# convexbrain/Totsu

Measured on AMD Instinct MI355X. Metric: solver iters/sec + time-to-eps, dense SOCP n=50k (value = iters/sec; time_to_eps beside it), higher is better.
Workload: dtype f32

## Files before the change

### include/totsu_f32hip.h

```cpp
#ifndef TOTSU_F32HIP_H
#define TOTSU_F32HIP_H

#include <stddef.h>
#include <stdint.h>

#ifdef __cplusplus
extern "C" {
#endif

#define THIP_E_INVALID   10001
#define THIP_E_NOTINIT   10002
#define THIP_E_NOGPU     10003
#define THIP_E_WORK      10004
#define THIP_E_NOCONV    10005
#define THIP_E_TIMEOUT   10006

int  thip_init(int device);
int  thip_shutdown(void);
int  thip_device_count(int *host_count);
int  thip_set_stream(void *hip_stream);
void *thip_get_stream(void);
int  thip_sync(void);
const char *thip_last_error(void);
const char *thip_version(void);

int thip_alloc(size_t n, float **out);
int thip_alloc_zeroed(size_t n, float **out);
int thip_free(float *p);
int thip_h2d(float *dst, const float *host_src, size_t n);
int thip_d2h(float *host_dst, const float *src, size_t n);
int thip_get(const float *x, size_t idx, float *host_out);
int thip_set(float *x, size_t idx, float val);

int thip_norm(size_t n, const float *x, float *host_out);
int thip_copy(size_t n, const float *x, float *y);
int thip_scale(size_t n, float alpha, float *x);
int thip_add(size_t n, float alpha, const float *x, float *y);
int thip_adds(size_t n, float s, float *y);
int thip_abssum(size_t len, const float *x, size_t incx, float *host_out);
int thip_transform_di(size_t n, float alpha, const float *d, const float *x,
                      float beta, float *y);

int thip_transform_ge(int transpose, size_t n_row, size_t n_col, float alpha, const float *mat,
                      const float *x, float beta, float *y);
int thip_set_lazy_gemv(int on);
int thip_get_lazy_gemv(int *host_on);
int thip_lazy_gemv_stats(int64_t *host_deferred, int64_t *host_flushes);
int thip_lazy_plan_stats(int64_t *host_hits, int64_t *host_misses);
int thip_lazy_read_stats(int64_t *host_served, int64_t *host_fetches);
int thip_transform_sp(size_t n, float alpha, const float *mat, const float *x, float beta, float *y);
enum { THIP_A_F32 = 0, THIP_A_BF16 = 1, THIP_A_F16 = 2 };
int thip_to_bf16(size_t n_row, size_t n_col, const float *mat, uint16_t *mat16, size_t ld16);
int thip_transform_ge_bf16(int transpose, size_t n_row, size_t n_col, float alpha, const uint16_t *mat16, size_t ld16,
                           const float *x, float beta, float *y);
int thip_to_f16(size_t n_row, size_t n_col, const float *mat, uint16_t *mat16, size_t ld16, float *inv_scale);
int thip_transform_ge_f16(int transpose, size_t n_row, size_t n_col, float alpha, const uint16_t *mat16, size_t ld16,
                          const float *inv_scale, const float *x, float beta, float *y);
size_t thip_map_eig_worklen(size_t n);
int thip_map_eig(size_t n, float *mat, int has_scale, float scale_diag, float eps_zero,
                 float *work, size_t worklen, int map_kind);
int thip_eig_decompose(size_t n, float *mat, int has_scale, float scale_diag, float eps_zero,
                       float *work, size_t worklen, float *host_w);
int thip_eig_rebuild(size_t n, float *mat, int has_scale, float scale_diag,
                     float *work, size_t worklen, const float *host_e, const uint8_t *host_keep);
int thip_eig_engine_info(int *host_engine, int *host_polish, float *host_cert);

int thip_spmv_csr(size_t n_row, size_t n_col, size_t nnz, const int64_t *dev_rowptr, const int32_t *dev_colidx,
                  const float *vals, float alpha, const float *x, float beta, float *y, int abs_mode);

typedef struct thip_sptile thip_sptile;
int thip_sptile_create(size_t n_row, size_t n_col, size_t nnz, const int64_t *host_colptr, const int32_t *host_rowidx,
                       const float *host_vals, thip_sptile **out);
int thip_sptile_destroy(thip_sptile *mat);
int thip_sptile_mv(thip_sptile *mat, int transpose, float alpha, const float *x, float beta, float *y, int abs_mode);
int thip_sptile_info(const thip_sptile *mat, size_t *host_nnz_stored, int *host_tiles, int *host_items_n, int *host_items_t,
                     int *host_slices_n, int *host_slices_t, size_t *host_bytes);
int thip_sptile_layout(const thip_sptile *mat, int *host_dense_tiles, size_t *host_indexed_entries, size_t *host_bytes_per_product);

typedef struct thip_sptile_builder thip_sptile_builder;
int thip_sptile_builder_create(size_t n_row, size_t n_col, thip_sptile_builder **out);
int thip_sptile_builder_count(thip_sptile_builder *b, size_t c0, size_t ncols, const float *dev_panel, size_t ld);
int thip_sptile_builder_plan(thip_sptile_builder *b, size_t *host_nnz, int *host_dense_tiles, size_t *host_indexed_entries,
                             size_t *host_bytes_per_product);
int thip_sptile_builder_fill(thip_sptile_builder *b, size_t c0, size_t ncols, const float *dev_panel, size_t ld);
int thip_sptile_builder_finish(thip_sptile_builder *b, thip_sptile **out);
int thip_sptile_builder_destroy(thip_sptile_builder *b);
int thip_sptile_from_dense(size_t n_row, size_t n_col, const float *dev_mat, size_t ld, thip_sptile **out);

int thip_norm_dev(size_t n, const float *x, float *dev_out);
int thip_dot_dev(size_t n, const float *x, const float *y, float *dev_out);
int thip_abssum_dev(size_t len, const float *x, size_t incx, float *dev_out);

int thip_absadd_cols(size_t n_row, size_t n_col, const float *mat, float *tau);
int thip_absadd_rows(size_t n_row, size_t n_col, const float *mat, float *sigma);
int thip_absadd_sympack(size_t n, const float *mat, float *y);
int thip_recip_max(size_t n, float eps_zero, float *x);

int thip_copy_block(int transposed, size_t n_row, size_t n_col, float sign, const float *src, float *dst, size_t ld_dst);

enum { THIP_CONE_ZERO = 0, THIP_CONE_RPOS = 1, THIP_CONE_SOC = 2, THIP_CONE_ROTSOC = 3, THIP_CONE_PSD = 4 };
int thip_proj_zero(int dual_cone, size_t n, float *x);
int thip_proj_rpos(size_t n, float *x);
int thip_proj_soc(size_t n, float *x);
int thip_proj_rotsoc(size_t n, float *x);
int thip_proj_soc_batched(float *x, const int64_t *dev_offs, size_t n_cones, int rotated, size_t max_len);
int thip_proj_psd(size_t sn, float *x, float eps_zero, float *work, size_t worklen);
int thip_group_min_batched(float *dp_tau, const int64_t *dev_offs, size_t n_groups, size_t max_len);

typedef struct thip_solver thip_solver;

enum { THIP_STATE_COMPENSATED = 0, THIP_STATE_PLAIN = 1 };

typedef struct thip_param {
    int64_t max_iter;
    float   eps_acc, eps_inf, eps_zero;
    int64_t log_period;
    int32_t state_arith;
    int32_t reserved;
} thip_param;

enum { THIP_ST_RUNNING = -1,
       THIP_ST_OK = 0, THIP_ST_UNBOUNDED = 1, THIP_ST_INFEASIBLE = 2, THIP_ST_EXCESS_ITER = 3,
       THIP_ST_INVALID_OP = 4, THIP_ST_WORK_SHORTAGE = 5, THIP_ST_CONE_FAILURE = 6 };

enum { THIP_SCHED_REFERENCE = 0,
       THIP_SCHED_FUSED     = 1,
       THIP_SCHED_CARRIED   = 2,
       THIP_SCHED_SWEEP     = 3 };

typedef struct thip_problem {
    size_t n, m;
    const float *mat_a;
    const float *vec_b;
    const float *vec_c;
    const float *vec_b_rowabs;
    size_t n_seg;
    const int32_t *host_seg_type;
    const int64_t *host_seg_len;
} thip_problem;

typedef struct thip_status {
    int32_t state;
    int64_t iter;
    int32_t kind;
    float   cri[3];
    float   tau, kappa;
    float   norm_b, norm_c;
} thip_status;

typedef int (*thip_allreduce_fn)(void *ctx, float *dev_buf, size_t n, void *hip_stream);

int thip_comm_unique_id(uint8_t *host_id128);
int thip_comm_init(int rank, int world, const uint8_t *host_id128);
int thip_comm_allreduce(float *dev_buf, size_t n);
int thip_comm_count(int *host_ranks);
int thip_comm_destroy(void);
int thip_solver_use_rccl(thip_solver *s);

int thip_oneshot_init(int rank, int world, size_t max_floats, uint8_t *host_handle64);
int thip_oneshot_connect(const uint8_t *host_handles);
int thip_oneshot_allreduce(float *dev_buf, size_t n);
int thip_oneshot_error(int *host_err);
int thip_oneshot_destroy(void);
int thip_solver_use_oneshot(thip_solver *s);

int thip_solver_create(const thip_problem *prob, const thip_param *par, int schedule, thip_solver **out);
int thip_solver_set_csr(thip_solver *s, size_t nnz,
                        const int64_t *dev_rowptr, const int32_t *dev_colidx, const float *dev_vals,
                        const int64_t *dev_t_rowptr, const int32_t *dev_t_colidx, const float *dev_t_vals);
int thip_solver_set_sptile(thip_solver *s, thip_sptile *mat);
int thip_solver_set_allreduce(thip_solver *s, thip_allreduce_fn fn, void *ctx);
enum { THIP_OVERLAP_OFF = 0, THIP_OVERLAP_LOCAL_ROWS = 1, THIP_OVERLAP_COLUMN_PIPELINE = 2, THIP_OVERLAP_COLUMN_INORDER = 3 };
int thip_solver_set_overlap(thip_solver *s, int mode);
int thip_solver_set_gemv_autotune(thip_solver *s, int on);
int thip_solver_set_lda_pad(thip_solver *s, int floats);
int thip_solver_overlap_info(thip_solver *s, int *host_mode, int *host_launches_per_pass, size_t *host_split_col);
int thip_solver_set_a_storage(thip_solver *s, int a_kind);
int thip_solver_set_a_bf16(thip_solver *s, const uint16_t *mat16, size_t ld16);
int thip_solver_set_a_f16(thip_solver *s, const uint16_t *mat16, size_t ld16, const float *inv_scale);
int thip_solver_init(thip_solver *s);
int thip_solver_run(thip_solver *s, int64_t max_steps, int64_t poll_every, thip_status *host_status);
int thip_solver_status(thip_solver *s, thip_status *host_status);
int thip_solver_resume(thip_solver *s);
int thip_solver_set_param(thip_solver *s, const thip_param *par);
int thip_solver_solution(thip_solver *s, float *host_x, float *host_y);
int thip_solver_iterate(thip_solver *s, float *host_x, float *host_y);
int thip_solver_precond(thip_solver *s, float *host_dp_tau, float *host_dp_sigma);
int thip_solver_destroy(thip_solver *s);
int thip_solver_passes(const thip_solver *s, int *host_passes, size_t *host_bytes_per_pass);
int thip_solver_schedule_in_use(thip_solver *s, int *host_schedule);
int thip_solver_set_sweep_min_bytes(thip_solver *s, size_t bytes);
int thip_solver_sweep_plan(thip_solver *s, int *host_members, int *host_cols_per_panel, int *host_slots, float *host_ms);
int thip_solver_set_column_shard(thip_solver *s, int on);
int thip_sweep_probe(size_t m, size_t n_local, size_t lda, int elem, int *host_ok);

typedef struct thip_batch thip_batch;
#define THIP_BATCH_MAX 64
#define THIP_BATCH_GROUP_DEFAULT 8
typedef struct thip_batch_info_t {
    int32_t n_inst, max_group;
    int32_t groups;
    int32_t passes_per_iteration;
    int32_t a_copies;
    int32_t reserved;
    size_t  a_bytes;
    size_t  bytes_per_pass;
    size_t  arena_bytes;
    size_t  device_bytes;
    int32_t plan_nj[4], plan_blocks[4];
    float   plan_ms[4];
} thip_batch_info_t;
int thip_batch_create(const thip_problem *prob_template, int n_inst, const float *const *host_vec_b,
                      const float *const *host_vec_c, const thip_param *par, thip_batch **out);
int thip_batch_set_a_storage(thip_batch *b, int a_kind);
int thip_batch_set_gemv_autotune(thip_batch *b, int on);
int thip_batch_set_max_group(thip_batch *b, int max_group);
int thip_batch_set_param(thip_batch *b, const thip_param *par);
int thip_batch_init(thip_batch *b);
int thip_batch_run(thip_batch *b, int64_t max_steps, int64_t poll_every, thip_status *host_status);
int thip_batch_status(thip_batch *b, int i, thip_status *host_status);
int thip_batch_solution(thip_batch *b, int i, float *host_x, float *host_y);
int thip_batch_iterate(thip_batch *b, int i, float *host_x, float *host_y);
int thip_batch_precond(thip_batch *b, int i, float *host_dp_tau, float *host_dp_sigma);
int thip_batch_info(const thip_batch *b, thip_batch_info_t *host_info);
int thip_batch_grouping(int n_inst, int max_group, int *host_groups, int *host_members);
int thip_batch_destroy(thip_batch *b);

int thip_batch_replace(thip_batch *b, int i, const float *dev_vec_b, const float *dev_vec_c);
int thip_batch_set_regroup(thip_batch *b, int on);
int thip_batch_run_until_any(thip_batch *b, int64_t max_steps, int64_t poll_every, thip_status *host_status);
int thip_batch_live_grouping(int n_inst, int max_group, const int *host_live, int *host_groups, int *host_group_sizes,
                             int *host_members);
typedef struct thip_batch_counters_t {
    int64_t launches[4];
    int64_t passes;
    int64_t instance_iterations;
    int64_t replaced;
    int32_t live, groups_now;
} thip_batch_counters_t;
int thip_batch_counters(const thip_batch *b, thip_batch_counters_t *host);

typedef struct thip_smallbatch thip_smallbatch;
typedef struct thip_smallbatch_info_t {
    int32_t n_prob, threads;
    int32_t lds_bytes, live;
    size_t  arena_bytes;
    size_t  device_bytes;
    size_t  device_bytes_all;
    int64_t launches, workgroups;
} thip_smallbatch_info_t;
int thip_smallbatch_fits(size_t n, size_t m, size_t n_seg, const int32_t *host_seg_type, const int64_t *host_seg_len,
                         size_t *host_lds_bytes, int *host_threads);
int thip_smallbatch_create(size_t n, size_t m, size_t n_prob, const float *dev_mats_a, const float *dev_vecs_b,
                           const float *dev_vecs_c, const float *dev_vecs_b_rowabs, size_t n_seg, const int32_t *host_seg_type,
                           const int64_t *host_seg_len, const thip_param *par, thip_smallbatch **out);
int thip_smallbatch_set_param(thip_smallbatch *h, const thip_param *par);
int thip_smallbatch_init(thip_smallbatch *h);
int thip_smallbatch_run(thip_smallbatch *h, int64_t max_steps, int64_t poll_every, thip_status *host_status);
int thip_smallbatch_run_until_any(thip_smallbatch *h, int64_t max_steps, int64_t poll_every, thip_status *host_status);
int thip_smallbatch_status(thip_smallbatch *h, int i, thip_status *host_status);
int thip_smallbatch_solution(thip_smallbatch *h, int i, float *host_x, float *host_y);
int thip_smallbatch_iterate(thip_smallbatch *h, int i, float *host_x, float *host_y);
int thip_smallbatch_precond(thip_smallbatch *h, int i, float *host_dp_tau, float *host_dp_sigma);
int thip_smallbatch_replace(thip_smallbatch *h, int i, const float *dev_mat_a, const float *dev_vec_b, const float *dev_vec_c,
                            const float *dev_vec_b_rowabs);
int thip_smallbatch_info(const thip_smallbatch *h, thip_smallbatch_info_t *host_info);
int thip_smallbatch_destroy(thip_smallbatch *h);

typedef struct thip_midbatch thip_midbatch;
typedef struct thip_midbatch_info_t {
    int32_t n_prob, threads;
    int32_t lds_bytes, live;
    size_t  arena_bytes;
    size_t  device_bytes;
    size_t  device_bytes_all;
    int64_t launches, workgroups;
    int32_t load_bytes, reserved;
    size_t  a_bytes_per_iter;
} thip_midbatch_info_t;
int thip_midbatch_fits(size_t n, size_t m, size_t n_seg, const int32_t *host_seg_type, const int64_t *host_seg_len,
                       size_t *host_lds_bytes, int *host_threads);
int thip_midbatch_create(size_t n, size_t m, size_t n_prob, const float *dev_mats_a, const float *dev_vecs_b,
                         const float *dev_vecs_c, const float *dev_vecs_b_rowabs, size_t n_seg, const int32_t *host_seg_type,
                         const int64_t *host_seg_len, const thip_param *par, thip_midbatch **out);
int thip_midbatch_set_param(thip_midbatch *h, const thip_param *par);
int thip_midbatch_init(thip_midbatch *h);
int thip_midbatch_run(thip_midbatch *h, int64_t max_steps, int64_t poll_every, thip_status *host_status);
int thip_midbatch_run_until_any(thip_midbatch *h, int64_t max_steps, int64_t poll_every, thip_status *host_status);
int thip_midbatch_status(thip_midbatch *h, int i, thip_status *host_status);
int thip_midbatch_solution(thip_midbatch *h, int i, float *host_x, float *host_y);
int thip_midbatch_iterate(thip_midbatch *h, int i, float *host_x, float *host_y);
int thip_midbatch_precond(thip_midbatch *h, int i, float *host_dp_tau, float *host_dp_sigma);
int thip_midbatch_replace(thip_midbatch *h, int i, const float *dev_mat_a, const float *dev_vec_b, const float *dev_vec_c,
                          const float *dev_vec_b_rowabs);
int thip_midbatch_info(const thip_midbatch *h, thip_midbatch_info_t *host_info);
int thip_midbatch_destroy(thip_midbatch *h);

typedef struct thip_sdpbatch thip_sdpbatch;
typedef struct thip_sdpbatch_info_t {
    int32_t n_prob, threads;
    int32_t lds_bytes, live;
    size_t  arena_bytes;
    size_t  device_bytes;
    size_t  device_bytes_all;
    int64_t launches, workgroups;
    int32_t load_bytes, reserved;
    size_t  a_bytes_per_iter;
    int32_t max_psd_order, n_psd;
    size_t  psd_lds_bytes;
} thip_sdpbatch_info_t;
int thip_sdpbatch_fits(size_t n, size_t m, size_t n_seg, const int32_t *host_seg_type, const int64_t *host_seg_len,
                       size_t *host_lds_bytes, int *host_threads);
int thip_sdpbatch_create(size_t n, size_t m, size_t n_prob, const float *dev_mats_a, const float *dev_vecs_b,
                         const float *dev_vecs_c, const float *dev_vecs_b_rowabs, size_t n_seg, const int32_t *host_seg_type,
                         const int64_t *host_seg_len, const thip_param *par, thip_sdpbatch **out);
int thip_sdpbatch_set_param(thip_sdpbatch *h, const thip_param *par);
int thip_sdpbatch_init(thip_sdpbatch *h);
int thip_sdpbatch_run(thip_sdpbatch *h, int64_t max_steps, int64_t poll_every, thip_status *host_status);
int thip_sdpbatch_run_until_any(thip_sdpbatch *h, int64_t max_steps, int64_t poll_every, thip_status *host_status);
int thip_sdpbatch_status(thip_sdpbatch *h, int i, thip_status *host_status);
int thip_sdpbatch_solution(thip_sdpbatch *h, int i, float *host_x, float *host_y);
int thip_sdpbatch_iterate(thip_sdpbatch *h, int i, float *host_x, float *host_y);
int thip_sdpbatch_precond(thip_sdpbatch *h, int i, float *host_dp_tau, float *host_dp_sigma);
int thip_sdpbatch_replace(thip_sdpbatch *h, int i, const float *dev_mat_a, const float *dev_vec_b, const float *dev_vec_c,
                          const float *dev_vec_b_rowabs);
int thip_sdpbatch_info(const thip_sdpbatch *h, thip_sdpbatch_info_t *host_info);
int thip_sdpbatch_destroy(thip_sdpbatch *h);

int thip_stream_probe(const void *dev_ptr, size_t bytes, int reps, float *host_best_ms, float *host_avg_ms);

int thip_solver_sweep_faults(thip_solver *s, int *host_faults, int *host_last_word, int64_t *host_restored_iter);
int thip_solver_set_sweep_publish(thip_solver *s, int agent_scope);
int thip_sweep_publish_selftest(int mode, int *host_agent_scope, int *host_info);


int thip_solver_gemv_plan(const thip_solver *s, int *host_nj, int *host_blocks, float *host_ms);

int thip_prof_enable(int on);
int thip_prof_read_psd(int64_t *host_spans, double *host_total_ms);
int thip_prof_read(int64_t *host_launches, double *host_total_ms);

int thip_gen_vector(float *out, size_t n, uint64_t seed, uint64_t stream, uint64_t idx0,
                    int kind, float scale, float shift);
int thip_gen_matrix(float *out, size_t n_row, size_t n_col, size_t lda, uint64_t seed, uint64_t stream,
                    uint64_t row0, uint64_t col0, uint64_t ld_index, int kind, float scale, float shift);
int thip_gen_identity(float *out, size_t n_row, size_t n_col, size_t lda, uint64_t row0, float value);


#ifdef __cplusplus
}
#endif
#endif
```

### rust/totsu_f32hip/src/ffi.rs

```rust
#![allow(non_camel_case_types)]
use std::os::raw::{c_char, c_int, c_void};

#[repr(C)]
pub struct thip_param { pub max_iter: i64, pub eps_acc: f32, pub eps_inf: f32, pub eps_zero: f32, pub log_period: i64,
                         pub state_arith: i32, pub reserved: i32 }
pub const THIP_STATE_COMPENSATED: i32 = 0;
pub const THIP_STATE_PLAIN: i32 = 1;

#[repr(C)]
pub struct thip_problem {
    pub n: usize, pub m: usize,
    pub mat_a: *const f32, pub vec_b: *const f32, pub vec_c: *const f32, pub vec_b_rowabs: *const f32,
    pub n_seg: usize, pub host_seg_type: *const i32, pub host_seg_len: *const i64,
}

#[repr(C)]
#[derive(Default, Clone, Copy)]
pub struct thip_status {
    pub state: i32, pub iter: i64, pub kind: i32, pub cri: [f32; 3],
    pub tau: f32, pub kappa: f32, pub norm_b: f32, pub norm_c: f32,
}

#[repr(C)]
#[derive(Default, Clone, Copy)]
pub struct thip_batch_info_t {
    pub n_inst: i32, pub max_group: i32, pub groups: i32, pub passes_per_iteration: i32, pub a_copies: i32, pub reserved: i32,
    pub a_bytes: usize, pub bytes_per_pass: usize, pub arena_bytes: usize, pub device_bytes: usize,
    pub plan_nj: [i32; 4], pub plan_blocks: [i32; 4], pub plan_ms: [f32; 4],
}
#[repr(C)]
#[derive(Default, Clone, Copy)]
pub struct thip_batch_counters_t {
    pub launches: [i64; 4], pub passes: i64, pub instance_iterations: i64, pub replaced: i64,
    pub live: i32, pub groups_now: i32,
}
#[repr(C)]
#[derive(Default, Clone, Copy)]
pub struct thip_smallbatch_info_t {
    pub n_prob: i32, pub threads: i32, pub lds_bytes: i32, pub live: i32,
    pub arena_bytes: usize, pub device_bytes: usize, pub device_bytes_all: usize,
    pub launches: i64, pub workgroups: i64,
}
#[repr(C)]
#[derive(Default, Clone, Copy)]
pub struct thip_midbatch_info_t {
    pub n_prob: i32, pub threads: i32, pub lds_bytes: i32, pub live: i32,
    pub arena_bytes: usize, pub device_bytes: usize, pub device_bytes_all: usize,
    pub launches: i64, pub workgroups: i64,
    pub load_bytes: i32, pub reserved: i32,
    pub a_bytes_per_iter: usize,
}
#[repr(C)]
#[derive(Default, Clone, Copy)]
pub struct thip_sdpbatch_info_t {
    pub n_prob: i32, pub threads: i32, pub lds_bytes: i32, pub live: i32,
    pub arena_bytes: usize, pub device_bytes: usize, pub device_bytes_all: usize,
    pub launches: i64, pub workgroups: i64,
    pub load_bytes: i32, pub reserved: i32,
    pub a_bytes_per_iter: usize,
    pub max_psd_order: i32, pub n_psd: i32,
    pub psd_lds_bytes: usize,
}
pub const THIP_BATCH_MAX: c_int = 64;
pub const THIP_BATCH_GROUP_DEFAULT: c_int = 8;

#[repr(C)]
pub struct thip_sweep_test {
    pub m: usize, pub n: usize, pub lda: usize,
    pub mat_a: *const f32, pub v: *const f32, pub xy: *const f32, pub c: *const f32, pub su: *const f32, pub tx: *const f32,
    pub u: *mut f32, pub ku: *mut f32,
    pub xx_in: *const f32, pub kx_in: *const f32,
    pub xx_out: *mut f32, pub kx_out: *mut f32, pub gp: *mut f32, pub hn: *mut f32, pub h3: *mut f32,
    pub kappa: f32, pub rtau: f32, pub first: i32, pub reps: i32,
    pub force_members: i32, pub pub_agent: i32, pub variant: i32, pub elem: i32,
    pub inv_s: *const f32,
    pub host_sums: *mut f32,
}

pub enum thip_solver {}
pub enum thip_batch {}
pub enum thip_smallbatch {}
pub enum thip_midbatch {}
pub enum thip_sdpbatch {}
pub enum thip_sptile {}
pub enum thip_sptile_builder {}
pub type thip_allreduce_fn = Option<unsafe extern "C" fn(ctx: *mut c_void, dev_buf: *mut f32, n: usize, stream: *mut c_void) -> c_int>;

pub const THIP_CONE_ZERO: i32 = 0;
pub const THIP_CONE_RPOS: i32 = 1;
pub const THIP_CONE_SOC: i32 = 2;
pub const THIP_CONE_ROTSOC: i32 = 3;
pub const THIP_CONE_PSD: i32 = 4;
pub const THIP_SCHED_REFERENCE: c_int = 0;
pub const THIP_SCHED_FUSED: c_int = 1;
pub const THIP_SCHED_CARRIED: c_int = 2;
pub const THIP_SCHED_SWEEP: c_int = 3;
pub const THIP_OVERLAP_OFF: c_int = 0;
pub const THIP_OVERLAP_LOCAL_ROWS: c_int = 1;
pub const THIP_OVERLAP_COLUMN_PIPELINE: c_int = 2;
pub const THIP_OVERLAP_COLUMN_INORDER: c_int = 3;

extern "C" {
    pub fn thip_init(device: c_int) -> c_int;
    pub fn thip_shutdown() -> c_int;
    pub fn thip_sync() -> c_int;
    pub fn thip_last_error() -> *const c_char;
    pub fn thip_alloc(n: usize, out: *mut *mut f32) -> c_int;
    pub fn thip_free(p: *mut f32) -> c_int;
    pub fn thip_h2d(dst: *mut f32, host_src: *const f32, n: usize) -> c_int;
    pub fn thip_d2h(host_dst: *mut f32, src: *const f32, n: usize) -> c_int;
    pub fn thip_get(x: *const f32, idx: usize, host_out: *mut f32) -> c_int;
    pub fn thip_set(x: *mut f32, idx: usize, val: f32) -> c_int;

    pub fn thip_norm(n: usize, x: *const f32, host_out: *mut f32) -> c_int;
    pub fn thip_copy(n: usize, x: *const f32, y: *mut f32) -> c_int;
    pub fn thip_scale(n: usize, alpha: f32, x: *mut f32) -> c_int;
    pub fn thip_add(n: usize, alpha: f32, x: *const f32, y: *mut f32) -> c_int;
    pub fn thip_adds(n: usize, s: f32, y: *mut f32) -> c_int;
    pub fn thip_abssum(len: usize, x: *const f32, incx: usize, host_out: *mut f32) -> c_int;
    pub fn thip_transform_di(n: usize, alpha: f32, d: *const f32, x: *const f32, beta: f32, y: *mut f32) -> c_int;

    pub fn thip_transform_ge(transpose: c_int, n_row: usize, n_col: usize, alpha: f32, mat: *const f32,
                             x: *const f32, beta: f32, y: *mut f32) -> c_int;
    pub fn thip_transform_sp(n: usize, alpha: f32, mat: *const f32, x: *const f32, beta: f32, y: *mut f32) -> c_int;
    pub fn thip_map_eig_worklen(n: usize) -> usize;
    pub fn thip_map_eig(n: usize, mat: *mut f32, has_scale: c_int, scale_diag: f32, eps_zero: f32,
                        work: *mut f32, worklen: usize, map_kind: c_int) -> c_int;
    pub fn thip_eig_decompose(n: usize, mat: *mut f32, has_scale: c_int, scale_diag: f32, eps_zero: f32,
                              work: *mut f32, worklen: usize, host_w: *mut f32) -> c_int;
    pub fn thip_eig_rebuild(n: usize, mat: *mut f32, has_scale: c_int, scale_diag: f32, work: *mut f32,
                            worklen: usize, host_e: *const f32, host_keep: *const u8) -> c_int;
    pub fn thip_eig_engine_info(host_engine: *mut c_int, host_polish: *mut c_int, host_cert: *mut f32) -> c_int;

    pub fn thip_absadd_cols(n_row: usize, n_col: usize, mat: *const f32, tau: *mut f32) -> c_int;
    pub fn thip_absadd_rows(n_row: usize, n_col: usize, mat: *const f32, sigma: *mut f32) -> c_int;
    pub fn thip_recip_max(n: usize, eps_zero: f32, x: *mut f32) -> c_int;
    pub fn thip_copy_block(transposed: c_int, n_row: usize, n_col: usize, sign: f32, src: *const f32, dst: *mut f32,
                           ld_dst: usize) -> c_int;
    pub fn thip_set_lazy_gemv(on: c_int) -> c_int;
    pub fn thip_get_lazy_gemv(host_on: *mut c_int) -> c_int;
    pub fn thip_lazy_gemv_stats(host_deferred: *mut i64, host_flushes: *mut i64) -> c_int;
    pub fn thip_lazy_plan_stats(host_hits: *mut i64, host_misses: *mut i64) -> c_int;
    pub fn thip_lazy_read_stats(host_served: *mut i64, host_fetches: *mut i64) -> c_int;
    pub fn thip_proj_zero(dual_cone: c_int, n: usize, x: *mut f32) -> c_int;
    pub fn thip_proj_rpos(n: usize, x: *mut f32) -> c_int;
    pub fn thip_proj_soc(n: usize, x: *mut f32) -> c_int;
    pub fn thip_proj_rotsoc(n: usize, x: *mut f32) -> c_int;
    pub fn thip_proj_psd(sn: usize, x: *mut f32, eps_zero: f32, work: *mut f32, worklen: usize) -> c_int;

    pub fn thip_solver_create(prob: *const thip_problem, par: *const thip_param, schedule: c_int,
                              out: *mut *mut thip_solver) -> c_int;
    pub fn thip_solver_set_allreduce(s: *mut thip_solver, f: thip_allreduce_fn, ctx: *mut c_void) -> c_int;
    pub fn thip_solver_set_overlap(s: *mut thip_solver, mode: c_int) -> c_int;
    pub fn thip_solver_overlap_info(s: *mut thip_solver, host_mode: *mut c_int, host_launches_per_pass: *mut c_int,
                                    host_split_col: *mut usize) -> c_int;
    pub fn thip_solver_init(s: *mut thip_solver) -> c_int;
    pub fn thip_solver_run(s: *mut thip_solver, max_steps: i64, poll_every: i64, host_status: *mut thip_status) -> c_int;
    pub fn thip_solver_solution(s: *mut thip_solver, host_x: *mut f32, host_y: *mut f32) -> c_int;
    pub fn thip_solver_destroy(s: *mut thip_solver) -> c_int;

    pub fn thip_version() -> *const c_char;
    pub fn thip_device_count(host_count: *mut c_int) -> c_int;
    pub fn thip_set_stream(hip_stream: *mut c_void) -> c_int;
    pub fn thip_get_stream() -> *mut c_void;
    pub fn thip_alloc_zeroed(n: usize, out: *mut *mut f32) -> c_int;

    pub fn thip_norm_dev(n: usize, x: *const f32, dev_out: *mut f32) -> c_int;
    pub fn thip_dot_dev(n: usize, x: *const f32, y: *const f32, dev_out: *mut f32) -> c_int;
    pub fn thip_abssum_dev(len: usize, x: *const f32, incx: usize, dev_out: *mut f32) -> c_int;
    pub fn thip_absadd_sympack(n: usize, mat: *const f32, y: *mut f32) -> c_int;
    pub fn thip_spmv_csr(n_row: usize, n_col: usize, nnz: usize, dev_rowptr: *const i64, dev_colidx: *const i32,
                         vals: *const f32, alpha: f32, x: *const f32, beta: f32, y: *mut f32, abs_mode: c_int) -> c_int;
    pub fn thip_sptile_create(n_row: usize, n_col: usize, nnz: usize, host_colptr: *const i64, host_rowidx: *const i32,
                              host_vals: *const f32, out: *mut *mut thip_sptile) -> c_int;
    pub fn thip_sptile_destroy(mat: *mut thip_sptile) -> c_int;
    pub fn thip_sptile_mv(mat: *mut thip_sptile, transpose: c_int, alpha: f32, x: *const f32, beta: f32, y: *mut f32,
                          abs_mode: c_int) -> c_int;
    pub fn thip_sptile_info(mat: *const thip_sptile, host_nnz_stored: *mut usize, host_tiles: *mut c_int,
                            host_items_n: *mut c_int, host_items_t: *mut c_int, host_slices_n: *mut c_int,
                            host_slices_t: *mut c_int, host_bytes: *mut usize) -> c_int;
    pub fn thip_sptile_layout(mat: *const thip_sptile, host_dense_tiles: *mut c_int, host_indexed_entries: *mut usize,
                              host_bytes_per_product: *mut usize) -> c_int;
    pub fn thip_sptile_builder_create(n_row: usize, n_col: usize, out: *mut *mut thip_sptile_builder) -> c_int;
    pub fn thip_sptile_builder_count(b: *mut thip_sptile_builder, c0: usize, ncols: usize, dev_panel: *const f32,
                                     ld: usize) -> c_int;
    pub fn thip_sptile_builder_plan(b: *mut thip_sptile_builder, host_nnz: *mut usize, host_dense_tiles: *mut c_int,
                                    host_indexed_entries: *mut usize, host_bytes_per_product: *mut usize) -> c_int;
    pub fn thip_sptile_builder_fill(b: *mut thip_sptile_builder, c0: usize, ncols: usize, dev_panel: *const f32,
                                    ld: usize) -> c_int;
    pub fn thip_sptile_builder_finish(b: *mut thip_sptile_builder, out: *mut *mut thip_sptile) -> c_int;
    pub fn thip_sptile_builder_destroy(b: *mut thip_sptile_builder) -> c_int;
    pub fn thip_sptile_from_dense(n_row: usize, n_col: usize, dev_mat: *const f32, ld: usize,
                                  out: *mut *mut thip_sptile) -> c_int;
    pub fn thip_to_bf16(n_row: usize, n_col: usize, mat: *const f32, mat16: *mut u16, ld16: usize) -> c_int;
    pub fn thip_transform_ge_bf16(transpose: c_int, n_row: usize, n_col: usize, alpha: f32, mat16: *const u16,
                                  ld16: usize, x: *const f32, beta: f32, y: *mut f32) -> c_int;

    pub fn thip_proj_soc_batched(x: *mut f32, dev_offs: *const i64, n_cones: usize, rotated: c_int, max_len: usize) -> c_int;
    pub fn thip_group_min_batched(dp_tau: *mut f32, dev_offs: *const i64, n_groups: usize, max_len: usize) -> c_int;

    pub fn thip_solver_set_csr(s: *mut thip_solver, nnz: usize, dev_rowptr: *const i64, dev_colidx: *const i32,
                               dev_vals: *const f32, dev_t_rowptr: *const i64, dev_t_colidx: *const i32,
                               dev_t_vals: *const f32) -> c_int;
    pub fn thip_solver_set_sptile(s: *mut thip_solver, mat: *mut thip_sptile) -> c_int;
    pub fn thip_solver_set_a_storage(s: *mut thip_solver, a_kind: c_int) -> c_int;
    pub fn thip_solver_set_a_bf16(s: *mut thip_solver, mat16: *const u16, ld16: usize) -> c_int;
    pub fn thip_solver_set_a_f16(s: *mut thip_solver, mat16: *const u16, ld16: usize, inv_scale: *const f32) -> c_int;
    pub fn thip_to_f16(n_row: usize, n_col: usize, mat: *const f32, mat16: *mut u16, ld16: usize, inv_scale: *mut f32) -> c_int;
    pub fn thip_transform_ge_f16(transpose: c_int, n_row: usize, n_col: usize, alpha: f32, mat16: *const u16, ld16: usize,
                                 inv_scale: *const f32, x: *const f32, beta: f32, y: *mut f32) -> c_int;
    pub fn thip_solver_set_param(s: *mut thip_solver, par: *const thip_param) -> c_int;
    pub fn thip_solver_resume(s: *mut thip_solver) -> c_int;
    pub fn thip_solver_status(s: *mut thip_solver, host_status: *mut thip_status) -> c_int;
    pub fn thip_solver_iterate(s: *mut thip_solver, host_x: *mut f32, host_y: *mut f32) -> c_int;
    pub fn thip_solver_precond(s: *mut thip_solver, host_dp_tau: *mut f32, host_dp_sigma: *mut f32) -> c_int;
    pub fn thip_solver_passes(s: *const thip_solver, host_passes: *mut c_int, host_bytes_per_pass: *mut usize) -> c_int;
    pub fn thip_solver_schedule_in_use(s: *mut thip_solver, host_schedule: *mut c_int) -> c_int;
    pub fn thip_solver_set_sweep_min_bytes(s: *mut thip_solver, bytes: usize) -> c_int;
    pub fn thip_solver_set_column_shard(s: *mut thip_solver, on: c_int) -> c_int;
    pub fn thip_sweep_probe(m: usize, n_local: usize, lda: usize, elem: c_int, host_ok: *mut c_int) -> c_int;
    pub fn thip_solver_sweep_plan(s: *mut thip_solver, host_members: *mut c_int, host_cols_per_panel: *mut c_int, host_slots: *mut c_int, host_ms: *mut f32) -> c_int;
    pub fn thip_stream_probe(dev_ptr: *const c_void, bytes: usize, reps: c_int, host_best_ms: *mut f32, host_avg_ms: *mut f32) -> c_int;
    pub fn thip_solver_sweep_faults(s: *mut thip_solver, host_faults: *mut c_int, host_last_word: *mut c_int, host_restored_iter: *mut i64) -> c_int;
    pub fn thip_solver_set_sweep_publish(s: *mut thip_solver, agent_scope: c_int) -> c_int;
    pub fn thip_sweep_publish_selftest(mode: c_int, host_agent_scope: *mut c_int, host_info: *mut c_int) -> c_int;
    pub fn thip_solver_gemv_plan(s: *const thip_solver, host_nj: *mut c_int, host_blocks: *mut c_int, host_ms: *mut f32) -> c_int;

    pub fn thip_batch_create(prob_template: *const thip_problem, n_inst: c_int, host_vec_b: *const *const f32,
                             host_vec_c: *const *const f32, par: *const thip_param, out: *mut *mut thip_batch) -> c_int;
    pub fn thip_batch_set_a_storage(b: *mut thip_batch, a_kind: c_int) -> c_int;
    pub fn thip_batch_set_gemv_autotune(b: *mut thip_batch, on: c_int) -> c_int;
    pub fn thip_batch_set_max_group(b: *mut thip_batch, max_group: c_int) -> c_int;
    pub fn thip_batch_set_param(b: *mut thip_batch, par: *const thip_param) -> c_int;
    pub fn thip_batch_init(b: *mut thip_batch) -> c_int;
    pub fn thip_batch_run(b: *mut thip_batch, max_steps: i64, poll_every: i64, host_status: *mut thip_status) -> c_int;
    pub fn thip_batch_status(b: *mut thip_batch, i: c_int, host_status: *mut thip_status) -> c_int;
    pub fn thip_batch_solution(b: *mut thip_batch, i: c_int, host_x: *mut f32, host_y: *mut f32) -> c_int;
    pub fn thip_batch_iterate(b: *mut thip_batch, i: c_int, host_x: *mut f32, host_y: *mut f32) -> c_int;
    pub fn thip_batch_precond(b: *mut thip_batch, i: c_int, host_dp_tau: *mut f32, host_dp_sigma: *mut f32) -> c_int;
    pub fn thip_batch_info(b: *const thip_batch, host_info: *mut thip_batch_info_t) -> c_int;
    pub fn thip_batch_grouping(n_inst: c_int, max_group: c_int, host_groups: *mut c_int, host_members: *mut c_int) -> c_int;
    pub fn thip_batch_destroy(b: *mut thip_batch) -> c_int;
    pub fn thip_batch_replace(b: *mut thip_batch, i: c_int, dev_vec_b: *const f32, dev_vec_c: *const f32) -> c_int;
    pub fn thip_batch_set_regroup(b: *mut thip_batch, on: c_int) -> c_int;
    pub fn thip_batch_run_until_any(b: *mut thip_batch, max_steps: i64, poll_every: i64, host_status: *mut thip_status) -> c_int;
    pub fn thip_batch_live_grouping(n_inst: c_int, max_group: c_int, host_live: *const c_int, host_groups: *mut c_int,
                                    host_group_sizes: *mut c_int, host_members: *mut c_int) -> c_int;
    pub fn thip_batch_counters(b: *const thip_batch, host: *mut thip_batch_counters_t) -> c_int;

    pub fn thip_smallbatch_fits(n: usize, m: usize, n_seg: usize, host_seg_type: *const i32, host_seg_len: *const i64,
                                host_lds_bytes: *mut usize, host_threads: *mut c_int) -> c_int;
    pub fn thip_smallbatch_create(n: usize, m: usize, n_prob: usize, dev_mats_a: *const f32, dev_vecs_b: *const f32,
                                  dev_vecs_c: *const f32, dev_vecs_b_rowabs: *const f32, n_seg: usize, host_seg_type: *const i32,
                                  host_seg_len: *const i64, par: *const thip_param, out: *mut *mut thip_smallbatch) -> c_int;
    pub fn thip_smallbatch_set_param(h: *mut thip_smallbatch, par: *const thip_param) -> c_int;
    pub fn thip_smallbatch_init(h: *mut thip_smallbatch) -> c_int;
    pub fn thip_smallbatch_run(h: *mut thip_smallbatch, max_steps: i64, poll_every: i64, host_status: *mut thip_status) -> c_int;
    pub fn thip_smallbatch_run_until_any(h: *mut thip_smallbatch, max_steps: i64, poll_every: i64, host_status: *mut thip_status) -> c_int;
    pub fn thip_smallbatch_status(h: *mut thip_smallbatch, i: c_int, host_status: *mut thip_status) -> c_int;
    pub fn thip_smallbatch_solution(h: *mut thip_smallbatch, i: c_int, host_x: *mut f32, host_y: *mut f32) -> c_int;
    pub fn thip_smallbatch_iterate(h: *mut thip_smallbatch, i: c_int, host_x: *mut f32, host_y: *mut f32) -> c_int;
    pub fn thip_smallbatch_precond(h: *mut thip_smallbatch, i: c_int, host_dp_tau: *mut f32, host_dp_sigma: *mut f32) -> c_int;
    pub fn thip_smallbatch_replace(h: *mut thip_smallbatch, i: c_int, dev_mat_a: *const f32, dev_vec_b: *const f32,
                                   dev_vec_c: *const f32, dev_vec_b_rowabs: *const f32) -> c_int;
    pub fn thip_smallbatch_info(h: *const thip_smallbatch, host_info: *mut thip_smallbatch_info_t) -> c_int;
    pub fn thip_smallbatch_destroy(h: *mut thip_smallbatch) -> c_int;
    pub fn thip_test_smallbatch_force_threads(h: *mut thip_smallbatch, threads: c_int) -> c_int;

    pub fn thip_midbatch_fits(n: usize, m: usize, n_seg: usize, host_seg_type: *const i32, host_seg_len: *const i64,
                              host_lds_bytes: *mut usize, host_threads: *mut c_int) -> c_int;
    pub fn thip_midbatch_create(n: usize, m: usize, n_prob: usize, dev_mats_a: *const f32, dev_vecs_b: *const f32,
                                dev_vecs_c: *const f32, dev_vecs_b_rowabs: *const f32, n_seg: usize, host_seg_type: *const i32,
                                host_seg_len: *const i64, par: *const thip_param, out: *mut *mut thip_midbatch) -> c_int;
    pub fn thip_midbatch_set_param(h: *mut thip_midbatch, par: *const thip_param) -> c_int;
    pub fn thip_midbatch_init(h: *mut thip_midbatch) -> c_int;
    pub fn thip_midbatch_run(h: *mut thip_midbatch, max_steps: i64, poll_every: i64, host_status: *mut thip_status) -> c_int;
    pub fn thip_midbatch_run_until_any(h: *mut thip_midbatch, max_steps: i64, poll_every: i64, host_status: *mut thip_status) -> c_int;
    pub fn thip_midbatch_status(h: *mut thip_midbatch, i: c_int, host_status: *mut thip_status) -> c_int;
    pub fn thip_midbatch_solution(h: *mut thip_midbatch, i: c_int, host_x: *mut f32, host_y: *mut f32) -> c_int;
    pub fn thip_midbatch_iterate(h: *mut thip_midbatch, i: c_int, host_x: *mut f32, host_y: *mut f32) -> c_int;
    pub fn thip_midbatch_precond(h: *mut thip_midbatch, i: c_int, host_dp_tau: *mut f32, host_dp_sigma: *mut f32) -> c_int;
    pub fn thip_midbatch_replace(h: *mut thip_midbatch, i: c_int, dev_mat_a: *const f32, dev_vec_b: *const f32,
                                 dev_vec_c: *const f32, dev_vec_b_rowabs: *const f32) -> c_int;
    pub fn thip_midbatch_info(h: *const thip_midbatch, host_info: *mut thip_midbatch_info_t) -> c_int;
    pub fn thip_midbatch_destroy(h: *mut thip_midbatch) -> c_int;
    pub fn thip_test_midbatch_force_threads(h: *mut thip_midbatch, threads: c_int) -> c_int;

    pub fn thip_sdpbatch_fits(n: usize, m: usize, n_seg: usize, host_seg_type: *const i32, host_seg_len: *const i64,
                              host_lds_bytes: *mut usize, host_threads: *mut c_int) -> c_int;
    pub fn thip_sdpbatch_create(n: usize, m: usize, n_prob: usize, dev_mats_a: *const f32, dev_vecs_b: *const f32,
                                dev_vecs_c: *const f32, dev_vecs_b_rowabs: *const f32, n_seg: usize, host_seg_type: *const i32,
                                host_seg_len: *const i64, par: *const thip_param, out: *mut *mut thip_sdpbatch) -> c_int;
    pub fn thip_sdpbatch_set_param(h: *mut thip_sdpbatch, par: *const thip_param) -> c_int;
    pub fn thip_sdpbatch_init(h: *mut thip_sdpbatch) -> c_int;
    pub fn thip_sdpbatch_run(h: *mut thip_sdpbatch, max_steps: i64, poll_every: i64, host_status: *mut thip_status) -> c_int;
    pub fn thip_sdpbatch_run_until_any(h: *mut thip_sdpbatch, max_steps: i64, poll_every: i64, host_status: *mut thip_status) -> c_int;
    pub fn thip_sdpbatch_status(h: *mut thip_sdpbatch, i: c_int, host_status: *mut thip_status) -> c_int;
    pub fn thip_sdpbatch_solution(h: *mut thip_sdpbatch, i: c_int, host_x: *mut f32, host_y: *mut f32) -> c_int;
    pub fn thip_sdpbatch_iterate(h: *mut thip_sdpbatch, i: c_int, host_x: *mut f32, host_y: *mut f32) -> c_int;
    pub fn thip_sdpbatch_precond(h: *mut thip_sdpbatch, i: c_int, host_dp_tau: *mut f32, host_dp_sigma: *mut f32) -> c_int;
    pub fn thip_sdpbatch_replace(h: *mut thip_sdpbatch, i: c_int, dev_mat_a: *const f32, dev_vec_b: *const f32,
                                 dev_vec_c: *const f32, dev_vec_b_rowabs: *const f32) -> c_int;
    pub fn thip_sdpbatch_info(h: *const thip_sdpbatch, host_info: *mut thip_sdpbatch_info_t) -> c_int;
    pub fn thip_sdpbatch_destroy(h: *mut thip_sdpbatch) -> c_int;
    pub fn thip_test_sdpbatch_force_threads(h: *mut thip_sdpbatch, threads: c_int) -> c_int;
    pub fn thip_test_sdpbatch_project(k: c_int, count: c_int, dev_packed: *mut f32, dev_rx_or_null: *mut f32) -> c_int;

    pub fn thip_comm_unique_id(host_id128: *mut u8) -> c_int;
    pub fn thip_comm_init(rank: c_int, world: c_int, host_id128: *const u8) -> c_int;
    pub fn thip_comm_allreduce(dev_buf: *mut f32, n: usize) -> c_int;
    pub fn thip_comm_count(host_ranks: *mut c_int) -> c_int;
    pub fn thip_comm_destroy() -> c_int;
    pub fn thip_solver_use_rccl(s: *mut thip_solver) -> c_int;
    pub fn thip_oneshot_init(rank: c_int, world: c_int, max_floats: usize, host_handle64: *mut u8) -> c_int;
    pub fn thip_oneshot_connect(host_handles: *const u8) -> c_int;
    pub fn thip_oneshot_allreduce(dev_buf: *mut f32, n: usize) -> c_int;
    pub fn thip_oneshot_error(host_err: *mut c_int) -> c_int;
    pub fn thip_oneshot_destroy() -> c_int;
    pub fn thip_solver_use_oneshot(s: *mut thip_solver) -> c_int;
    pub fn thip_solver_set_gemv_autotune(s: *mut thip_solver, on: c_int) -> c_int;
    pub fn thip_solver_set_lda_pad(s: *mut thip_solver, floats: c_int) -> c_int;

    pub fn thip_gen_vector(out: *mut f32, n: usize, seed: u64, stream: u64, idx0: u64, kind: c_int, scale: f32, shift: f32) -> c_int;
    pub fn thip_gen_matrix(out: *mut f32, n_row: usize, n_col: usize, lda: usize, seed: u64, stream: u64, row0: u64,
                           col0: u64, ld_index: u64, kind: c_int, scale: f32, shift: f32) -> c_int;
    pub fn thip_gen_identity(out: *mut f32, n_row: usize, n_col: usize, lda: usize, row0: u64, value: f32) -> c_int;

    pub fn thip_prof_enable(on: c_int) -> c_int;
    pub fn thip_prof_read(host_launches: *mut i64, host_total_ms: *mut f64) -> c_int;
    pub fn thip_prof_read_psd(host_spans: *mut i64, host_total_ms: *mut f64) -> c_int;
}

#[cfg(feature = "test-hooks")]
extern "C" {
    pub fn thip_test_eig_force(engine: c_int) -> c_int;
    pub fn thip_test_gemv_multi(m: usize, n: usize, mat: *const f32, nv: c_int, host_xn: *const *const f32, host_xt: *const *const f32,
                                host_out_n: *const *mut f32, host_out_t: *const *mut f32, host_stopped: *const c_int, nj: c_int,
                                target_blocks: c_int, reps: c_int, host_ms: *mut f32) -> c_int;
    pub fn thip_test_spin_allreduce(s: *mut thip_solver, latency_us: c_int) -> c_int;
    pub fn thip_test_sweep(t: *const thip_sweep_test, host_ms: *mut f32, host_info: *mut c_int) -> c_int;
    pub fn thip_test_solver_kahan(s: *mut thip_solver, host_kx: *mut f32, host_ky: *mut f32, host_ks: *mut f32, host_ku: *mut f32,
                                  host_kv: *mut f32, host_mtail_form: *mut c_int) -> c_int;
    pub fn thip_test_sweep_fault(s: *mut thip_solver, kind: c_int, after_sweeps: i64, spin_max: c_int) -> c_int;
    pub fn thip_test_gemm_sym(n: c_int, ld: c_int, alpha: f32, a: *const f32, b: *const f32, beta: f32, d: *const f32,
                              gamma: f32, c: *mut f32) -> c_int;
    pub fn thip_test_gemm_chain(shape: c_int, kernel: c_int, n: c_int, ld: c_int, nb: c_int, alpha: f32, x: *const f32,
                                y: *const f32, beta: f32, d: *const f32, gamma: f32, c: *mut f32) -> c_int;
    pub fn thip_test_chain_probe(mode: c_int, ld: c_int, reps: c_int, host_us: *mut f32) -> c_int;
    pub fn thip_test_sptile_time(mat: *mut thip_sptile, reps: c_int, host_ms: *mut f32) -> c_int;
    pub fn thip_test_sptile_equal(a: *const thip_sptile, b: *const thip_sptile, host_first_difference: *mut c_int) -> c_int;
    pub fn thip_test_gemm_dual(kernel: c_int, n: c_int, ld: c_int, nb: c_int, a: *const f32, b0: *const f32, b1: *const f32,
                               coef: *const f32, o0: *mut f32, o1: *mut f32) -> c_int;
}

pub const THIP_A_F32: c_int = 0;
pub const THIP_A_BF16: c_int = 1;
pub const THIP_A_F16: c_int = 2;

pub fn chk(rc: c_int) {
    if rc != 0 {
        let msg = unsafe { std::ffi::CStr::from_ptr(thip_last_error()) }.to_string_lossy().into_owned();
        panic!("totsu_f32hip: error {}: {}", rc, msg);
    }
}
```

### totsu_amd/_lib.py

```python
import ctypes as C
import os

_HERE = os.path.dirname(os.path.abspath(__file__))
SO_PATH = os.path.join(_HERE, "lib", "libtotsu_f32hip.so")

E_INVALID, E_NOTINIT, E_NOGPU, E_WORK, E_NOCONV, E_TIMEOUT = 10001, 10002, 10003, 10004, 10005, 10006

ST_RUNNING, ST_OK, ST_UNBOUNDED, ST_INFEASIBLE, ST_EXCESS_ITER, ST_INVALID_OP, ST_WORK_SHORTAGE, ST_CONE_FAILURE = \
    -1, 0, 1, 2, 3, 4, 5, 6
SCHED_REFERENCE, SCHED_FUSED, SCHED_CARRIED, SCHED_SWEEP = 0, 1, 2, 3
STATE_COMPENSATED, STATE_PLAIN = 0, 1
CONE_ZERO, CONE_RPOS, CONE_SOC, CONE_ROTSOC, CONE_PSD = 0, 1, 2, 3, 4

fp = C.POINTER(C.c_float)


class ThipError(RuntimeError):
    def __init__(self, code, msg):
        super().__init__("totsu_f32hip error %d: %s" % (code, msg))
        self.code = code


class Param(C.Structure):
    _fields_ = [("max_iter", C.c_int64), ("eps_acc", C.c_float), ("eps_inf", C.c_float),
                ("eps_zero", C.c_float), ("log_period", C.c_int64), ("state_arith", C.c_int32), ("reserved", C.c_int32)]


class Problem(C.Structure):
    _fields_ = [("n", C.c_size_t), ("m", C.c_size_t), ("mat_a", C.c_void_p), ("vec_b", C.c_void_p),
                ("vec_c", C.c_void_p), ("vec_b_rowabs", C.c_void_p), ("n_seg", C.c_size_t),
                ("host_seg_type", C.POINTER(C.c_int32)), ("host_seg_len", C.POINTER(C.c_int64))]


class Status(C.Structure):
    _fields_ = [("state", C.c_int32), ("iter", C.c_int64), ("kind", C.c_int32), ("cri", C.c_float * 3),
                ("tau", C.c_float), ("kappa", C.c_float), ("norm_b", C.c_float), ("norm_c", C.c_float)]


class SweepTest(C.Structure):
    _fields_ = [("m", C.c_size_t), ("n", C.c_size_t), ("lda", C.c_size_t)] + \
               [(k, C.c_void_p) for k in ("mat_a", "v", "xy", "c", "su", "tx", "u", "ku", "xx_in", "kx_in", "xx_out",
                                          "kx_out", "gp", "hn", "h3")] + \
               [("kappa", C.c_float), ("rtau", C.c_float), ("first", C.c_int32), ("reps", C.c_int32),
                ("force_members", C.c_int32), ("pub_agent", C.c_int32), ("variant", C.c_int32), ("elem", C.c_int32), ("inv_s", C.c_void_p),
                ("host_sums", C.POINTER(C.c_float))]


class BatchInfo(C.Structure):
    _fields_ = [("n_inst", C.c_int32), ("max_group", C.c_int32), ("groups", C.c_int32), ("passes_per_iteration", C.c_int32),
                ("a_copies", C.c_int32), ("reserved", C.c_int32), ("a_bytes", C.c_size_t), ("bytes_per_pass", C.c_size_t),
                ("arena_bytes", C.c_size_t), ("device_bytes", C.c_size_t), ("plan_nj", C.c_int32 * 4),
                ("plan_blocks", C.c_int32 * 4), ("plan_ms", C.c_float * 4)]


class BatchCounters(C.Structure):
    _fields_ = [("launches", C.c_int64 * 4), ("passes", C.c_int64), ("instance_iterations", C.c_int64), ("replaced", C.c_int64),
                ("live", C.c_int32), ("groups_now", C.c_int32)]


class SmallBatchInfo(C.Structure):
    _fields_ = [("n_prob", C.c_int32), ("threads", C.c_int32), ("lds_bytes", C.c_int32), ("live", C.c_int32),
                ("arena_bytes", C.c_size_t), ("device_bytes", C.c_size_t), ("device_bytes_all", C.c_size_t),
                ("launches", C.c_int64), ("workgroups", C.c_int64)]


class MidBatchInfo(C.Structure):
    _fields_ = SmallBatchInfo._fields_ + [("load_bytes", C.c_int32), ("reserved", C.c_int32), ("a_bytes_per_iter", C.c_size_t)]


class SdpBatchInfo(C.Structure):
    _fields_ = MidBatchInfo._fields_ + [("max_psd_order", C.c_int32), ("n_psd", C.c_int32), ("psd_lds_bytes", C.c_size_t)]


BATCH_MAX, BATCH_GROUP_DEFAULT = 64, 8
SMALLBATCH_MAX_DIM, SMALLBATCH_MAX_AREA, SMALLBATCH_MAX_PROB, SMALLBATCH_LDS_MAX = 1024, 24576, 1048576, 163840
ALLREDUCE_FN = C.CFUNCTYPE(C.c_int, C.c_void_p, C.c_void_p, C.c_size_t, C.c_void_p)

_sz, _f, _i, _vp, _u64 = C.c_size_t, C.c_float, C.c_int, C.c_void_p, C.c_uint64
PROTOTYPES = {
    "thip_init": (_i, [_i]),
    "thip_shutdown": (_i, []),
    "thip_device_count": (_i, [C.POINTER(_i)]),
    "thip_set_stream": (_i, [_vp]),
    "thip_get_stream": (_vp, []),
    "thip_sync": (_i, []),
    "thip_last_error": (C.c_char_p, []),
    "thip_version": (C.c_char_p, []),
    "thip_alloc": (_i, [_sz, C.POINTER(_vp)]),
    "thip_alloc_zeroed": (_i, [_sz, C.POINTER(_vp)]),
    "thip_free": (_i, [_vp]),
    "thip_h2d": (_i, [_vp, _vp, _sz]),
    "thip_d2h": (_i, [_vp, _vp, _sz]),
    "thip_get": (_i, [_vp, _sz, fp]),
    "thip_set": (_i, [_vp, _sz, _f]),
    "thip_norm": (_i, [_sz, _vp, fp]),
    "thip_copy": (_i, [_sz, _vp, _vp]),
    "thip_scale": (_i, [_sz, _f, _vp]),
    "thip_add": (_i, [_sz, _f, _vp, _vp]),
    "thip_adds": (_i, [_sz, _f, _vp]),
    "thip_abssum": (_i, [_sz, _vp, _sz, fp]),
    "thip_transform_di": (_i, [_sz, _f, _vp, _vp, _f, _vp]),
    "thip_transform_ge": (_i, [_i, _sz, _sz, _f, _vp, _vp, _f, _vp]),
    "thip_transform_sp": (_i, [_sz, _f, _vp, _vp, _f, _vp]),
    "thip_set_lazy_gemv": (_i, [_i]),
    "thip_get_lazy_gemv": (_i, [C.POINTER(_i)]),
    "thip_lazy_gemv_stats": (_i, [C.POINTER(C.c_int64), C.POINTER(C.c_int64)]),
    "thip_lazy_plan_stats": (_i, [C.POINTER(C.c_int64), C.POINTER(C.c_int64)]),
    "thip_lazy_read_stats": (_i, [C.POINTER(C.c_int64), C.POINTER(C.c_int64)]),
    "thip_to_bf16": (_i, [_sz, _sz, _vp, _vp, _sz]),
    "thip_to_f16": (_i, [_sz, _sz, _vp, _vp, _sz, _vp]),
    "thip_transform_ge_f16": (_i, [_i, _sz, _sz, _f, _vp, _sz, _vp, _vp, _f, _vp]),
    "thip_transform_ge_bf16": (_i, [_i, _sz, _sz, _f, _vp, _sz, _vp, _f, _vp]),
    "thip_spmv_csr": (_i, [_sz, _sz, _sz, _vp, _vp, _vp, _f, _vp, _f, _vp, _i]),
    "thip_sptile_create": (_i, [_sz, _sz, _sz, _vp, _vp, _vp, C.POINTER(_vp)]),
    "thip_sptile_destroy": (_i, [_vp]),
    "thip_sptile_mv": (_i, [_vp, _i, _f, _vp, _f, _vp, _i]),
    "thip_sptile_info": (_i, [_vp, C.POINTER(_sz), C.POINTER(_i), C.POINTER(_i), C.POINTER(_i), C.POINTER(_i), C.POINTER(_i),
                              C.POINTER(_sz)]),
    "thip_sptile_layout": (_i, [_vp, C.POINTER(_i), C.POINTER(_sz), C.POINTER(_sz)]),
    "thip_sptile_builder_create": (_i, [_sz, _sz, C.POINTER(_vp)]),
    "thip_sptile_builder_count": (_i, [_vp, _sz, _sz, _vp, _sz]),
    "thip_sptile_builder_plan": (_i, [_vp, C.POINTER(_sz), C.POINTER(_i), C.POINTER(_sz), C.POINTER(_sz)]),
    "thip_sptile_builder_fill": (_i, [_vp, _sz, _sz, _vp, _sz]),
    "thip_sptile_builder_finish": (_i, [_vp, C.POINTER(_vp)]),
    "thip_sptile_builder_destroy": (_i, [_vp]),
    "thip_sptile_from_dense": (_i, [_sz, _sz, _vp, _sz, C.POINTER(_vp)]),
    "thip_map_eig_worklen": (_sz, [_sz]),
    "thip_map_eig": (_i, [_sz, _vp, _i, _f, _f, _vp, _sz, _i]),
    "thip_eig_decompose": (_i, [_sz, _vp, _i, _f, _f, _vp, _sz, fp]),
    "thip_eig_rebuild": (_i, [_sz, _vp, _i, _f, _vp, _sz, fp, C.POINTER(C.c_uint8)]),
    "thip_eig_engine_info": (_i, [C.POINTER(_i), C.POINTER(_i), fp]),
    "thip_test_eig_force": (_i, [_i]),
    "thip_norm_dev": (_i, [_sz, _vp, _vp]),
    "thip_dot_dev": (_i, [_sz, _vp, _vp, _vp]),
    "thip_abssum_dev": (_i, [_sz, _vp, _sz, _vp]),
    "thip_absadd_cols": (_i, [_sz, _sz, _vp, _vp]),
    "thip_absadd_rows": (_i, [_sz, _sz, _vp, _vp]),
    "thip_absadd_sympack": (_i, [_sz, _vp, _vp]),
    "thip_recip_max": (_i, [_sz, _f, _vp]),
    "thip_copy_block": (_i, [_i, _sz, _sz, _f, _vp, _vp, _sz]),
    "thip_proj_zero": (_i, [_i, _sz, _vp]),
    "thip_proj_rpos": (_i, [_sz, _vp]),
    "thip_proj_soc": (_i, [_sz, _vp]),
    "thip_proj_rotsoc": (_i, [_sz, _vp]),
    "thip_proj_soc_batched": (_i, [_vp, _vp, _sz, _i, _sz]),
    "thip_proj_psd": (_i, [_sz, _vp, _f, _vp, _sz]),
    "thip_group_min_batched": (_i, [_vp, _vp, _sz, _sz]),
    "thip_comm_unique_id": (_i, [C.POINTER(C.c_uint8)]),
    "thip_comm_init": (_i, [_i, _i, C.POINTER(C.c_uint8)]),
    "thip_comm_allreduce": (_i, [_vp, _sz]),
    "thip_comm_count": (_i, [C.POINTER(_i)]),
    "thip_comm_destroy": (_i, []),
    "thip_solver_use_rccl": (_i, [_vp]),
    "thip_oneshot_init": (_i, [_i, _i, _sz, C.POINTER(C.c_uint8)]),
    "thip_oneshot_connect": (_i, [C.POINTER(C.c_uint8)]),
    "thip_oneshot_allreduce": (_i, [_vp, _sz]),
    "thip_oneshot_error": (_i, [C.POINTER(_i)]),
    "thip_oneshot_destroy": (_i, []),
    "thip_solver_use_oneshot": (_i, [_vp]),
    "thip_solver_set_gemv_autotune": (_i, [_vp, _i]),
    "thip_solver_set_lda_pad": (_i, [_vp, _i]),
    "thip_solver_create": (_i, [C.POINTER(Problem), C.POINTER(Param), _i, C.POINTER(_vp)]),
    "thip_solver_set_csr": (_i, [_vp, _sz, _vp, _vp, _vp, _vp, _vp, _vp]),
    "thip_solver_set_sptile": (_i, [_vp, _vp]),
    "thip_solver_set_allreduce": (_i, [_vp, ALLREDUCE_FN, _vp]),
    "thip_solver_set_overlap": (_i, [_vp, _i]),
    "thip_solver_overlap_info": (_i, [_vp, C.POINTER(_i), C.POINTER(_i), C.POINTER(_sz)]),
    "thip_test_spin_allreduce": (_i, [_vp, _i]),
    "thip_solver_set_a_storage": (_i, [_vp, _i]),
    "thip_solver_set_a_bf16": (_i, [_vp, _vp, _sz]),
    "thip_solver_set_a_f16": (_i, [_vp, _vp, _sz, _vp]),
    "thip_solver_resume": (_i, [_vp]),
    "thip_solver_set_param": (_i, [_vp, _vp]),
    "thip_solver_init": (_i, [_vp]),
    "thip_solver_run": (_i, [_vp, C.c_int64, C.c_int64, C.POINTER(Status)]),
    "thip_solver_status": (_i, [_vp, C.POINTER(Status)]),
    "thip_solver_solution": (_i, [_vp, _vp, _vp]),
    "thip_solver_iterate": (_i, [_vp, _vp, _vp]),
    "thip_solver_precond": (_i, [_vp, _vp, _vp]),
    "thip_solver_destroy": (_i, [_vp]),
    "thip_solver_passes": (_i, [_vp, C.POINTER(_i), C.POINTER(_sz)]),
    "thip_solver_schedule_in_use": (_i, [_vp, C.POINTER(_i)]),
    "thip_solver_set_sweep_min_bytes": (_i, [_vp, _sz]),
    "thip_solver_set_column_shard": (_i, [_vp, _i]),
    "thip_sweep_probe": (_i, [_sz, _sz, _sz, _i, C.POINTER(_i)]),
    "thip_solver_sweep_plan": (_i, [_vp, C.POINTER(_i), C.POINTER(_i), C.POINTER(_i), C.POINTER(_f)]),
    "thip_test_sweep": (_i, [_vp, C.POINTER(_f), C.POINTER(_i)]),
    "thip_stream_probe": (_i, [_vp, _sz, _i, C.POINTER(_f), C.POINTER(_f)]),
    "thip_solver_sweep_faults": (_i, [_vp, C.POINTER(_i), C.POINTER(_i), C.POINTER(C.c_int64)]),
    "thip_test_sweep_fault": (_i, [_vp, _i, C.c_int64, _i]),
    "thip_test_solver_kahan": (_i, [_vp, _vp, _vp, _vp, _vp, _vp, C.POINTER(_i)]),
    "thip_solver_set_sweep_publish": (_i, [_vp, _i]),
    "thip_sweep_publish_selftest": (_i, [_i, C.POINTER(_i), C.POINTER(_i)]),
    "thip_test_gemm_sym": (_i, [_i, _i, _f, _vp, _vp, _f, _vp, _f, _vp]),
    "thip_test_gemm_chain": (_i, [_i, _i, _i, _i, _i, _f, _vp, _vp, _f, _vp, _f, _vp]),
    "thip_test_chain_probe": (_i, [_i, _i, _i, C.POINTER(_f)]),
    "thip_test_sptile_time": (_i, [_vp, _i, C.POINTER(_f)]),
    "thip_test_sptile_equal": (_i, [_vp, _vp, C.POINTER(_i)]),
    "thip_test_gemm_dual": (_i, [_i, _i, _i, _i, _vp, _vp, _vp, _vp, _vp, _vp]),
    "thip_solver_gemv_plan": (_i, [_vp, C.POINTER(_i), C.POINTER(_i), C.POINTER(_f)]),
    "thip_batch_create": (_i, [C.POINTER(Problem), _i, C.POINTER(_vp), C.POINTER(_vp), C.POINTER(Param), C.POINTER(_vp)]),
    "thip_batch_set_a_storage": (_i, [_vp, _i]),
    "thip_batch_set_gemv_autotune": (_i, [_vp, _i]),
    "thip_batch_set_max_group": (_i, [_vp, _i]),
    "thip_batch_set_param": (_i, [_vp, _vp]),
    "thip_batch_init": (_i, [_vp]),
    "thip_batch_run": (_i, [_vp, C.c_int64, C.c_int64, C.POINTER(Status)]),
    "thip_batch_status": (_i, [_vp, _i, C.POINTER(Status)]),
    "thip_batch_solution": (_i, [_vp, _i, _vp, _vp]),
    "thip_batch_iterate": (_i, [_vp, _i, _vp, _vp]),
    "thip_batch_precond": (_i, [_vp, _i, _vp, _vp]),
    "thip_batch_info": (_i, [_vp, C.POINTER(BatchInfo)]),
    "thip_batch_grouping": (_i, [_i, _i, C.POINTER(_i), C.POINTER(_i)]),
    "thip_batch_destroy": (_i, [_vp]),
    "thip_batch_replace": (_i, [_vp, _i, _vp, _vp]),
    "thip_batch_set_regroup": (_i, [_vp, _i]),
    "thip_batch_run_until_any": (_i, [_vp, C.c_int64, C.c_int64, C.POINTER(Status)]),
    "thip_batch_live_grouping": (_i, [_i, _i, C.POINTER(_i), C.POINTER(_i), C.POINTER(_i), C.POINTER(_i)]),
    "thip_batch_counters": (_i, [_vp, C.POINTER(BatchCounters)]),
    "thip_test_gemv_multi": (_i, [_sz, _sz, _vp, _i, C.POINTER(_vp), C.POINTER(_vp), C.POINTER(_vp), C.POINTER(_vp),
                                  C.POINTER(_i), _i, _i, _i, C.POINTER(_f)]),
    "thip_test_sdpbatch_project": (_i, [_i, _i, _vp, _vp]),
    "thip_prof_enable": (_i, [_i]),
    "thip_prof_read": (_i, [C.POINTER(C.c_int64), C.POINTER(C.c_double)]),
    "thip_prof_read_psd": (_i, [C.POINTER(C.c_int64), C.POINTER(C.c_double)]),
    "thip_gen_vector": (_i, [_vp, _sz, _u64, _u64, _u64, _i, _f, _f]),
    "thip_gen_identity": (_i, [_vp, _sz, _sz, _sz, _u64, _f]),
    "thip_gen_matrix": (_i, [_vp, _sz, _sz, _sz, _u64, _u64, _u64, _u64, _u64, _i, _f, _f]),
}

for _name, _info in (("smallbatch", SmallBatchInfo), ("midbatch", MidBatchInfo), ("sdpbatch", SdpBatchInfo)):
    _p = "thip_%s_" % _name
    PROTOTYPES.update({
        _p + "fits": (_i, [_sz, _sz, _sz, C.POINTER(C.c_int32), C.POINTER(C.c_int64), C.POINTER(_sz), C.POINTER(_i)]),
        _p + "create": (_i, [_sz, _sz, _sz, _vp, _vp, _vp, _vp, _sz, C.POINTER(C.c_int32), C.POINTER(C.c_int64), C.POINTER(Param),
                             C.POINTER(_vp)]),
        _p + "set_param": (_i, [_vp, C.POINTER(Param)]),
        _p + "init": (_i, [_vp]),
        _p + "run": (_i, [_vp, C.c_int64, C.c_int64, C.POINTER(Status)]),
        _p + "run_until_any": (_i, [_vp, C.c_int64, C.c_int64, C.POINTER(Status)]),
        _p + "status": (_i, [_vp, _i, C.POINTER(Status)]),
        _p + "solution": (_i, [_vp, _i, _vp, _vp]),
        _p + "iterate": (_i, [_vp, _i, _vp, _vp]),
        _p + "precond": (_i, [_vp, _i, _vp, _vp]),
        _p + "replace": (_i, [_vp, _i, _vp, _vp, _vp, _vp]),
        _p + "info": (_i, [_vp, C.POINTER(_info)]),
        _p + "destroy": (_i, [_vp]),
        "thip_test_%s_force_threads" % _name: (_i, [_vp, _i]),
    })

_NOCHECK = {"thip_last_error", "thip_version", "thip_get_stream", "thip_map_eig_worklen"}

_cdll = None


def load():
    global _cdll
    if _cdll is not None:
        return _cdll
    if not os.path.exists(SO_PATH):
        raise ImportError("totsu_amd: %s is missing -- run `python -c 'import __graft_entry__ as g; g.build()'` "
                          "(there is no CPU fallback)" % SO_PATH)
    try:
        import torch
    except Exception:
        pass
    lib = C.CDLL(SO_PATH, mode=C.RTLD_GLOBAL)
    for name, (res, args) in PROTOTYPES.items():
        f = getattr(lib, name)
        f.restype = res
        f.argtypes = args
    _cdll = lib
    return lib


class _Checked:

    def __getattr__(self, name):
        lib = load()
        f = getattr(lib, name)
        if name in _NOCHECK:
            return f

        def call(*a):
            rc = f(*a)
            if rc != 0:
                raise ThipError(rc, lib.thip_last_error().decode(errors="replace"))
            return rc
        call.__name__ = name
        setattr(self, name, call)
        return call


lib = _Checked()
_inited = False


def init(device=None):
    global _inited
    if device is None:
        device = int(os.environ.get("LOCAL_RANK", "0"))
    lib.thip_init(int(device))
    _inited = True


class lazy_calls:

    def __enter__(self):
        prev = C.c_int(0)
        lib.thip_get_lazy_gemv(C.byref(prev))
        self.prev = prev.value
        lib.thip_set_lazy_gemv(1)
        return self

    def __exit__(self, *exc):
        lib.thip_set_lazy_gemv(self.prev)
        return False


def ensure_init():
    if not _inited:
        init()
```

### totsu_amd/csrc/thip_common.h

```cpp
#pragma once

#include <hip/hip_runtime.h>
#include <stddef.h>
#include <stdint.h>

#include "totsu_f32hip.h"
#include "totsu_f32hip_test.h"

namespace thip {

struct Ctx {
    bool         inited = false;
    int          device = 0;
    hipStream_t  own_stream = nullptr;
    hipStream_t  stream = nullptr;
    float       *scratch = nullptr;
    size_t       scratch_n = 0;
    float       *dev_scalar = nullptr;
    float       *pinned = nullptr;
    void        *stage = nullptr;
    size_t       stage_bytes = 0;
    hipEvent_t   stage_ev[2] = { nullptr, nullptr };
    int          num_cu = 256;
    int         *never_stop = nullptr;
    float       *eig_pin = nullptr;
    size_t       eig_pin_floats = 0;
    hipStream_t  eig_side = nullptr;
    hipEvent_t   eig_ev[2] = { nullptr, nullptr };
};

int  fetch_scalar(const float *dev_src, float *host_out);

Ctx &ctx();
bool lazy_pending();
int  lazy_flush();
int  lazy_push(int transpose, size_t n_row, size_t n_col, float alpha, const float *mat, const float *x, float beta,
               float *y, int *deferred);
int  lazy_push_scale(size_t n, float alpha, float *x, int *deferred);
int  lazy_push_add(size_t n, float alpha, const float *x, float *y, int *deferred);
int  lazy_push_proj(int kind, size_t n, float *x, int *deferred);
int  lazy_push_set(float *x, float value, int *deferred);
int  lazy_read(int is_norm, const float *p, size_t n, float *value, int *served);
void lazy_release();
void lazy_forget(uintptr_t lo, uintptr_t hi);
int  fail(int code, const char *what, const char *file, int line);
int  need_init();
int  scratch(size_t n, float **out);

#define THIP_TRY(expr)                                                            \
    do {                                                                          \
        hipError_t e__ = (expr);                                                  \
        if (e__ != hipSuccess) return ::thip::fail((int)e__, #expr, __FILE__, __LINE__); \
    } while (0)

#define THIP_RC(expr)                                                             \
    do {                                                                          \
        int rc__ = (expr);                                                        \
        if (rc__ != 0) return rc__;                                               \
    } while (0)

#define THIP_NEED_INIT()                                                          \
    do {                                                                          \
        if (!::thip::ctx().inited) return ::thip::need_init();                    \
        if (::thip::lazy_pending()) { int rcl__ = ::thip::lazy_flush(); if (rcl__ != 0) return rcl__; } \
    } while (0)

#define THIP_NEED_INIT_NOFLUSH()                                                  \
    do {                                                                          \
        if (!::thip::ctx().inited) return ::thip::need_init();                    \
    } while (0)

#define THIP_LAUNCH_CHECK() THIP_TRY(hipGetLastError())


__device__ __forceinline__ float wave_sum(float v)
{
#pragma unroll
    for (int o = 32; o > 0; o >>= 1) v += __shfl_xor(v, o, 64);
    return v;
}

__device__ __forceinline__ float wave_sum_dpp(float v)
{
#define THIP_DPP_ADD(ctrl, rows) v += __int_as_float(__builtin_amdgcn_update_dpp(0, __float_as_int(v), ctrl, rows, 0xf, true))
    THIP_DPP_ADD(0x111, 0xf);
    THIP_DPP_ADD(0x112, 0xf);
    THIP_DPP_ADD(0x114, 0xf);
    THIP_DPP_ADD(0x118, 0xf);
    THIP_DPP_ADD(0x142, 0xa);
    THIP_DPP_ADD(0x143, 0xc);
#undef THIP_DPP_ADD
    return __int_as_float(__builtin_amdgcn_readlane(__float_as_int(v), 63));
}

__device__ __forceinline__ double wave_sum_d(double v)
{
#pragma unroll
    for (int o = 32; o > 0; o >>= 1) v += __shfl_xor(v, o, 64);
    return v;
}

__device__ __forceinline__ float wave_min(float v)
{
#pragma unroll
    for (int o = 32; o > 0; o >>= 1) v = fminf(v, __shfl_xor(v, o, 64));
    return v;
}

__device__ __forceinline__ float block_sum(float v, float *sh)
{
    const int lane = threadIdx.x & 63, w = threadIdx.x >> 6, nw = (blockDim.x + 63) >> 6;
    v = wave_sum(v);
    __syncthreads();
    if (lane == 0) sh[w] = v;
    __syncthreads();
    float t = (lane < nw) ? sh[lane] : 0.0f;
    t = wave_sum(t);
    return t;
}

__device__ __forceinline__ float block_sum_dpp(float v, float *sh)
{
    const int lane = threadIdx.x & 63, w = threadIdx.x >> 6, nw = (blockDim.x + 63) >> 6;
    v = wave_sum_dpp(v);
    __syncthreads();
    if (lane == 0) sh[w] = v;
    __syncthreads();
    return wave_sum_dpp((lane < nw) ? sh[lane] : 0.0f);
}

__device__ __forceinline__ double block_sum_d(double v, double *sh)
{
    const int lane = threadIdx.x & 63, w = threadIdx.x >> 6, nw = (blockDim.x + 63) >> 6;
    v = wave_sum_d(v);
    __syncthreads();
    if (lane == 0) sh[w] = v;
    __syncthreads();
    double t = (lane < nw) ? sh[lane] : 0.0;
    t = wave_sum_d(t);
    return t;
}

__device__ __forceinline__ float block_min(float v, float *sh)
{
    const int lane = threadIdx.x & 63, w = threadIdx.x >> 6, nw = (blockDim.x + 63) >> 6;
    v = wave_min(v);
    __syncthreads();
    if (lane == 0) sh[w] = v;
    __syncthreads();
    float t = (lane < nw) ? sh[lane] : __builtin_inff();
    t = wave_min(t);
    return t;
}

static inline unsigned grid_for(size_t n, unsigned block, unsigned max_blocks)
{
    size_t g = (n + block - 1) / block;
    if (g < 1) g = 1;
    if (g > max_blocks) g = max_blocks;
    return (unsigned)g;
}

struct DenseA {
    const void *mat = nullptr; size_t lda = 0; int kind = THIP_A_F32; const float *inv_s = nullptr; bool pad_zero = false;
    bool is16() const { return kind != THIP_A_F32; }
    size_t elem_bytes() const { return is16() ? 2 : 4; }
    int vec_elems() const { return is16() ? 8 : 4; }
    bool vec_ok() const { return ((uintptr_t)mat & 15u) == 0 && lda % vec_elems() == 0; }
    int vec_width() const { return vec_ok() ? vec_elems() : 1; }
};
inline DenseA dense_f32(const float *mat, size_t lda) { return DenseA{ mat, lda, THIP_A_F32, nullptr, false }; }
int dual_gemv(hipStream_t st, size_t n_row, size_t n_col, const DenseA &A,
              const float *xn, float alphaN, float betaN, float *outN,
              const float *xt, float alphaT, float betaT, float *outT,
              bool abs_mode, const int *stop_flag);
int to_bf16(hipStream_t st, size_t n_row, size_t n_col, const float *src, uint16_t *dst, size_t ld16);
int to_f16(hipStream_t st, size_t n_row, size_t n_col, const float *src, uint16_t *dst, size_t ld16, float *inv_s);
struct GemvPartials {
    const float *partN; int nN; size_t strideN;
    const float *partT; int nT; size_t strideT;
};
struct GroupDesc { const float *A; const float *xn; const float *xt; float *partN; float *partT; int nr, nc, cpc, pad; };
int grouped_gemv(hipStream_t st, const GroupDesc *dev_tab, int n_desc, int max_tiles, int max_chunks, int mode);
struct GemvHint { int nj; int target_blocks; };
const GemvHint *gemv_candidates(int *count);
int dual_gemv_partials(hipStream_t st, size_t n_row, size_t n_col, const DenseA &A,
                       const float *xn, const float *xt, bool do_n, bool do_t, bool abs_mode,
                       float *scratch_base, size_t scratch_floats, GemvPartials *out, const int *stop_flag,
                       const GemvHint *hint = nullptr);
int dual_gemv_partials_cols(hipStream_t st, size_t n_row, size_t n_col, const DenseA &A,
                            const float *xn, const float *xt, bool do_n, bool do_t, bool abs_mode,
                            float *scratch_base, size_t scratch_floats, GemvPartials *out, const int *stop_flag,
                            const GemvHint *hint, size_t col0, size_t col1, int chunk_row0, int max_chunk_rows,
                            int *chunks_used);
int dual_gemv_chunk_rows(size_t n_row, size_t cols, const DenseA &A, const GemvHint *hint, int *tiles);
int dual_gemv_partials_geometry(size_t n_row, size_t n_col, const DenseA &A, bool do_n, bool do_t,
                                float *scratch_base, GemvPartials *out);
size_t dual_gemv_scratch_floats(size_t n_row, size_t n_col);
int finalize_partials(hipStream_t st, size_t n, const float *part, int np, size_t stride, float alpha, float beta,
                      float *y, const int *stop);

constexpr int GEMV_MULTI_MAX = 8;
struct MultiTab { const float *xn[GEMV_MULTI_MAX]; const float *xt[GEMV_MULTI_MAX]; float *scr[GEMV_MULTI_MAX]; const int *stop[GEMV_MULTI_MAX]; };
int gemv_multi_instance(int nv);
const GemvHint *gemv_multi_candidates(int *count);
size_t dual_gemv_multi_scratch_floats(size_t n_row, size_t n_col);
int dual_gemv_multi_partials(hipStream_t st, size_t n_row, size_t n_col, const DenseA &A, int nv, const float *const *xn,
                             const float *const *xt, float *const *scratch, size_t scratch_floats, const int *const *stop,
                             GemvPartials *out, const GemvHint *hint = nullptr);

constexpr int SW_SPIN_MAX = 2000000;
struct SweepGeom { int G, ngroups, rows_per_member, cols_per_group, nslot, npan, w, variant, m_eff; size_t mpad; int elem; };
struct SweepArgs {
    const float *A; size_t lda; int m, n;
    const float *inv_s;
    int G, rows_per_member, cols_per_group;
    const float *v, *xy;
    const float *c, *Su, *Tx;
    float *u, *ku;
    const float *xx_in, *kx_in;
    float *xx_out, *kx_out;
    float *gP;
    float *partH; size_t mpad;
    unsigned long long *gran;
    unsigned *census;
    unsigned seq, tagbase;
    int first;
    int dbg;
    const int *stop; const float *kappa_p, *rtau_p;
    float *pn; int pn_stride; const float *tau_p; float eps_zero;
    const float *pn_in; int pn_in_stride;
    int spin_max;
    int fault;
    int pub_agent;
    float *kappa_out; const float *skappa_p; const float *pm_brx; int np_m, pn_count;
};
int sweep_publish_default();
int sweep_plan(size_t m, size_t n, const DenseA &A, SweepGeom *g);
int sweep_candidates(size_t m, size_t n, const DenseA &A, SweepGeom *out, int max_out);
int sweep_launch16(hipStream_t st, const SweepGeom &g, const SweepArgs &a);
size_t sweep_gran_words(const SweepGeom &g);
int sweep_census_dry_run(hipStream_t st, unsigned *census, unsigned seq);
int sweep_launch(hipStream_t st, const SweepGeom &g, const SweepArgs &a);

size_t sptile_part_floats(const thip_sptile *M, bool tphase);
int sptile_slices(const thip_sptile *M, bool tphase);
size_t sptile_pad(const thip_sptile *M, bool tphase);
size_t sptile_bytes_per_pass(const thip_sptile *M);
void sptile_dims(const thip_sptile *M, size_t *m, size_t *n, size_t *nnz);
constexpr int SPT_NMAX = 256;
int sptile_product(hipStream_t st, const thip_sptile *M, bool tphase, const float *in0, const float *in1, float *part,
                   float *xmax, int abs_mode, const int *stop, bool xmax_ready = false);
int sptile_colupdate(hipStream_t st, const thip_sptile *M, const SweepArgs &a, const float *partT, float *xmax);

thip_allreduce_fn oneshot_hook();
const unsigned *oneshot_error_word();

void prof_release();

int reduce_to_dev(hipStream_t st, int op, size_t n, const float *x, const float *y, size_t incx, float *dev_out);
enum { RED_SUMSQ_SQRT = 0, RED_ABSSUM = 1, RED_DOT = 2 };

int soc_batched(hipStream_t st, float *x, const int64_t *dev_begs, const int64_t *dev_ends, size_t n_cones,
                int rotated, size_t max_len, const int *stop);
int soc_batched2(hipStream_t st, float *x0, float *x1, float *rx0, float *rx1, const int64_t *dev_begs,
                 const int64_t *dev_ends, size_t n_cones, int rotated, size_t max_len, const int *stop);
int group_min_batched(hipStream_t st, float *t, const int64_t *dev_begs, const int64_t *dev_ends, size_t n_groups,
                      size_t max_len);

int eig_psd_project(hipStream_t st, size_t n, float *packed, int has_scale, float scale_diag, float eps_zero,
                    float *work, size_t worklen, int map_kind, const int *stop, int nbatch = 1, ptrdiff_t pstride = 0,
                    float *rx = nullptr, ptrdiff_t rx_stride = 0);
bool psd_project_takes_rx(size_t n);
int eig_psd_project_small(hipStream_t st, size_t n, float *base, const int64_t *dev_offs, int count, int has_scale,
                          float scale_diag, const int *stop, int nbatch, ptrdiff_t pstride, float *rx = nullptr,
                          ptrdiff_t rx_stride = 0);
size_t psd_small_max();

size_t tri_eigen_scratch_floats(int n);
int tri_eigen(hipStream_t st, int n, int ld, const float *d, const float *e, float *w32, float *V0, unsigned *cert_bits,
              float *scr);
int tri_orth_partials(hipStream_t st, int n, int ld, const float *P, float *part, int nblocks);
int tri_map(hipStream_t st, int n, int ld, int map_kind, const float *w, float *e);

__host__ __device__ __forceinline__ uint64_t rng_hash(uint64_t seed, uint64_t stream, uint64_t idx)
{
    uint64_t z = seed * 0x9E3779B97F4A7C15ull + stream * 0xD1B54A32D192ED03ull + idx * 0xBF58476D1CE4E5B9ull
                 + 0x94D049BB133111EBull;
    z = (z ^ (z >> 30)) * 0xBF58476D1CE4E5B9ull;
    z = (z ^ (z >> 27)) * 0x94D049BB133111EBull;
    z = z ^ (z >> 31);
    return z;
}
__host__ __device__ __forceinline__ float rng_uniform(uint64_t seed, uint64_t stream, uint64_t idx)
{
    return (float)(rng_hash(seed, stream, idx) >> 40) * (1.0f / 16777216.0f);
}
__host__ __device__ __forceinline__ float rng_normal(uint64_t seed, uint64_t stream, uint64_t idx)
{
    const uint64_t h = rng_hash(seed, stream, idx);
    const uint32_t s = (uint32_t)(h & 0xFFFF) + (uint32_t)((h >> 16) & 0xFFFF)
                     + (uint32_t)((h >> 32) & 0xFFFF) + (uint32_t)((h >> 48) & 0xFFFF);
    return ((float)((int32_t)s - 131070) * (1.0f / 65536.0f)) * 1.7320508f;
}

}
```

### totsu_amd/csrc/thip_gemv.hip

```cpp
#include "thip_common.h"
#include "thip_gemv_reduce.h"

#include <cstdlib>

using namespace thip;

namespace {

constexpr int BLK = 256;
constexpr int MAXCW = 1024;

typedef unsigned short bf16raw;
typedef _Float16 f16elt;
template <typename E> struct IsF16 { static constexpr bool v = false; };
template <> struct IsF16<f16elt> { static constexpr bool v = true; };
__device__ __forceinline__ float elt_f32(float v) { return v; }
__device__ __forceinline__ float elt_f32(bf16raw v) { return __uint_as_float((unsigned)v << 16); }
__device__ __forceinline__ float elt_f32(f16elt v) { return (float)v; }
__device__ __forceinline__ unsigned raw16(bf16raw v) { return v; }
__device__ __forceinline__ unsigned raw16(f16elt v) { return (unsigned)__builtin_bit_cast(unsigned short, v); }

template <typename E, int VW, int NJ, int K, bool DO_N, bool DO_T, bool ABS, bool NT, bool FULL, bool CLAMP = false>
__device__ __forceinline__ void step(const E *__restrict__ A, size_t lda, int m, int r_first, int c, int cc,
                                     const float *__restrict__ xn, const float (&xtv)[NJ][VW],
                                     float (&accN)[NJ][VW], float *ldsT_wave, int lane, const float *__restrict__ inv_s,
                                     const int (&rofs)[NJ])
{
    static_assert(FULL || !CLAMP, "CLAMP is a form of FULL");
    constexpr bool F16 = IsF16<E>::v;
    if constexpr (VW == 8) {
        typedef unsigned u32x4_t __attribute__((ext_vector_type(4)));
        u32x4_t raw[K][NJ];
        float xsv[K], isv[K];
#pragma unroll
        for (int u = 0; u < K; ++u) {
            isv[u] = F16 ? inv_s[c + u] : 1.0f;
            xsv[u] = ((ABS || !DO_N) ? 1.0f : xn[c + u]) * isv[u];
        }
        if constexpr (FULL) {
#pragma unroll
            for (int u = 0; u < K; ++u) {
                const E *col = A + (size_t)(c + u) * lda + (CLAMP ? 0 : r_first);
#pragma unroll
                for (int j = 0; j < NJ; ++j) {
                    const u32x4_t *src = reinterpret_cast<const u32x4_t *>(col + (CLAMP ? rofs[j] : j * (BLK * VW)));
                    raw[u][j] = NT ? __builtin_nontemporal_load(src) : *src;
                }
            }
            __builtin_amdgcn_sched_barrier(0);
        } else {
#pragma unroll
            for (int u = 0; u < K; ++u) {
                const E *col = A + (size_t)(c + u) * lda;
#pragma unroll
                for (int j = 0; j < NJ; ++j) {
                    const int r = r_first + j * (BLK * VW);
                    if (r + 8 <= m) {
                        raw[u][j] = *reinterpret_cast<const u32x4_t *>(col + r);
                    } else {
#pragma unroll
                        for (int d = 0; d < 4; ++d) {
                            const unsigned lo = (r + 2 * d < m) ? raw16(col[r + 2 * d]) : 0u;
                            const unsigned hi = (r + 2 * d + 1 < m) ? raw16(col[r + 2 * d + 1]) : 0u;
                            raw[u][j][d] = lo | (hi << 16);
                        }
                    }
                }
            }
        }
        float p[K];
        constexpr unsigned HI = ABS ? 0x7fff0000u : 0xffff0000u;
#pragma unroll
        for (int u = 0; u < K; ++u) {
            typedef float f32x2_t __attribute__((ext_vector_type(2)));
            const f32x2_t xs2 = { xsv[u], xsv[u] };
            f32x2_t s2 = { 0.0f, 0.0f };
#pragma unroll
            for (int j = 0; j < NJ; ++j)
#pragma unroll
                for (int d = 0; d < 4; ++d) {
                    const unsigned q = raw[u][j][d];
                    f32x2_t a2;
                    if constexpr (F16) {
                        typedef _Float16 f16x2_t __attribute__((ext_vector_type(2)));
                        const f16x2_t hv = __builtin_bit_cast(f16x2_t, q);
                        a2 = f32x2_t{ (float)hv[0], (float)hv[1] };
                        if constexpr (ABS) a2 = f32x2_t{ fabsf(a2[0]), fabsf(a2[1]) };
                    } else {
                        a2 = f32x2_t{ __uint_as_float((q << 16) & HI), __uint_as_float(q & HI) };
                    }
                    if constexpr (DO_N) {
                        f32x2_t acc2 = { accN[j][2 * d], accN[j][2 * d + 1] };
                        acc2 = __builtin_elementwise_fma(a2, xs2, acc2);
                        accN[j][2 * d] = acc2[0]; accN[j][2 * d + 1] = acc2[1];
                    }
                    if constexpr (DO_T) {
                        const f32x2_t t2 = { xtv[j][2 * d], xtv[j][2 * d + 1] };
                        s2 = __builtin_elementwise_fma(a2, t2, s2);
                    }
                }
            p[u] = (s2[0] + s2[1]) * isv[u];
            if constexpr (DO_N) {
#pragma unroll
                for (int j = 0; j < NJ; ++j)
#pragma unroll
                    for (int k = 0; k < 8; ++k) asm volatile("" : "+v"(accN[j][k]));
            }
            asm volatile("" : "+v"(p[u]));
        }
        if constexpr (DO_T) {
            const float r = multi_reduce<K>(p, lane);
            constexpr int SH = 6 - Log2<K>::v;
            if ((lane & ((64 >> Log2<K>::v) - 1)) == 0) ldsT_wave[cc + (lane >> SH)] = r;
        }
        return;
    }
    float av[K][NJ][VW];
#pragma unroll
    for (int u = 0; u < K; ++u) {
        const E *col = A + (size_t)(c + u) * lda;
#pragma unroll
        for (int j = 0; j < NJ; ++j) {
            const int r = CLAMP ? rofs[j] : r_first + j * (BLK * VW);
            if constexpr (VW == 4) {
                if (FULL || r + 4 <= m) {
                    typedef float f32x4_t __attribute__((ext_vector_type(4)));
                    const f32x4_t *src = reinterpret_cast<const f32x4_t *>(col + r);
                    const f32x4_t q = NT ? __builtin_nontemporal_load(src) : *src;
                    av[u][j][0] = q[0]; av[u][j][1] = q[1]; av[u][j][2] = q[2]; av[u][j][3] = q[3];
                } else {
#pragma unroll
                    for (int k = 0; k < 4; ++k) av[u][j][k] = (r + k < m) ? elt_f32(col[r + k]) : 0.0f;
                }
            } else {
                av[u][j][0] = (FULL || r < m) ? elt_f32(col[r]) : 0.0f;
            }
        }
    }
    if constexpr (ABS) {
#pragma unroll
        for (int u = 0; u < K; ++u)
#pragma unroll
            for (int j = 0; j < NJ; ++j)
#pragma unroll
                for (int k = 0; k < VW; ++k) av[u][j][k] = fabsf(av[u][j][k]);
    }
    if constexpr (DO_N) {
#pragma unroll
        for (int u = 0; u < K; ++u) {
            const float xs = (ABS ? 1.0f : xn[c + u]) * (F16 ? inv_s[c + u] : 1.0f);
#pragma unroll
            for (int j = 0; j < NJ; ++j)
#pragma unroll
                for (int k = 0; k < VW; ++k) accN[j][k] = fmaf(av[u][j][k], xs, accN[j][k]);
        }
    }
    if constexpr (DO_T) {
        float p[K];
#pragma unroll
        for (int u = 0; u < K; ++u) {
            float s = 0.0f;
#pragma unroll
            for (int j = 0; j < NJ; ++j)
#pragma unroll
                for (int k = 0; k < VW; ++k) s = fmaf(av[u][j][k], xtv[j][k], s);
            p[u] = F16 ? s * inv_s[c + u] : s;
        }
        const float r = multi_reduce<K>(p, lane);
        constexpr int SH = 6 - Log2<K>::v;
        if ((lane & ((64 >> Log2<K>::v) - 1)) == 0) ldsT_wave[cc + (lane >> SH)] = r;
    }
}

template <typename E, int VW, int NJ, int KU, bool DO_N, bool DO_T, bool ABS, bool NT>
__global__ __launch_bounds__(BLK) void dual_gemv_k(const E *__restrict__ A, size_t lda, int m, int n,
                                                   const float *__restrict__ xn, const float *__restrict__ xt,
                                                   float *__restrict__ partN, size_t strideN,
                                                   float *__restrict__ partT, size_t strideT,
                                                   int cols_per_chunk, const int *__restrict__ stop,
                                                   const float *__restrict__ inv_s, int m_load)
{
    if (stop != nullptr && *stop != 0) return;
    __shared__ float ldsT[DO_T ? 4 * MAXCW : 4];

    constexpr int TILE = BLK * VW * NJ;
    const int tid = threadIdx.x, lane = tid & 63, wave = tid >> 6;
    const int tile = blockIdx.x, chunk = blockIdx.y;
    const int r_first = tile * TILE + tid * VW;
    const int c0 = chunk * cols_per_chunk;
    const int c1 = min(n, c0 + cols_per_chunk);

    float xtv[NJ][VW];
    float accN[NJ][VW];
#pragma unroll
    for (int j = 0; j < NJ; ++j)
#pragma unroll
        for (int k = 0; k < VW; ++k) {
            const int r = r_first + j * (BLK * VW) + k;
            accN[j][k] = 0.0f;
            xtv[j][k] = (DO_T && r < m) ? (ABS ? 1.0f : xt[r]) : 0.0f;
        }

    if constexpr (VW == 8 && DO_T) {
#pragma unroll
        for (int j = 0; j < NJ; ++j)
#pragma unroll
            for (int k = 0; k < VW; ++k) asm volatile("" : "+v"(xtv[j][k]));
    }

    float *ldsT_wave = ldsT + wave * (DO_T ? MAXCW : 1);
    int c = c0;
    int rofs[NJ];
#pragma unroll
    for (int j = 0; j < NJ; ++j) rofs[j] = 0;
    if ((tile + 1) * TILE <= m) {
        for (; c + KU <= c1; c += KU)
            step<E, VW, NJ, KU, DO_N, DO_T, ABS, NT, true>(A, lda, m, r_first, c, c - c0, xn, xtv, accN, ldsT_wave, lane, inv_s, rofs);
        for (; c < c1; ++c)
            step<E, VW, NJ, 1, DO_N, DO_T, ABS, NT, true>(A, lda, m, r_first, c, c - c0, xn, xtv, accN, ldsT_wave, lane, inv_s, rofs);
    } else if (VW > 1 && m_load > 0) {
#pragma unroll
        for (int j = 0; j < NJ; ++j) {
            const int r = r_first + j * (BLK * VW);
            rofs[j] = (r + VW <= m_load) ? r : tile * TILE;
        }
        for (; c + KU <= c1; c += KU)
            step<E, VW, NJ, KU, DO_N, DO_T, ABS, NT, true, true>(A, lda, m, r_first, c, c - c0, xn, xtv, accN, ldsT_wave, lane, inv_s, rofs);
        for (; c < c1; ++c)
            step<E, VW, NJ, 1, DO_N, DO_T, ABS, NT, true, true>(A, lda, m, r_first, c, c - c0, xn, xtv, accN, ldsT_wave, lane, inv_s, rofs);
    } else {
        for (; c + KU <= c1; c += KU)
            step<E, VW, NJ, KU, DO_N, DO_T, ABS, NT, false>(A, lda, m, r_first, c, c - c0, xn, xtv, accN, ldsT_wave, lane, inv_s, rofs);
        for (; c < c1; ++c)
            step<E, VW, NJ, 1, DO_N, DO_T, ABS, NT, false>(A, lda, m, r_first, c, c - c0, xn, xtv, accN, ldsT_wave, lane, inv_s, rofs);
    }

    if constexpr (DO_N) {
        float *dst = partN + (size_t)chunk * strideN;
#pragma unroll
        for (int j = 0; j < NJ; ++j) {
            const int r = r_first + j * (BLK * VW);
            if constexpr (VW >= 4) {
                if (r + VW <= m) {
#pragma unroll
                    for (int q = 0; q < VW; q += 4)
                        *reinterpret_cast<float4 *>(dst + r + q) =
                            make_float4(accN[j][q], accN[j][q + 1], accN[j][q + 2], accN[j][q + 3]);
                } else {
#pragma unroll
                    for (int k = 0; k < VW; ++k) if (r + k < m) dst[r + k] = accN[j][k];
                }
            } else {
                if (r < m) dst[r] = accN[j][0];
            }
        }
    }
    if constexpr (DO_T) {
        __syncthreads();
        float *dst = partT + (size_t)tile * strideT + c0;
        for (int t = tid; t < c1 - c0; t += BLK)
            dst[t] = (ldsT[t] + ldsT[MAXCW + t]) + (ldsT[2 * MAXCW + t] + ldsT[3 * MAXCW + t]);
    }
}

constexpr int GROWS = 128;
template <bool DO_N, bool DO_T>
__global__ __launch_bounds__(BLK) void grouped_gemv_k(const GroupDesc *__restrict__ tab)
{
    const GroupDesc d = tab[blockIdx.z];
    const int lane = threadIdx.x & 63, wave = threadIdx.x >> 6;
    const int tile = blockIdx.x, chunk = blockIdx.y * 4 + wave;
    __shared__ float ldsT[DO_T ? 4 * MAXCW : 4];
    if (tile * GROWS >= d.nr || chunk * d.cpc >= d.nc) return;
    const int r0 = tile * GROWS + lane, r1 = r0 + 64;
    const bool ok0 = r0 < d.nr, ok1 = r1 < d.nr;
    const int c0 = chunk * d.cpc, c1 = min(d.nc, c0 + d.cpc);
    const float *__restrict__ A = d.A;
    const size_t lda = (size_t)d.nr;
    float xt0 = 0.0f, xt1 = 0.0f, acc0 = 0.0f, acc1 = 0.0f;
    if constexpr (DO_T) { xt0 = ok0 ? d.xt[r0] : 0.0f; xt1 = ok1 ? d.xt[r1] : 0.0f; }
    float *lw = ldsT + wave * (DO_T ? MAXCW : 1);
    int c = c0;
    for (; c + 8 <= c1; c += 8) {
        float a0[8], a1[8];
#pragma unroll
        for (int u = 0; u < 8; ++u) {
            const float *col = A + (size_t)(c + u) * lda;
            a0[u] = ok0 ? __builtin_nontemporal_load(col + r0) : 0.0f;
            a1[u] = ok1 ? __builtin_nontemporal_load(col + r1) : 0.0f;
        }
        if constexpr (DO_N) {
#pragma unroll
            for (int u = 0; u < 8; ++u) { const float xs = d.xn[c + u]; acc0 = fmaf(a0[u], xs, acc0); acc1 = fmaf(a1[u], xs, acc1); }
        }
        if constexpr (DO_T) {
            float p[8];
#pragma unroll
            for (int u = 0; u < 8; ++u) p[u] = fmaf(a0[u], xt0, a1[u] * xt1);
            const float r = multi_reduce<8>(p, lane);
            if ((lane & 7) == 0) lw[c - c0 + (lane >> 3)] = r;
        }
    }
    for (; c < c1; ++c) {
        const float *col = A + (size_t)c * lda;
        const float a0 = ok0 ? col[r0] : 0.0f, a1 = ok1 ? col[r1] : 0.0f;
        if constexpr (DO_N) { const float xs = d.xn[c]; acc0 = fmaf(a0, xs, acc0); acc1 = fmaf(a1, xs, acc1); }
        if constexpr (DO_T) { const float r = wave_sum(fmaf(a0, xt0, a1 * xt1)); if (lane == 0) lw[c - c0] = r; }
    }
    if constexpr (DO_N) {
        float *dst = d.partN + (size_t)chunk * d.nr;
        if (ok0) dst[r0] = acc0;
        if (ok1) dst[r1] = acc1;
    }
    if constexpr (DO_T) {
        __builtin_amdgcn_s_waitcnt(0xc07f);
        __builtin_amdgcn_wave_barrier();
        float *dst = d.partT + (size_t)tile * d.nc + c0;
        for (int t = lane; t < c1 - c0; t += 64) dst[t] = lw[t];
    }
}

__global__ void finalize_k(size_t n, const float *__restrict__ part, int np, size_t stride, float alpha, float beta,
                           float *__restrict__ y, const int *__restrict__ stop)
{
    if (stop != nullptr && *stop != 0) return;
    for (size_t i = blockIdx.x * (size_t)BLK + threadIdx.x; i < n; i += (size_t)gridDim.x * BLK) {
        double sd = 0.0;
        for (int k = 0; k < np; ++k) sd += (double)part[(size_t)k * stride + i];
        const float s = (float)sd;
        y[i] = (beta == 0.0f) ? alpha * s : alpha * s + beta * y[i];
    }
}

__global__ void spmv_k(int n, float alpha, const float *__restrict__ sp, const float *__restrict__ x, float beta,
                       float *__restrict__ y)
{
    const int lane = threadIdx.x & 63;
    const int r = blockIdx.x * (BLK / 64) + (threadIdx.x >> 6);
    if (r >= n) return;
    float s = 0.0f;
    const size_t base = (size_t)r * (r + 1) / 2;
    for (int c = lane; c <= r; c += 64) s = fmaf(sp[base + c], x[c], s);
    for (int c = r + 1 + lane; c < n; c += 64) s = fmaf(sp[(size_t)c * (c + 1) / 2 + r], x[c], s);
    s = wave_sum(s);
    if (lane == 0) y[r] = (beta == 0.0f) ? alpha * s : alpha * s + beta * y[r];
}

__global__ void sp_absadd_k(int n, const float *__restrict__ sp, float *__restrict__ y)
{
    const int lane = threadIdx.x & 63;
    const int r = blockIdx.x * (BLK / 64) + (threadIdx.x >> 6);
    if (r >= n) return;
    float s = 0.0f;
    const size_t base = (size_t)r * (r + 1) / 2;
    for (int c = lane; c <= r; c += 64) s += fabsf(sp[base + c]);
    for (int c = r + 1 + lane; c < n; c += 64) s += fabsf(sp[(size_t)c * (c + 1) / 2 + r]);
    s = wave_sum(s);
    if (lane == 0) y[r] = y[r] + s;
}

struct Plan {
    int vw, nj, ku, nt;
    int tiles, chunks, cols_per_chunk;
    int m_load = 0;
    size_t strideN, strideT;
};

static size_t round_up(size_t v, size_t a) { return (v + a - 1) / a * a; }

static int env_int(const char *name, int dflt)
{
    const char *v = getenv(name);
    return v ? atoi(v) : dflt;
}

Plan make_plan(size_t n_row, size_t n_col, int vw, const GemvHint *hint = nullptr)
{
    const bool vec_ok = vw > 1;
    static const int env_nj = env_int("THIP_GEMV_NJ", 0);
    static const int env_blocks = env_int("THIP_GEMV_BLOCKS", 0);
    static const int env_nt = env_int("THIP_GEMV_NT", -1);
    Plan p;
    p.vw = vw;
    if (vec_ok) {
        p.nj = 1; p.ku = 8;
        int nj = env_nj;
        if (hint && hint->nj > 0) nj = hint->nj;
        if (nj == 1) { p.nj = 1; p.ku = 8; }
        if (nj == 2) { p.nj = 2; p.ku = 4; }
        if (nj == 4) { p.nj = 4; p.ku = 2; }
    } else {
        if (n_row >= (size_t)BLK * 4 * 4) { p.nj = 4; p.ku = 4; }
        else { p.nj = 1; p.ku = 8; }
    }
    p.nt = env_nt >= 0 ? env_nt : 1;
    const size_t tile = (size_t)BLK * p.vw * p.nj;
    p.tiles = (int)((n_row + tile - 1) / tile);
    int target_blocks = (int)((double)n_row * (double)n_col * (vw == 8 ? 2.0 : 4.0) / 2.0e5);
    if (target_blocks < 2048) target_blocks = 2048;
    if (target_blocks > 8192) target_blocks = 8192;
    if (env_blocks > 0) target_blocks = env_blocks;
    if (hint && hint->target_blocks > 0) target_blocks = hint->target_blocks;
    int chunks = target_blocks / p.tiles;
    if (chunks < 1) chunks = 1;
    int cpc = (int)((n_col + chunks - 1) / chunks);
    static const int env_mincpc = env_int("THIP_GEMV_MINCPC", 0);
    const int mincpc = env_mincpc > 0 ? env_mincpc : (((double)n_row * (double)n_col * 4.0 < 64.0e6) ? 16 : 32);
    if (cpc < mincpc) cpc = mincpc;
    if (cpc > MAXCW) cpc = MAXCW;
    cpc = (int)round_up(cpc, 8);
    if (cpc > MAXCW) cpc = MAXCW;
    p.cols_per_chunk = cpc;
    p.chunks = (int)((n_col + cpc - 1) / cpc);
    p.strideN = round_up(n_row, 4);
    p.strideT = round_up(n_col, 4);
    return p;
}

template <typename E, bool DO_N, bool DO_T, bool ABS>
void launch_cfg(const Plan &p, hipStream_t st, const E *A, size_t lda, int m, int n, const float *xn,
                const float *xt, float *partN, float *partT, const int *stop, const float *inv_s)
{
    dim3 g(p.tiles, p.chunks), b(BLK);
    constexpr int VV = sizeof(E) == 2 ? 8 : 4;
#define THIP_GEMV_LAUNCH(VW, NJ, KU)                                                                          \
    do {                                                                                                      \
        if (p.nt)                                                                                             \
            hipLaunchKernelGGL((dual_gemv_k<E, VW, NJ, KU, DO_N, DO_T, ABS, true>), g, b, 0, st, A, lda, m, n, xn, xt, \
                               partN, p.strideN, partT, p.strideT, p.cols_per_chunk, stop, inv_s, p.m_load);  \
        else                                                                                                  \
            hipLaunchKernelGGL((dual_gemv_k<E, VW, NJ, KU, DO_N, DO_T, ABS, false>), g, b, 0, st, A, lda, m, n, xn, xt, \
                               partN, p.strideN, partT, p.strideT, p.cols_per_chunk, stop, inv_s, p.m_load);  \
    } while (0)
    if (p.vw == VV) {
        if (p.nj == 4) THIP_GEMV_LAUNCH(VV, 4, 2);
        else if (p.nj == 2) THIP_GEMV_LAUNCH(VV, 2, 4);
        else THIP_GEMV_LAUNCH(VV, 1, 8);
    } else {
        if (p.nj == 4) THIP_GEMV_LAUNCH(1, 4, 4);
        else THIP_GEMV_LAUNCH(1, 1, 8);
    }
#undef THIP_GEMV_LAUNCH
}

template <typename E>
void launch_any(const Plan &p, hipStream_t st, const E *mat, size_t lda, int m, int n, const float *xn, const float *xt,
                bool do_n, bool do_t, bool abs_mode, float *partN, float *partT, const int *stop_flag,
                const float *inv_s = nullptr)
{
    if (abs_mode) {
        if (do_n && do_t) launch_cfg<E, true, true, true>(p, st, mat, lda, m, n, xn, xt, partN, partT, stop_flag, inv_s);
        else if (do_n)    launch_cfg<E, true, false, true>(p, st, mat, lda, m, n, xn, xt, partN, partT, stop_flag, inv_s);
        else              launch_cfg<E, false, true, true>(p, st, mat, lda, m, n, xn, xt, partN, partT, stop_flag, inv_s);
    } else {
        if (do_n && do_t) launch_cfg<E, true, true, false>(p, st, mat, lda, m, n, xn, xt, partN, partT, stop_flag, inv_s);
        else if (do_n)    launch_cfg<E, true, false, false>(p, st, mat, lda, m, n, xn, xt, partN, partT, stop_flag, inv_s);
        else              launch_cfg<E, false, true, false>(p, st, mat, lda, m, n, xn, xt, partN, partT, stop_flag, inv_s);
    }
}

__global__ void to_bf16_k(size_t n_row, size_t n_col, const float *__restrict__ src, bf16raw *__restrict__ dst, size_t ld16)
{
    const size_t total = ld16 * n_col;
    for (size_t i = blockIdx.x * (size_t)BLK + threadIdx.x; i < total; i += (size_t)gridDim.x * BLK) {
        const size_t c = i / ld16, r = i - c * ld16;
        unsigned out = 0;
        if (r < n_row) {
            const unsigned b = __float_as_uint(src[c * n_row + r]);
            if ((b & 0x7f800000u) == 0x7f800000u) out = (b >> 16) | ((b & 0xffffu) ? 0x40u : 0u);
            else out = (b + 0x7fffu + ((b >> 16) & 1u)) >> 16;
        }
        dst[i] = (bf16raw)out;
    }
}

__global__ __launch_bounds__(BLK) void f16_scale_k(size_t n_row, const float *__restrict__ src, float *__restrict__ inv_s)
{
    __shared__ float sh[16];
    const float *col = src + (size_t)blockIdx.x * n_row;
    float mx = 0.0f;
    for (size_t r = threadIdx.x; r < n_row; r += BLK) {
        const float v = fabsf(col[r]);
        if (v > mx && v <= 3.4028235e38f) mx = v;
    }
    mx = -block_min(-mx, sh);
    if (threadIdx.x == 0) {
        float inv = 1.0f;
        if (mx > 0.0f) {
            int e;
            (void)frexpf(mx, &e);
            inv = ldexpf(1.0f, e - 14);
        }
        inv_s[blockIdx.x] = inv;
    }
}

__global__ void to_f16_k(size_t n_row, size_t n_col, const float *__restrict__ src, const float *__restrict__ inv_s,
                         f16elt *__restrict__ dst, size_t ld16)
{
    const size_t total = ld16 * n_col;
    for (size_t i = blockIdx.x * (size_t)BLK + threadIdx.x; i < total; i += (size_t)gridDim.x * BLK) {
        const size_t c = i / ld16, r = i - c * ld16;
        dst[i] = (r < n_row) ? (f16elt)(src[c * n_row + r] / inv_s[c]) : (f16elt)0.0f;
    }
}

}

namespace thip {

const GemvHint *gemv_candidates(int *count)
{
    static const GemvHint c[] = { {1, 8192}, {1, 4096}, {2, 8192}, {2, 2048}, {4, 8192}, {4, 4096}, {4, 2048}, {4, 1024}, {4, 768} };
    *count = (int)(sizeof(c) / sizeof(c[0]));
    return c;
}

static void clamp_rows(Plan &p, size_t n_row, const DenseA &A)
{
    static const int clamp_on = getenv("THIP_GEMV_CLAMP") ? atoi(getenv("THIP_GEMV_CLAMP")) : 1;
    const size_t m_up = round_up(n_row, (size_t)p.vw);
    if (clamp_on && p.vw > 1 && (n_row % p.vw == 0 || (A.pad_zero && A.lda >= m_up))) p.m_load = (int)m_up;
}

size_t dual_gemv_scratch_floats(size_t n_row, size_t n_col)
{
    size_t best = 0;
    int nc = 0;
    const GemvHint *c = gemv_candidates(&nc);
    static const int vws[3] = { 4, 1, 8 };
    for (int i = -1; i < nc; ++i)
        for (int v = 0; v < 3; ++v) {
            const Plan p = make_plan(n_row, n_col, vws[v], i < 0 ? nullptr : &c[i]);
            const size_t f = (size_t)p.chunks * p.strideN + (size_t)p.tiles * p.strideT;
            if (f > best) best = f;
        }
    return best + 64;
}

int dual_gemv_partials_cols(hipStream_t st, size_t n_row, size_t n_col, const DenseA &A,
                            const float *xn, const float *xt, bool do_n, bool do_t, bool abs_mode,
                            float *scratch_base, size_t scratch_floats, GemvPartials *out, const int *stop_flag,
                            const GemvHint *hint, size_t col0, size_t col1, int chunk_row0, int max_chunk_rows,
                            int *chunks_used)
{
    if (chunks_used) *chunks_used = 0;
    *out = GemvPartials{};
    if (n_row == 0 || n_col == 0 || (!do_n && !do_t) || col1 <= col0) return 0;
    if (n_row > 0x7fffffffull || n_col > 0x7fffffffull || col1 > n_col)
        return fail(THIP_E_INVALID, "matrix dimension > 2^31, or bad column range", __FILE__, __LINE__);
    const size_t lda = A.lda; const float *inv_s = A.inv_s;
    const bool bf16 = A.kind == THIP_A_BF16, f16 = A.kind == THIP_A_F16;
    if (f16 && inv_s == nullptr) return fail(THIP_E_INVALID, "f16 storage needs the per-column scales", __FILE__, __LINE__);
    DenseA R = A;
    R.mat = (const char *)A.mat + col0 * lda * A.elem_bytes();
    const char *base = (const char *)R.mat;
    Plan p = make_plan(n_row, col1 - col0, A.vec_ok() ? R.vec_width() : 1, hint);
    p.strideN = round_up(n_row, 4);
    p.strideT = round_up(n_col, 4);
    clamp_rows(p, n_row, A);
    if (max_chunk_rows < 0) max_chunk_rows = chunk_row0 + p.chunks;
    if (chunk_row0 + p.chunks > max_chunk_rows) return fail(THIP_E_WORK, "gemv scratch: too many chunk rows", __FILE__, __LINE__);
    const size_t needN = do_n ? (size_t)max_chunk_rows * p.strideN : 0;
    const size_t needT = do_t ? (size_t)p.tiles * p.strideT : 0;
    if (needN + needT > scratch_floats) return fail(THIP_E_WORK, "gemv scratch too small", __FILE__, __LINE__);
    float *partN = scratch_base;
    float *partT = scratch_base + needN;
    out->partN = do_n ? partN : nullptr; out->nN = do_n ? chunk_row0 + p.chunks : 0; out->strideN = p.strideN;
    out->partT = do_t ? partT : nullptr; out->nT = do_t ? p.tiles : 0;  out->strideT = p.strideT;
    if (chunks_used) *chunks_used = p.chunks;
    const int m = (int)n_row, n = (int)(col1 - col0);
    float *pn = partN + (size_t)chunk_row0 * p.strideN;
    float *pt = partT + col0;
    const float *xnr = xn ? xn + col0 : nullptr;
    if (bf16) launch_any(p, st, (const bf16raw *)base, lda, m, n, xnr, xt, do_n, do_t, abs_mode, pn, pt, stop_flag);
    else if (f16) launch_any(p, st, (const f16elt *)base, lda, m, n, xnr, xt, do_n, do_t, abs_mode, pn, pt, stop_flag, inv_s + col0);
    else      launch_any(p, st, (const float *)base, lda, m, n, xnr, xt, do_n, do_t, abs_mode, pn, pt, stop_flag);
    THIP_LAUNCH_CHECK();
    return 0;
}

int dual_gemv_partials(hipStream_t st, size_t n_row, size_t n_col, const DenseA &A,
                       const float *xn, const float *xt, bool do_n, bool do_t, bool abs_mode,
                       float *scratch_base, size_t scratch_floats, GemvPartials *out, const int *stop_flag,
                       const GemvHint *hint)
{
    return dual_gemv_partials_cols(st, n_row, n_col, A, xn, xt, do_n, do_t, abs_mode, scratch_base, scratch_floats, out, stop_flag,
                                   hint, 0, n_col, 0, -1, nullptr);
}

int dual_gemv_chunk_rows(size_t n_row, size_t cols, const DenseA &A, const GemvHint *hint, int *tiles)
{
    const Plan p = make_plan(n_row, cols, A.vec_width(), hint);
    if (tiles) *tiles = p.tiles;
    return p.chunks;
}

int dual_gemv_partials_geometry(size_t n_row, size_t n_col, const DenseA &A, bool do_n, bool do_t,
                                float *scratch_base, GemvPartials *out)
{
    const Plan p = make_plan(n_row, n_col, A.vec_width(), nullptr);
    const size_t needN = do_n ? (size_t)p.chunks * p.strideN : 0;
    float *partN = scratch_base, *partT = scratch_base + needN;
    out->partN = do_n ? partN : nullptr; out->nN = do_n ? p.chunks : 0; out->strideN = p.strideN;
    out->partT = do_t ? partT : nullptr; out->nT = do_t ? p.tiles : 0;  out->strideT = p.strideT;
    return 0;
}

int grouped_gemv(hipStream_t st, const GroupDesc *dev_tab, int n_desc, int max_tiles, int max_chunks, int mode)
{
    if (n_desc <= 0) return 0;
    dim3 g(max_tiles, max_chunks, n_desc);
    if (mode == 2)      hipLaunchKernelGGL((grouped_gemv_k<true, true>), g, dim3(BLK), 0, st, dev_tab);
    else if (mode == 1) hipLaunchKernelGGL((grouped_gemv_k<false, true>), g, dim3(BLK), 0, st, dev_tab);
    else                hipLaunchKernelGGL((grouped_gemv_k<true, false>), g, dim3(BLK), 0, st, dev_tab);
    THIP_LAUNCH_CHECK();
    return 0;
}

int finalize_partials(hipStream_t st, size_t n, const float *part, int np, size_t stride, float alpha, float beta,
                      float *y, const int *stop)
{
    if (n == 0) return 0;
    hipLaunchKernelGGL(finalize_k, dim3(grid_for(n, BLK, 2048)), dim3(BLK), 0, st, n, part, np, stride, alpha, beta, y, stop);
    THIP_LAUNCH_CHECK();
    return 0;
}

int to_bf16(hipStream_t st, size_t n_row, size_t n_col, const float *src, uint16_t *dst, size_t ld16)
{
    if (ld16 < n_row) return fail(THIP_E_INVALID, "ld16 < n_row", __FILE__, __LINE__);
    if (ld16 * n_col == 0) return 0;
    hipLaunchKernelGGL(to_bf16_k, dim3(grid_for(ld16 * n_col, BLK, 16384)), dim3(BLK), 0, st, n_row, n_col, src, dst, ld16);
    THIP_LAUNCH_CHECK();
    return 0;
}

int to_f16(hipStream_t st, size_t n_row, size_t n_col, const float *src, uint16_t *dst, size_t ld16, float *inv_s)
{
    if (ld16 < n_row) return fail(THIP_E_INVALID, "ld16 < n_row", __FILE__, __LINE__);
    if (n_col == 0) return 0;
    hipLaunchKernelGGL(f16_scale_k, dim3((unsigned)n_col), dim3(BLK), 0, st, n_row, src, inv_s);
    hipLaunchKernelGGL(to_f16_k, dim3(grid_for(ld16 * n_col, BLK, 16384)), dim3(BLK), 0, st, n_row, n_col, src, inv_s,
                       reinterpret_cast<f16elt *>(dst), ld16);
    THIP_LAUNCH_CHECK();
    return 0;
}

int dual_gemv(hipStream_t st, size_t n_row, size_t n_col, const DenseA &A,
              const float *xn, float alphaN, float betaN, float *outN,
              const float *xt, float alphaT, float betaT, float *outT,
              bool abs_mode, const int *stop_flag)
{
    const bool do_n = outN != nullptr, do_t = outT != nullptr;
    float *scr = nullptr;
    const size_t need = dual_gemv_scratch_floats(n_row, n_col);
    THIP_RC(scratch(need, &scr));
    GemvPartials gp;
    THIP_RC(dual_gemv_partials(st, n_row, n_col, A, xn, xt, do_n, do_t, abs_mode, scr, need, &gp, stop_flag));
    if (do_n) THIP_RC(finalize_partials(st, n_row, gp.partN, gp.nN, gp.strideN, alphaN, betaN, outN, stop_flag));
    if (do_t) THIP_RC(finalize_partials(st, n_col, gp.partT, gp.nT, gp.strideT, alphaT, betaT, outT, stop_flag));
    return 0;
}

}

extern "C" {

int thip_transform_ge(int transpose, size_t n_row, size_t n_col, float alpha, const float *mat, const float *x,
                      float beta, float *y)
{
    THIP_NEED_INIT_NOFLUSH();
    const size_t ylen = transpose ? n_col : n_row;
    if (ylen == 0) return 0;
    if (n_row == 0 || n_col == 0) return thip_scale(ylen, beta, y);
    int deferred = 0;
    THIP_RC(lazy_push(transpose, n_row, n_col, alpha, mat, x, beta, y, &deferred));
    if (deferred) return 0;
    if (transpose)
        return dual_gemv(ctx().stream, n_row, n_col, dense_f32(mat, n_row), nullptr, 0.f, 0.f, nullptr, x, alpha, beta, y, false, nullptr);
    return dual_gemv(ctx().stream, n_row, n_col, dense_f32(mat, n_row), x, alpha, beta, y, nullptr, 0.f, 0.f, nullptr, false, nullptr);
}

int thip_to_bf16(size_t n_row, size_t n_col, const float *mat, uint16_t *mat16, size_t ld16)
{
    THIP_NEED_INIT();
    return to_bf16(ctx().stream, n_row, n_col, mat, mat16, ld16);
}

static int transform_ge16(int transpose, size_t n_row, size_t n_col, float alpha, const DenseA &A, const float *x, float beta, float *y)
{
    THIP_NEED_INIT();
    const size_t ylen = transpose ? n_col : n_row;
    if (ylen == 0) return 0;
    if (n_row == 0 || n_col == 0) return thip_scale(ylen, beta, y);
    if (A.lda < n_row) return fail(THIP_E_INVALID, "ld16 < n_row", __FILE__, __LINE__);
    if (transpose)
        return dual_gemv(ctx().stream, n_row, n_col, A, nullptr, 0.f, 0.f, nullptr, x, alpha, beta, y, false, nullptr);
    return dual_gemv(ctx().stream, n_row, n_col, A, x, alpha, beta, y, nullptr, 0.f, 0.f, nullptr, false, nullptr);
}

int thip_transform_ge_bf16(int transpose, size_t n_row, size_t n_col, float alpha, const uint16_t *mat16, size_t ld16,
                           const float *x, float beta, float *y)
{
    return transform_ge16(transpose, n_row, n_col, alpha, DenseA{ mat16, ld16, THIP_A_BF16, nullptr, false }, x, beta, y);
}

int thip_to_f16(size_t n_row, size_t n_col, const float *mat, uint16_t *mat16, size_t ld16, float *inv_scale)
{
    THIP_NEED_INIT();
    if (!inv_scale) return fail(THIP_E_INVALID, "inv_scale == NULL", __FILE__, __LINE__);
    return to_f16(ctx().stream, n_row, n_col, mat, mat16, ld16, inv_scale);
}

int thip_transform_ge_f16(int transpose, size_t n_row, size_t n_col, float alpha, const uint16_t *mat16, size_t ld16,
                          const float *inv_scale, const float *x, float beta, float *y)
{
    return transform_ge16(transpose, n_row, n_col, alpha, DenseA{ mat16, ld16, THIP_A_F16, inv_scale, false }, x, beta, y);
}

int thip_absadd_cols(size_t n_row, size_t n_col, const float *mat, float *tau)
{
    THIP_NEED_INIT();
    if (n_row == 0 || n_col == 0) return 0;
    return dual_gemv(ctx().stream, n_row, n_col, dense_f32(mat, n_row), nullptr, 0.f, 0.f, nullptr, nullptr, 1.0f, 1.0f, tau, true, nullptr);
}

int thip_absadd_rows(size_t n_row, size_t n_col, const float *mat, float *sigma)
{
    THIP_NEED_INIT();
    if (n_row == 0 || n_col == 0) return 0;
    return dual_gemv(ctx().stream, n_row, n_col, dense_f32(mat, n_row), nullptr, 1.0f, 1.0f, sigma, nullptr, 0.f, 0.f, nullptr, true, nullptr);
}

int thip_transform_sp(size_t n, float alpha, const float *mat, const float *x, float beta, float *y)
{
    THIP_NEED_INIT();
    if (n == 0) return 0;
    hipLaunchKernelGGL(spmv_k, dim3((unsigned)((n + 3) / 4)), dim3(BLK), 0, ctx().stream, (int)n, alpha, mat, x, beta, y);
    THIP_LAUNCH_CHECK();
    return 0;
}

int thip_absadd_sympack(size_t n, const float *mat, float *y)
{
    THIP_NEED_INIT();
    if (n == 0) return 0;
    hipLaunchKernelGGL(sp_absadd_k, dim3((unsigned)((n + 3) / 4)), dim3(BLK), 0, ctx().stream, (int)n, mat, y);
    THIP_LAUNCH_CHECK();
    return 0;
}

}
```

### totsu_amd/csrc/thip_lazy.hip

```cpp
#include "thip_common.h"

#include <algorithm>
#include <atomic>
#include <cstdio>
#include <cstdlib>
#include <cstring>
#include <mutex>
#include <unordered_map>
#include <vector>

using namespace thip;

namespace {

constexpr int BLK = 256;
constexpr size_t LAZY_MAX_ELEMS = (size_t)16 << 20;
constexpr size_t LAZY_MAX_VEC = 1024;
constexpr size_t LAZY_MAX_OPS = 32768;
constexpr int SHORT_LEN = 2048;
constexpr int MAX_PLANS = 64;

enum { K_N = 0, K_T = 1, K_AXPY = 2, K_DOT = 3, K_ADDV = 4, K_SCALE = 5, K_CONST = 6 };
enum { OP_GE = 0, OP_SCALE = 1, OP_ADD = 2, OP_PROJ = 3, OP_SET = 4 };

struct Call {
    uint8_t op, transpose, bclass, pkind;
    int grp, mem;
    float alpha, beta;
    size_t nr, nc;
    const float *A, *x;
    float *y;
};
bool same_shape(const Call &a, const Call &b)
{
    return a.op == b.op && a.transpose == b.transpose && a.bclass == b.bclass && a.pkind == b.pkind && a.nr == b.nr
           && a.nc == b.nc && a.A == b.A && a.x == b.x && a.y == b.y;
}
uint8_t beta_class(float b) { return b == 0.0f ? 0 : (b == 1.0f ? 1 : 2); }

struct Member {
    int kind; size_t nr, nc, inlen;
    float alpha;
    const float *A, *x;
    int call;
};
struct Group {
    float *y; size_t len; float beta;
    std::vector<Member> mem;
};

struct DotD { const float *v, *x; float *out; int len; int pad; };
enum { M_PART = 0, M_AXPY = 1, M_ADDV = 2, M_CONST = 3 };
struct FinMember { const float *src; const float *xs; int count; int type; size_t stride; };
struct FinGroup { float *y; int len; int first, count; };
struct BigMat { const float *A, *xn, *xt; size_t nr, nc; size_t scr_off, scr_floats; };

struct Plan {
    int type = 0;
    std::vector<Call> calls;
    uint64_t key = 0;
    bool replayable = true;
    unsigned generation = 0;
    char *dev = nullptr; size_t dev_bytes = 0;
    int nN = 0, nT = 0, nD = 0, nDot = 0, nLong = 0, nShort = 0, maxlen = 0;
    int long_members = 0;
    int maxt[3] = { 0, 0, 0 }, maxc[3] = { 0, 0, 0 };
    size_t off_dot = 0, off_grp = 0, off_mem = 0, off_alpha = 0, off_beta = 0;
    size_t n_members = 0, n_groups = 0;
    std::vector<float> alphas, betas;
    std::vector<int> mem_slot, grp_slot;
    std::vector<BigMat> big;
    int pkind = 0; float *base = nullptr; size_t ncones = 0, max_len = 0;
    Plan *next = nullptr;
    uint64_t last_use = 0;
};

enum { RD_GET = 0, RD_NORM = 1 };
struct ReadReq { int kind; const float *p; size_t n; };
struct ReadD { const float *p; unsigned n; int kind; };
struct ReadPlan {
    std::vector<ReadReq> reqs;
    std::vector<uintptr_t> suf_lo, suf_hi;
    char *dev = nullptr;
    uint64_t last_use = 0;
};

struct Queue {
    std::vector<ReadReq> rd_learn; bool rd_open = false;
    std::vector<ReadPlan *> rd_plans;
    ReadPlan *rd_cur = nullptr; size_t rd_pos = 0;
    std::vector<float> rd_vals;
    float *rd_pin = nullptr; size_t rd_pin_n = 0;
    long long rd_served = 0, rd_fetches = 0;
    std::vector<Group> groups;
    std::unordered_map<const float *, int> target;
    size_t n_members = 0;
    uintptr_t xlo = ~(uintptr_t)0, xhi = 0, ylo = ~(uintptr_t)0, yhi = 0;
    std::vector<Call> calls;
    bool seg_replayable = true;
    int proj_kind = -1;
    uintptr_t plo = ~(uintptr_t)0, phi = 0;
    Plan *pred = nullptr;
    size_t pos = 0;
    bool replaying = false;
    std::vector<float> cur_alpha, cur_beta;
    Plan *last_plan = nullptr;
    std::vector<Plan *> plans;
    uint64_t tick = 0;
    std::mutex mu;
    bool enabled = false, env_read = false;
    float *part = nullptr; size_t part_floats = 0; unsigned generation = 1;
    char *tab = nullptr; size_t tab_bytes = 0, tab_used = 0;
    char *pin[2] = { nullptr, nullptr }; size_t pin_bytes[2] = { 0, 0 }; hipEvent_t pin_ev[2] = { nullptr, nullptr };
    int pin_next = 0;
    long long flushes = 0, deferred = 0, hits = 0, misses = 0;
    std::atomic<bool> pending{ false };
} Q;

bool overlap(uintptr_t a0, uintptr_t a1, uintptr_t b0, uintptr_t b1) { return a0 < b1 && b0 < a1; }

bool tracing()
{
    static const int on = getenv("THIP_LAZY_TRACE") ? atoi(getenv("THIP_LAZY_TRACE")) : 0;
    return on != 0;
}
const char *g_why = "entry point";

constexpr int DBLK = 1024;
__global__ __launch_bounds__(DBLK) void dot_k(const DotD *__restrict__ tab)
{
    __shared__ double shd[16];
    const DotD d = tab[blockIdx.x];
    double s0 = 0.0, s1 = 0.0, s2 = 0.0, s3 = 0.0;
    int i = threadIdx.x;
    for (; i + 3 * DBLK < d.len; i += 4 * DBLK) {
        const float a0 = d.v[i], a1 = d.v[i + DBLK], a2 = d.v[i + 2 * DBLK], a3 = d.v[i + 3 * DBLK];
        const float b0 = d.x[i], b1 = d.x[i + DBLK], b2 = d.x[i + 2 * DBLK], b3 = d.x[i + 3 * DBLK];
        s0 += (double)a0 * (double)b0; s1 += (double)a1 * (double)b1; s2 += (double)a2 * (double)b2; s3 += (double)a3 * (double)b3;
    }
    for (; i < d.len; i += DBLK) s0 += (double)d.v[i] * (double)d.x[i];
    const double s = block_sum_d((s0 + s1) + (s2 + s3), shd);
    if (threadIdx.x == 0) d.out[0] = (float)s;
}

__device__ __forceinline__ double one_member(const FinMember &m, float al, int c)
{
    if (m.type == M_PART) {
        double s0 = 0.0, s1 = 0.0, s2 = 0.0, s3 = 0.0;
        const float *p = m.src + c;
        int t = 0;
        for (; t + 16 <= m.count; t += 16) {
            float a[16];
#pragma unroll
            for (int u = 0; u < 16; ++u) a[u] = p[(size_t)(t + u) * m.stride];
#pragma unroll
            for (int u = 0; u < 16; u += 4) { s0 += (double)a[u]; s1 += (double)a[u + 1]; s2 += (double)a[u + 2]; s3 += (double)a[u + 3]; }
        }
        for (; t + 4 <= m.count; t += 4) {
            const float a0 = p[(size_t)t * m.stride], a1 = p[(size_t)(t + 1) * m.stride];
            const float a2 = p[(size_t)(t + 2) * m.stride], a3 = p[(size_t)(t + 3) * m.stride];
            s0 += (double)a0; s1 += (double)a1; s2 += (double)a2; s3 += (double)a3;
        }
        for (; t < m.count; ++t) s0 += (double)p[(size_t)t * m.stride];
        return (double)al * ((s0 + s1) + (s2 + s3));
    }
    if (m.type == M_AXPY) return (double)(al * m.xs[0] * m.src[c]);
    if (m.type == M_CONST) return (double)al;
    return (double)(al * m.src[c]);
}

__device__ __forceinline__ double contributions(const FinGroup &g, const FinMember *__restrict__ mem,
                                                const float *__restrict__ alphas, int c, int k0, int kstep)
{
    constexpr int U = 8;
    double acc = 0.0;
    int k = k0;
    for (; k + (U - 1) * kstep < g.count; k += U * kstep) {
        FinMember m[U];
        float al[U];
        bool simple = true;
#pragma unroll
        for (int u = 0; u < U; ++u) {
            m[u] = mem[g.first + k + u * kstep];
            al[u] = alphas[g.first + k + u * kstep];
            simple = simple && (m[u].type == M_ADDV || (m[u].type == M_PART && m[u].count == 1) || m[u].type == M_AXPY);
        }
        if (simple) {
            float v[U], x0[U];
#pragma unroll
            for (int u = 0; u < U; ++u) { v[u] = m[u].src[c]; x0[u] = m[u].type == M_AXPY ? m[u].xs[0] : 1.0f; }
#pragma unroll
            for (int u = 0; u < U; ++u)
                acc += m[u].type == M_PART ? (double)al[u] * (double)v[u] : (double)(al[u] * x0[u] * v[u]);
        } else {
#pragma unroll
            for (int u = 0; u < U; ++u) acc += one_member(m[u], al[u], c);
        }
    }
    for (; k < g.count; k += kstep) acc += one_member(mem[g.first + k], alphas[g.first + k], c);
    return acc;
}

template <int E>
__device__ __forceinline__ void contributions_multi(const FinGroup &g, const FinMember *__restrict__ mem,
                                                    const float *__restrict__ alphas, int c0, int k0, int kstep, double *acc)
{
    constexpr int U = 8;
    int k = k0;
    for (; k + (U - 1) * kstep < g.count; k += U * kstep) {
        FinMember m[U];
        float al[U];
        bool simple = true;
#pragma unroll
        for (int u = 0; u < U; ++u) {
            m[u] = mem[g.first + k + u * kstep];
            al[u] = alphas[g.first + k + u * kstep];
            simple = simple && (m[u].type == M_ADDV || (m[u].type == M_PART && m[u].count == 1) || m[u].type == M_AXPY);
        }
        if (simple) {
            float v[U][E], x0[U];
#pragma unroll
            for (int u = 0; u < U; ++u) {
                x0[u] = m[u].type == M_AXPY ? m[u].xs[0] : 1.0f;
#pragma unroll
                for (int i = 0; i < E; ++i) v[u][i] = c0 + 64 * i < g.len ? m[u].src[c0 + 64 * i] : 0.0f;
            }
#pragma unroll
            for (int u = 0; u < U; ++u)
#pragma unroll
                for (int i = 0; i < E; ++i)
                    acc[i] += m[u].type == M_PART ? (double)al[u] * (double)v[u][i] : (double)(al[u] * x0[u] * v[u][i]);
        } else {
#pragma unroll
            for (int u = 0; u < U; ++u)
#pragma unroll
                for (int i = 0; i < E; ++i)
                    if (c0 + 64 * i < g.len) acc[i] += one_member(m[u], al[u], c0 + 64 * i);
        }
    }
    for (; k < g.count; k += kstep) {
        const FinMember m = mem[g.first + k];
        const float al = alphas[g.first + k];
#pragma unroll
        for (int i = 0; i < E; ++i)
            if (c0 + 64 * i < g.len) acc[i] += one_member(m, al, c0 + 64 * i);
    }
}

template <bool LONG, int FIN_LONG_LANES, int FIN_E = 1>
__global__ __launch_bounds__(LONG ? 64 * FIN_LONG_LANES : BLK) void fin_k(const FinGroup *__restrict__ groups, const FinMember *__restrict__ mem,
                                             const float *__restrict__ alphas, const float *__restrict__ betas)
{
    const int gi = LONG ? blockIdx.y : blockIdx.x;
    const FinGroup g = groups[gi];
    const float beta = betas[gi];
    if (LONG) {
        constexpr int E = FIN_E;
        __shared__ double comb[FIN_LONG_LANES - 1][E][64];
        const int e = threadIdx.x & 63, kq = threadIdx.x >> 6;
        const int c0 = blockIdx.x * (64 * E) + e;
        double a[E];
#pragma unroll
        for (int i = 0; i < E; ++i) a[i] = 0.0;
        if (c0 < g.len) contributions_multi<E>(g, mem, alphas, c0, kq, FIN_LONG_LANES, a);
        if (kq > 0) {
#pragma unroll
            for (int i = 0; i < E; ++i) comb[kq - 1][i][e] = a[i];
        }
        __syncthreads();
        if (kq == 0) {
#pragma unroll
            for (int i = 0; i < E; ++i) {
                const int c = c0 + 64 * i;
                if (c < g.len) {
                    double sacc = a[i];
#pragma unroll
                    for (int q = 0; q < FIN_LONG_LANES - 1; ++q) sacc += comb[q][i][e];
                    const float v = (float)sacc;
                    g.y[c] = beta == 0.0f ? v : fmaf(beta, g.y[c], v);
                }
            }
        }
    } else if (g.len <= 4 && g.count > 32) {
        __shared__ double shd[16];
        for (int c = 0; c < g.len; ++c) {
            const double a = block_sum_d(contributions(g, mem, alphas, c, threadIdx.x, BLK), shd);
            if (threadIdx.x == 0) { const float v = (float)a; g.y[c] = beta == 0.0f ? v : fmaf(beta, g.y[c], v); }
            __syncthreads();
        }
    } else {
        for (int c = threadIdx.x; c < g.len; c += BLK) {
            const float a = (float)contributions(g, mem, alphas, c, 0, 1);
            g.y[c] = beta == 0.0f ? a : fmaf(beta, g.y[c], a);
        }
    }
}

__global__ __launch_bounds__(BLK) void ewise_table_k(float *__restrict__ base, const int64_t *__restrict__ begs,
                                                     const int64_t *__restrict__ ends, int zero)
{
    const int64_t b = begs[blockIdx.x], e = ends[blockIdx.x];
    for (int64_t i = b + (int64_t)blockIdx.y * BLK + threadIdx.x; i < e; i += (int64_t)gridDim.y * BLK)
        base[i] = zero ? 0.0f : fmaxf(base[i], 0.0f);
}

__global__ __launch_bounds__(BLK) void read_batch_k(const ReadD *__restrict__ tab, float *__restrict__ out)
{
    __shared__ double shd[16];
    const ReadD d = tab[blockIdx.x];
    if (d.kind == RD_GET) { if (threadIdx.x == 0) out[blockIdx.x] = d.p[0]; return; }
    double acc = 0.0;
    for (unsigned i = threadIdx.x; i < d.n; i += BLK) { const double t = (double)d.p[i]; acc += t * t; }
    acc = block_sum_d(acc, shd);
    if (threadIdx.x == 0) out[blockIdx.x] = (float)sqrt(acc);
}

size_t up256(size_t v) { return (v + 255) / 256 * 256; }

void free_plan(Plan *p) { delete p; }

void drop_all_plans()
{
    for (Plan *p : Q.plans) free_plan(p);
    Q.plans.clear();
    Q.pred = Q.last_plan = nullptr;
    Q.replaying = false; Q.pos = 0;
    Q.tab_used = 0;
}

int alloc_tab(size_t bytes, char **out)
{
    bytes = (bytes + 255) / 256 * 256;
    if (Q.tab_used + bytes > Q.tab_bytes || (int)Q.plans.size() >= MAX_PLANS) {
        THIP_TRY(hipStreamSynchronize(ctx().stream));
        drop_all_plans();
        if (bytes > Q.tab_bytes) {
            if (Q.tab) { THIP_TRY(hipFree(Q.tab)); Q.tab = nullptr; Q.tab_bytes = 0; }
            const size_t want = std::max<size_t>((size_t)8 << 20, 2 * bytes);
            THIP_TRY(hipMalloc((void **)&Q.tab, want));
            Q.tab_bytes = want;
        }
    }
    *out = Q.tab + Q.tab_used;
    Q.tab_used += bytes;
    return 0;
}

int ensure_part(size_t floats)
{
    if (floats <= Q.part_floats) return 0;
    THIP_TRY(hipStreamSynchronize(ctx().stream));
    if (Q.part) { THIP_TRY(hipFree(Q.part)); Q.part = nullptr; Q.part_floats = 0; }
    const size_t want = floats + floats / 4 + (1 << 18);
    THIP_TRY(hipMalloc((void **)&Q.part, want * sizeof(float)));
    Q.part_floats = want;
    Q.generation += 1;
    return 0;
}

int staging(size_t bytes, char **out, int *half_out)
{
    const int half = Q.pin_next;
    Q.pin_next ^= 1;
    if (Q.pin_ev[half] == nullptr) THIP_TRY(hipEventCreateWithFlags(&Q.pin_ev[half], hipEventDisableTiming));
    else THIP_TRY(hipEventSynchronize(Q.pin_ev[half]));
    if (Q.pin_bytes[half] < bytes) {
        if (Q.pin[half]) THIP_TRY(hipHostFree(Q.pin[half]));
        Q.pin[half] = nullptr; Q.pin_bytes[half] = 0;
        const size_t want = bytes + bytes / 4 + 4096;
        THIP_TRY(hipHostMalloc((void **)&Q.pin[half], want, hipHostMallocDefault));
        Q.pin_bytes[half] = want;
    }
    *out = Q.pin[half];
    *half_out = half;
    return 0;
}

void reset_segment()
{
    Q.groups.clear(); Q.target.clear(); Q.n_members = 0;
    Q.xlo = Q.ylo = ~(uintptr_t)0; Q.xhi = Q.yhi = 0;
    Q.calls.clear();
    Q.seg_replayable = true;
    Q.proj_kind = -1; Q.plo = ~(uintptr_t)0; Q.phi = 0;
}

void update_pending()
{
    Q.pending.store(!Q.calls.empty() || (Q.replaying && Q.pos > 0) || Q.rd_cur != nullptr || Q.rd_open, std::memory_order_relaxed);
}

uint64_t mix(uint64_t h, uint64_t v)
{
    h ^= v + 0x9E3779B97F4A7C15ull + (h << 6) + (h >> 2);
    return h * 0xBF58476D1CE4E5B9ull;
}
uint64_t key_of(const std::vector<Call> &calls)
{
    uint64_t h = 0x94D049BB133111EBull ^ calls.size();
    for (const Call &c : calls) {
        h = mix(h, (uint64_t)c.op | ((uint64_t)c.transpose << 8) | ((uint64_t)c.bclass << 16) | ((uint64_t)c.pkind << 24));
        h = mix(h, c.nr); h = mix(h, c.nc);
        h = mix(h, (uint64_t)(uintptr_t)c.A); h = mix(h, (uint64_t)(uintptr_t)c.x); h = mix(h, (uint64_t)(uintptr_t)c.y);
    }
    return h;
}


int launch_plan(Plan *p)
{
    hipStream_t st = ctx().stream;
    Q.flushes += 1;
    p->last_use = ++Q.tick;
    if (p->type == 1) {
        const int64_t *begs = reinterpret_cast<const int64_t *>(p->dev), *ends = begs + p->ncones;
        if (p->pkind == THIP_CONE_SOC || p->pkind == THIP_CONE_ROTSOC)
            THIP_RC(soc_batched(st, p->base, begs, ends, p->ncones, p->pkind == THIP_CONE_ROTSOC, p->max_len, nullptr));
        else {
            const unsigned gy = (unsigned)std::min<size_t>(64, (p->max_len + BLK - 1) / BLK);
            hipLaunchKernelGGL(ewise_table_k, dim3((unsigned)p->ncones, gy ? gy : 1), dim3(BLK), 0, st, p->base, begs, ends,
                               p->pkind == THIP_CONE_ZERO ? 1 : 0);
            THIP_LAUNCH_CHECK();
        }
        return 0;
    }
    const GroupDesc *dgd = reinterpret_cast<const GroupDesc *>(p->dev);
    THIP_RC(grouped_gemv(st, dgd, p->nD, p->maxt[2], (p->maxc[2] + 3) / 4, 2));
    THIP_RC(grouped_gemv(st, dgd + p->nD, p->nN, p->maxt[0], (p->maxc[0] + 3) / 4, 0));
    THIP_RC(grouped_gemv(st, dgd + p->nD + p->nN, p->nT, p->maxt[1], (p->maxc[1] + 3) / 4, 1));
    for (const BigMat &b : p->big) {
        GemvPartials gp;
        THIP_RC(dual_gemv_partials(st, b.nr, b.nc, dense_f32(b.A, b.nr), b.xn, b.xt, b.xn != nullptr, b.xt != nullptr, false,
                                   Q.part + b.scr_off, b.scr_floats, &gp, nullptr));
    }
    if (p->nDot) hipLaunchKernelGGL(dot_k, dim3(p->nDot), dim3(DBLK), 0, st, reinterpret_cast<const DotD *>(p->dev + p->off_dot));
    const FinGroup *dg = reinterpret_cast<const FinGroup *>(p->dev + p->off_grp);
    const FinMember *dm = reinterpret_cast<const FinMember *>(p->dev + p->off_mem);
    const float *da = reinterpret_cast<const float *>(p->dev + p->off_alpha);
    const float *db = reinterpret_cast<const float *>(p->dev + p->off_beta);
    if (p->nLong && p->long_members < 256)
        hipLaunchKernelGGL((fin_k<true, 4, 1>), dim3((p->maxlen + 63) / 64, (unsigned)p->nLong), dim3(256), 0, st, dg, dm, da, db);
    else if (p->nLong)
        hipLaunchKernelGGL((fin_k<true, 16, 4>), dim3((p->maxlen + 255) / 256, (unsigned)p->nLong), dim3(1024), 0, st, dg, dm, da, db);
    if (p->nShort) hipLaunchKernelGGL((fin_k<false, 4>), dim3((unsigned)p->nShort), dim3(BLK), 0, st, dg + p->nLong, dm, da, db + p->nLong);
    THIP_LAUNCH_CHECK();
    return 0;
}

int upload_factors(Plan *p, const std::vector<float> &alphas, const std::vector<float> &betas)
{
    const bool da = alphas != p->alphas, db = betas != p->betas;
    if (!da && !db) return 0;
    hipStream_t st = ctx().stream;
    const size_t ba = up256(alphas.size() * sizeof(float)), bb = up256(betas.size() * sizeof(float));
    char *host; int half;
    THIP_RC(staging(ba + bb, &host, &half));
    if (da) {
        memcpy(host, alphas.data(), alphas.size() * sizeof(float));
        THIP_TRY(hipMemcpyAsync(p->dev + p->off_alpha, host, alphas.size() * sizeof(float), hipMemcpyHostToDevice, st));
        p->alphas = alphas;
    }
    if (db) {
        memcpy(host + ba, betas.data(), betas.size() * sizeof(float));
        THIP_TRY(hipMemcpyAsync(p->dev + p->off_beta, host + ba, betas.size() * sizeof(float), hipMemcpyHostToDevice, st));
        p->betas = betas;
    }
    THIP_TRY(hipEventRecord(Q.pin_ev[half], st));
    return 0;
}

void factors_from_calls(const Plan *p, const float *alpha, const float *beta, std::vector<float> &alphas, std::vector<float> &betas)
{
    alphas.assign(p->n_members, 0.0f);
    betas.assign(p->n_groups, 1.0f);
    for (size_t i = 0; i < p->calls.size(); ++i) {
        const Call &c = p->calls[i];
        const int gs = p->grp_slot[c.grp];
        if (c.op != OP_ADD && c.bclass != 1) betas[gs] = c.bclass == 0 ? 0.0f : betas[gs] * beta[i];
        if (c.mem >= 0 && p->mem_slot[i] >= 0) alphas[p->mem_slot[i]] = alpha[i];
    }
}

void plan_done(Plan *p)
{
    if (Q.last_plan && Q.last_plan != p) Q.last_plan->next = p;
    Q.last_plan = p;
    Q.pred = p->next;
    Q.pos = 0;
    Q.replaying = Q.pred != nullptr;
}

void remember(Plan *p) { Q.plans.push_back(p); }

Plan *find_plan(uint64_t key, const std::vector<Call> &calls, int type)
{
    for (Plan *p : Q.plans) {
        if (p->key != key || p->type != type || p->calls.size() != calls.size() || p->generation != Q.generation) continue;
        bool same = true;
        for (size_t i = 0; i < calls.size() && same; ++i) same = same_shape(p->calls[i], calls[i]);
        if (same) return p;
    }
    return nullptr;
}


int flush_projections()
{
    std::vector<Call> calls;
    calls.swap(Q.calls);
    const int kind = Q.proj_kind;
    reset_segment();
    update_pending();
    const uint64_t key = key_of(calls);
    Plan *p = find_plan(key, calls, 1);
    if (p) { Q.hits += 1; }
    else {
        Q.misses += 1;
        p = new Plan();
        p->type = 1; p->key = key; p->pkind = kind; p->ncones = calls.size(); p->generation = Q.generation;
        uintptr_t lo = ~(uintptr_t)0;
        for (const Call &c : calls) { lo = std::min(lo, (uintptr_t)c.y); p->max_len = std::max(p->max_len, c.nr); }
        p->base = reinterpret_cast<float *>(lo);
        const size_t bytes = up256(2 * calls.size() * sizeof(int64_t));
        hipStream_t st = ctx().stream;
        char *host; int half;
        int rc = staging(bytes, &host, &half);
        if (rc == 0) rc = alloc_tab(bytes, &p->dev);
        if (rc != 0) { delete p; return rc; }
        p->dev_bytes = bytes;
        int64_t *begs = reinterpret_cast<int64_t *>(host), *ends = begs + calls.size();
        for (size_t i = 0; i < calls.size(); ++i) {
            begs[i] = (int64_t)(((uintptr_t)calls[i].y - lo) / sizeof(float));
            ends[i] = begs[i] + (int64_t)calls[i].nr;
        }
        THIP_TRY(hipMemcpyAsync(p->dev, host, 2 * calls.size() * sizeof(int64_t), hipMemcpyHostToDevice, st));
        THIP_TRY(hipEventRecord(Q.pin_ev[half], st));
        p->calls.swap(calls);
        remember(p);
    }
    THIP_RC(launch_plan(p));
    plan_done(p);
    return 0;
}

int flush_products()
{
    hipStream_t st = ctx().stream;
    std::vector<Group> groups;
    groups.swap(Q.groups);
    std::vector<Call> calls;
    calls.swap(Q.calls);
    const size_t n_members = Q.n_members;
    const bool replayable = Q.seg_replayable;
    reset_segment();
    update_pending();

    std::vector<int> order;
    order.reserve(groups.size());
    for (size_t i = 0; i < groups.size(); ++i) if ((int)groups[i].len > SHORT_LEN) order.push_back((int)i);
    const int nLong = (int)order.size();
    for (size_t i = 0; i < groups.size(); ++i) if ((int)groups[i].len <= SHORT_LEN) order.push_back((int)i);
    std::vector<float> alphas, betas;
    alphas.reserve(n_members); betas.reserve(groups.size());
    for (int gi : order) { betas.push_back(groups[gi].beta); for (const Member &m : groups[gi].mem) alphas.push_back(m.alpha); }

    const uint64_t key = key_of(calls);
    Plan *p = find_plan(key, calls, 0);
    if (p) {
        Q.hits += 1;
        THIP_RC(upload_factors(p, alphas, betas));
        THIP_RC(launch_plan(p));
        plan_done(p);
        return 0;
    }
    Q.misses += 1;
    p = new Plan();
    p->type = 0; p->key = key; p->replayable = replayable;
    p->n_members = n_members; p->n_groups = groups.size();
    p->nLong = nLong; p->nShort = (int)groups.size() - nLong;

    struct MatRef { int g, m; };
    std::unordered_map<const float *, std::vector<MatRef>> byA;
    for (size_t gi = 0; gi < groups.size(); ++gi)
        for (size_t mi = 0; mi < groups[gi].mem.size(); ++mi) {
            const Member &m = groups[gi].mem[mi];
            if (m.kind == K_N || m.kind == K_T) byA[m.A].push_back(MatRef{ (int)gi, (int)mi });
        }
    std::vector<std::vector<MatRef>> partner(groups.size());
    for (size_t gi = 0; gi < groups.size(); ++gi) partner[gi].assign(groups[gi].mem.size(), MatRef{ -1, -1 });
    for (auto &kv : byA) {
        std::vector<MatRef> ns, ts;
        for (const MatRef &r : kv.second) (groups[r.g].mem[r.m].kind == K_N ? ns : ts).push_back(r);
        const size_t np = std::min(ns.size(), ts.size());
        for (size_t k = 0; k < np; ++k) {
            const Member &a = groups[ns[k].g].mem[ns[k].m], &b = groups[ts[k].g].mem[ts[k].m];
            if (a.nr != b.nr || a.nc != b.nc) continue;
            partner[ns[k].g][ns[k].m] = ts[k];
            partner[ts[k].g][ts[k].m] = ns[k];
        }
    }

    struct MatPlan { size_t offN, offT; int cpc, tiles, chunks; int big; };
    std::vector<std::vector<MatPlan>> mp(groups.size());
    for (size_t gi = 0; gi < groups.size(); ++gi) mp[gi].assign(groups[gi].mem.size(), MatPlan{ 0, 0, 0, 0, 0, -1 });
    size_t floats = 0;
    int nDot = 0;
    for (size_t gi = 0; gi < groups.size(); ++gi)
        for (size_t mi = 0; mi < groups[gi].mem.size(); ++mi) {
            const Member &m = groups[gi].mem[mi];
            if (m.kind == K_DOT) { nDot += 1; continue; }
            if (m.kind != K_N && m.kind != K_T) continue;
            const MatRef pr = partner[gi][mi];
            const bool paired = pr.g >= 0;
            if (paired && m.kind == K_T) continue;
            const Member *tm = paired ? &groups[pr.g].mem[pr.m] : nullptr;
            const bool doN = m.kind == K_N, doT = m.kind == K_T || paired;
            MatPlan q{ 0, 0, 0, 0, 0, -1 };
            if (m.nr * m.nc > LAZY_MAX_ELEMS) {
                BigMat b{ m.A, doN ? m.x : nullptr, m.kind == K_T ? m.x : (tm ? tm->x : nullptr), m.nr, m.nc, floats,
                          dual_gemv_scratch_floats(m.nr, m.nc) };
                q.big = (int)p->big.size();
                p->big.push_back(b);
                floats += b.scr_floats; floats = (floats + 63) / 64 * 64;
            } else {
                static const size_t wave_elems = getenv("THIP_LAZY_WAVE_ELEMS") ? (size_t)atol(getenv("THIP_LAZY_WAVE_ELEMS")) : 40000;
                size_t c = wave_elems / (m.nr < 128 ? m.nr : 128);
                c = std::max<size_t>(8, std::min<size_t>(1024, c / 8 * 8));
                q.cpc = (int)c; q.tiles = (int)((m.nr + 127) / 128); q.chunks = (int)((m.nc + c - 1) / c);
                if (doN) { q.offN = floats; floats += (size_t)q.chunks * m.nr; floats = (floats + 63) / 64 * 64; }
                if (doT) { q.offT = floats; floats += (size_t)q.tiles * m.nc; floats = (floats + 63) / 64 * 64; }
            }
            mp[gi][mi] = q;
            if (paired) mp[pr.g][pr.m] = q;
        }
    const size_t dot_off = floats;
    floats += (size_t)nDot;
    int rc = ensure_part(floats);
    if (rc != 0) { delete p; return rc; }
    p->generation = Q.generation;
    float *dpart = Q.part;
    std::vector<GemvPartials> biggp(p->big.size());
    for (size_t k = 0; k < p->big.size(); ++k) {
        const BigMat &b = p->big[k];
        dual_gemv_partials_geometry(b.nr, b.nc, dense_f32(b.A, b.nr), b.xn != nullptr, b.xt != nullptr, dpart + b.scr_off, &biggp[k]);
    }

    int nN = 0, nT = 0, nD = 0;
    for (size_t gi = 0; gi < groups.size(); ++gi)
        for (size_t mi = 0; mi < groups[gi].mem.size(); ++mi) {
            const Member &m = groups[gi].mem[mi];
            if ((m.kind != K_N && m.kind != K_T) || mp[gi][mi].big >= 0) continue;
            if (partner[gi][mi].g >= 0) { if (m.kind == K_N) nD += 1; }
            else if (m.kind == K_N) nN += 1; else nT += 1;
        }
    p->nN = nN; p->nT = nT; p->nD = nD; p->nDot = nDot;
    const size_t b_gd = up256((size_t)(nN + nT + nD) * sizeof(GroupDesc));
    const size_t b_dot = up256((size_t)nDot * sizeof(DotD));
    const size_t b_grp = up256(groups.size() * sizeof(FinGroup));
    const size_t b_mem = up256(n_members * sizeof(FinMember));
    const size_t b_al = up256(n_members * sizeof(float)), b_be = up256(groups.size() * sizeof(float));
    p->off_dot = b_gd; p->off_grp = b_gd + b_dot; p->off_mem = p->off_grp + b_grp; p->off_alpha = p->off_mem + b_mem;
    p->off_beta = p->off_alpha + b_al;
    const size_t b_tab = p->off_beta + b_be;
    char *host; int half;
    rc = staging(b_tab, &host, &half);
    if (rc == 0) rc = alloc_tab(b_tab, &p->dev);
    if (rc != 0) { delete p; return rc; }
    p->dev_bytes = b_tab;
    memset(host, 0, b_tab);
    GroupDesc *gdD = reinterpret_cast<GroupDesc *>(host), *gdN = gdD + nD, *gdT = gdN + nN;
    DotD *dd = reinterpret_cast<DotD *>(host + p->off_dot);
    FinGroup *hg = reinterpret_cast<FinGroup *>(host + p->off_grp);
    FinMember *hm = reinterpret_cast<FinMember *>(host + p->off_mem);
    p->mem_slot.assign(calls.size(), -1);
    p->grp_slot.assign(groups.size(), -1);
    int iD = 0, iN = 0, iT = 0, iDot = 0;
    size_t mpos = 0;
    for (size_t oi = 0; oi < order.size(); ++oi) {
        const int gi = order[oi];
        const Group &g = groups[gi];
        p->grp_slot[gi] = (int)oi;
        if ((int)g.len > SHORT_LEN) { p->maxlen = std::max(p->maxlen, (int)g.len); p->long_members = std::max(p->long_members, (int)g.mem.size()); }
        hg[oi] = FinGroup{ g.y, (int)g.len, (int)mpos, (int)g.mem.size() };
        for (size_t mi = 0; mi < g.mem.size(); ++mi) {
            const Member &m = g.mem[mi];
            FinMember fm{ nullptr, nullptr, 0, M_ADDV, 0 };
            if (m.kind == K_N || m.kind == K_T) {
                const MatPlan &q = mp[gi][mi];
                const MatRef pr = partner[gi][mi];
                fm.type = M_PART;
                if (q.big >= 0) {
                    const GemvPartials &gp = biggp[q.big];
                    if (m.kind == K_N) { fm.src = gp.partN; fm.count = gp.nN; fm.stride = gp.strideN; }
                    else               { fm.src = gp.partT; fm.count = gp.nT; fm.stride = gp.strideT; }
                } else if (m.kind == K_N) {
                    GroupDesc gd{ m.A, m.x, nullptr, dpart + q.offN, nullptr, (int)m.nr, (int)m.nc, q.cpc, 0 };
                    if (pr.g >= 0) {
                        gd.xt = groups[pr.g].mem[pr.m].x; gd.partT = dpart + q.offT;
                        gdD[iD++] = gd; p->maxt[2] = std::max(p->maxt[2], q.tiles); p->maxc[2] = std::max(p->maxc[2], q.chunks);
                    } else { gdN[iN++] = gd; p->maxt[0] = std::max(p->maxt[0], q.tiles); p->maxc[0] = std::max(p->maxc[0], q.chunks); }
                    fm.src = dpart + q.offN; fm.count = q.chunks; fm.stride = m.nr;
                } else {
                    if (pr.g < 0) {
                        GroupDesc gd{ m.A, nullptr, m.x, nullptr, dpart + q.offT, (int)m.nr, (int)m.nc, q.cpc, 0 };
                        gdT[iT++] = gd; p->maxt[1] = std::max(p->maxt[1], q.tiles); p->maxc[1] = std::max(p->maxc[1], q.chunks);
                    }
                    fm.src = dpart + q.offT; fm.count = q.tiles; fm.stride = m.nc;
                }
            } else if (m.kind == K_DOT) {
                dd[iDot] = DotD{ m.A, m.x, dpart + dot_off + iDot, (int)m.inlen, 0 };
                fm.src = dpart + dot_off + iDot; fm.type = M_ADDV;
                ++iDot;
            } else if (m.kind == K_AXPY) { fm.src = m.A; fm.xs = m.x; fm.type = M_AXPY; }
            else if (m.kind == K_CONST) { fm.type = M_CONST; }
            else { fm.src = m.x; fm.type = M_ADDV; }
            if (m.call >= 0 && (size_t)m.call < calls.size()) p->mem_slot[m.call] = (int)mpos;
            hm[mpos++] = fm;
        }
    }
    memcpy(host + p->off_alpha, alphas.data(), alphas.size() * sizeof(float));
    memcpy(host + p->off_beta, betas.data(), betas.size() * sizeof(float));
    THIP_TRY(hipMemcpyAsync(p->dev, host, b_tab, hipMemcpyHostToDevice, st));
    THIP_TRY(hipEventRecord(Q.pin_ev[half], st));
    p->alphas = alphas; p->betas = betas;
    p->calls.swap(calls);
    if (tracing()) fprintf(stderr, "lazy: new product plan of %zu calls: dual %d, N %d, T %d, big %zu, dots %d, replayable %d\n",
                           p->calls.size(), p->nD, p->nN, p->nT, p->big.size(), p->nDot, (int)p->replayable);
    remember(p);
    THIP_RC(launch_plan(p));
    plan_done(p);
    return 0;
}

int flush_segment()
{
    if (Q.calls.empty()) return 0;
    if (tracing()) fprintf(stderr, "lazy: flush %s segment of %zu calls (%zu groups, %zu members): %s\n",
                           Q.proj_kind >= 0 ? "projection" : "product", Q.calls.size(), Q.groups.size(), Q.n_members, g_why);
    g_why = "entry point";
    return Q.proj_kind >= 0 ? flush_projections() : flush_products();
}

int push_products(float *y, size_t len, float beta, Member m, Call c, int *deferred)
{
    if (Q.proj_kind >= 0) { g_why = "a product follows projections"; THIP_RC(flush_segment()); }
    const bool has_in = m.kind != K_SCALE && m.kind != K_CONST;
    const uintptr_t y0 = (uintptr_t)y, y1 = y0 + len * sizeof(float);
    const uintptr_t x0 = (uintptr_t)m.x, x1 = has_in ? x0 + m.inlen * sizeof(float) : x0;
    const bool has_a = m.kind == K_N || m.kind == K_T || m.kind == K_AXPY || m.kind == K_DOT;
    const uintptr_t a0 = (uintptr_t)m.A, a1 = has_a ? a0 + m.nr * m.nc * sizeof(float) : a0;
    bool must_flush = Q.n_members + Q.groups.size() >= LAZY_MAX_OPS;
    int join = -1;
    if (!must_flush && !Q.groups.empty()) {
        const bool raw = (has_in && overlap(x0, x1, Q.ylo, Q.yhi)) || (has_a && overlap(a0, a1, Q.ylo, Q.yhi));
        const bool war = overlap(y0, y1, Q.xlo, Q.xhi);
        const bool waw = overlap(y0, y1, Q.ylo, Q.yhi);
        if (waw) {
            auto it = Q.target.find(y);
            if (it != Q.target.end() && Q.groups[it->second].len == len) join = it->second;
        }
        if (raw || war || (waw && join < 0)) {
            for (size_t gi = 0; gi < Q.groups.size() && !must_flush; ++gi) {
                const Group &g = Q.groups[gi];
                const uintptr_t py0 = (uintptr_t)g.y, py1 = py0 + g.len * sizeof(float);
                if ((has_in && overlap(x0, x1, py0, py1)) || (has_a && overlap(a0, a1, py0, py1))) { must_flush = true; break; }
                if ((int)gi != join && overlap(y0, y1, py0, py1)) { must_flush = true; break; }
                if (war)
                    for (const Member &p : g.mem) {
                        if (p.kind == K_CONST) continue;
                        const uintptr_t px0 = (uintptr_t)p.x, px1 = px0 + p.inlen * sizeof(float);
                        if (overlap(y0, y1, px0, px1)) { must_flush = true; break; }
                        if (p.kind != K_ADDV) {
                            const uintptr_t pa0 = (uintptr_t)p.A, pa1 = pa0 + p.nr * p.nc * sizeof(float);
                            if (overlap(y0, y1, pa0, pa1)) { must_flush = true; break; }
                        }
                    }
            }
        }
    }
    if (must_flush) { g_why = "hazard / full (products)"; THIP_RC(flush_segment()); join = -1; }
    if (join < 0) {
        Q.target[y] = (int)Q.groups.size();
        Q.groups.push_back(Group{ y, len, 1.0f, {} });
        join = (int)Q.groups.size() - 1;
        Q.ylo = std::min(Q.ylo, y0); Q.yhi = std::max(Q.yhi, y1);
    }
    Group &g = Q.groups[join];
    if (beta != 1.0f) {
        if (!g.mem.empty()) Q.seg_replayable = false;
        if (beta == 0.0f) {
            Q.n_members -= g.mem.size();
            for (Member &pm : g.mem) Q.calls[pm.call].mem = -1;
            g.mem.clear(); g.beta = 0.0f;
        } else { g.beta *= beta; for (Member &p : g.mem) p.alpha *= beta; }
    }
    c.grp = join; c.mem = -1;
    if (m.kind != K_SCALE) {
        m.call = (int)Q.calls.size();
        c.mem = m.call;
        g.mem.push_back(m);
        Q.n_members += 1;
        if (has_in) { Q.xlo = std::min(Q.xlo, x0); Q.xhi = std::max(Q.xhi, x1); }
        if (has_a) { Q.xlo = std::min(Q.xlo, a0); Q.xhi = std::max(Q.xhi, a1); }
    }
    Q.calls.push_back(c);
    Q.deferred += 1;
    *deferred = 1;
    update_pending();
    return 0;
}

int push_projection(const Call &c, int *deferred)
{
    if (Q.proj_kind < 0 && !Q.calls.empty()) { g_why = "a projection follows products"; THIP_RC(flush_segment()); }
    const uintptr_t p0 = (uintptr_t)c.y, p1 = p0 + c.nr * sizeof(float);
    if (Q.proj_kind >= 0) {
        bool clash = Q.proj_kind != (int)c.pkind || Q.calls.size() >= LAZY_MAX_OPS;
        if (!clash && overlap(p0, p1, Q.plo, Q.phi))
            for (const Call &q : Q.calls) {
                const uintptr_t q0 = (uintptr_t)q.y;
                if (overlap(p0, p1, q0, q0 + q.nr * sizeof(float))) { clash = true; break; }
            }
        if (clash) { g_why = "projection kind / overlap"; THIP_RC(flush_segment()); }
    }
    Q.proj_kind = (int)c.pkind;
    Q.plo = std::min(Q.plo, p0); Q.phi = std::max(Q.phi, p1);
    Q.calls.push_back(c);
    Q.deferred += 1;
    *deferred = 1;
    update_pending();
    return 0;
}

int push_slow(const Call &c, int *deferred)
{
    if (c.op == OP_PROJ) return push_projection(c, deferred);
    Member m{};
    size_t outlen = c.nr;
    float beta = 1.0f;
    if (c.op == OP_GE) {
        m.nr = c.nr; m.nc = c.nc; m.alpha = c.alpha; m.A = c.A; m.x = c.x;
        const bool tr = c.transpose != 0;
        if (c.nc == 1)      { m.kind = tr ? K_DOT : K_AXPY; m.inlen = tr ? c.nr : 1; outlen = tr ? 1 : c.nr; }
        else if (c.nr == 1) { m.kind = tr ? K_AXPY : K_DOT; m.inlen = tr ? 1 : c.nc; outlen = tr ? c.nc : 1; }
        else                { m.kind = tr ? K_T : K_N; m.inlen = tr ? c.nr : c.nc; outlen = tr ? c.nc : c.nr; }
        beta = c.beta;
    } else if (c.op == OP_SCALE) { m.kind = K_SCALE; beta = c.beta; }
    else if (c.op == OP_SET) { m.kind = K_CONST; m.alpha = c.alpha; beta = 0.0f; outlen = 1; }
    else { m.kind = K_ADDV; m.alpha = c.alpha; m.x = c.x; m.inlen = c.nr; m.nr = m.nc = 0; }
    return push_products(c.y, outlen, beta, m, c, deferred);
}

int abandon_replay()
{
    const size_t n = Q.pos;
    if (tracing()) fprintf(stderr, "lazy: prediction of %zu calls abandoned after %zu\n", Q.pred->calls.size(), n);
    const std::vector<Call> matched(Q.pred->calls.begin(), Q.pred->calls.begin() + n);
    Q.replaying = false; Q.pred = nullptr; Q.pos = 0;
    for (size_t i = 0; i < n; ++i) {
        Call c = matched[i];
        c.alpha = Q.cur_alpha[i]; c.beta = Q.cur_beta[i];
        int d = 0;
        Q.deferred -= 1;
        THIP_RC(push_slow(c, &d));
    }
    update_pending();
    return 0;
}

int finish_replay()
{
    Plan *p = Q.pred;
    if (p->type == 0) {
        std::vector<float> alphas, betas;
        factors_from_calls(p, Q.cur_alpha.data(), Q.cur_beta.data(), alphas, betas);
        THIP_RC(upload_factors(p, alphas, betas));
    }
    Q.hits += 1;
    Q.pos = 0;
    if (tracing()) fprintf(stderr, "lazy: replayed %s plan of %zu calls (dual %d, N %d, T %d, big %zu)\n",
                           p->type ? "projection" : "product", p->calls.size(), p->nD, p->nN, p->nT, p->big.size());
    THIP_RC(launch_plan(p));
    plan_done(p);
    update_pending();
    return 0;
}


void drop_read_cache() { Q.rd_cur = nullptr; Q.rd_pos = 0; }

void free_read_plan(ReadPlan *p) { if (p->dev) hipFree(p->dev); delete p; }

void close_read_group()
{
    if (!Q.rd_open) return;
    Q.rd_open = false;
    if (Q.rd_learn.size() < 16 || Q.rd_learn.size() > 65536) { Q.rd_learn.clear(); return; }
    for (size_t i = 0; i < Q.rd_plans.size(); ++i) {
        const ReadReq &f = Q.rd_plans[i]->reqs[0];
        if (f.kind == Q.rd_learn[0].kind && f.p == Q.rd_learn[0].p && f.n == Q.rd_learn[0].n) {
            hipStreamSynchronize(ctx().stream);
            free_read_plan(Q.rd_plans[i]);
            Q.rd_plans.erase(Q.rd_plans.begin() + i);
            break;
        }
    }
    if (Q.rd_plans.size() >= 4) {
        size_t v = 0;
        for (size_t i = 1; i < Q.rd_plans.size(); ++i) if (Q.rd_plans[i]->last_use < Q.rd_plans[v]->last_use) v = i;
        hipStreamSynchronize(ctx().stream);
        free_read_plan(Q.rd_plans[v]);
        Q.rd_plans.erase(Q.rd_plans.begin() + v);
    }
    ReadPlan *p = new ReadPlan();
    p->reqs.swap(Q.rd_learn);
    const size_t n = p->reqs.size();
    p->suf_lo.assign(n + 1, ~(uintptr_t)0); p->suf_hi.assign(n + 1, 0);
    for (size_t i = n; i-- > 0;) {
        const uintptr_t a = (uintptr_t)p->reqs[i].p, b = a + p->reqs[i].n * sizeof(float);
        p->suf_lo[i] = std::min(p->suf_lo[i + 1], a); p->suf_hi[i] = std::max(p->suf_hi[i + 1], b);
    }
    const size_t b_tab = up256(n * sizeof(ReadD)), b_out = up256(n * sizeof(float));
    if (hipMalloc((void **)&p->dev, b_tab + b_out) != hipSuccess) { (void)hipGetLastError(); delete p; return; }
    std::vector<ReadD> tab(n);
    for (size_t i = 0; i < n; ++i) tab[i] = ReadD{ p->reqs[i].p, (unsigned)p->reqs[i].n, p->reqs[i].kind };
    if (hipMemcpy(p->dev, tab.data(), n * sizeof(ReadD), hipMemcpyHostToDevice) != hipSuccess) { free_read_plan(p); return; }
    Q.rd_plans.push_back(p);
}

int flush_work();

void reads_vs_write(uintptr_t w0, uintptr_t w1)
{
    if (Q.rd_cur == nullptr) return;
    const ReadPlan *p = Q.rd_cur;
    if (!overlap(w0, w1, p->suf_lo[Q.rd_pos], p->suf_hi[Q.rd_pos])) return;
    for (size_t i = Q.rd_pos; i < p->reqs.size(); ++i) {
        const uintptr_t a = (uintptr_t)p->reqs[i].p;
        if (overlap(w0, w1, a, a + p->reqs[i].n * sizeof(float))) { drop_read_cache(); return; }
    }
}

int read_request(int kind, const float *p, size_t n, float *value, int *served)
{
    *served = 0;
    if (Q.rd_cur) {
        const ReadPlan *pl = Q.rd_cur;
        const ReadReq &r = pl->reqs[Q.rd_pos];
        if (r.kind == kind && r.p == p && r.n == n) {
            *value = Q.rd_vals[Q.rd_pos];
            Q.rd_pos += 1; Q.rd_served += 1;
            if (Q.rd_pos == pl->reqs.size()) drop_read_cache();
            *served = 1;
            update_pending();
            return 0;
        }
        drop_read_cache();
    }
    ReadPlan *pl = nullptr;
    if (!Q.rd_open)
        for (ReadPlan *q : Q.rd_plans) if (q->reqs[0].kind == kind && q->reqs[0].p == p && q->reqs[0].n == n) { pl = q; break; }
    THIP_RC(flush_work());
    if (pl) {
        hipStream_t st = ctx().stream;
        const size_t nr = pl->reqs.size();
        if (Q.rd_pin_n < nr) {
            if (Q.rd_pin) THIP_TRY(hipHostFree(Q.rd_pin));
            Q.rd_pin = nullptr; Q.rd_pin_n = 0;
            THIP_TRY(hipHostMalloc((void **)&Q.rd_pin, (nr + 1024) * sizeof(float), hipHostMallocDefault));
            Q.rd_pin_n = nr + 1024;
        }
        float *dout = reinterpret_cast<float *>(pl->dev + up256(nr * sizeof(ReadD)));
        hipLaunchKernelGGL(read_batch_k, dim3((unsigned)nr), dim3(BLK), 0, st, reinterpret_cast<const ReadD *>(pl->dev), dout);
        THIP_LAUNCH_CHECK();
        THIP_TRY(hipMemcpyAsync(Q.rd_pin, dout, nr * sizeof(float), hipMemcpyDeviceToHost, st));
        THIP_TRY(hipStreamSynchronize(st));
        Q.rd_vals.assign(Q.rd_pin, Q.rd_pin + nr);
        pl->last_use = ++Q.tick;
        Q.rd_fetches += 1; Q.rd_served += 1;
        Q.rd_cur = pl; Q.rd_pos = 1;
        if (nr == 1) drop_read_cache();
        *value = Q.rd_vals[0];
        *served = 1;
        update_pending();
        return 0;
    }
    if (!Q.rd_open) { Q.rd_learn.clear(); Q.rd_open = true; }
    Q.rd_learn.push_back(ReadReq{ kind, p, n });
    update_pending();
    return 0;
}

uintptr_t write_len(const Call &c)
{
    if (c.op == OP_GE) return (c.transpose ? c.nc : c.nr) * sizeof(float);
    if (c.op == OP_SET) return sizeof(float);
    return c.nr * sizeof(float);
}

int push_call(const Call &c, int *deferred)
{
    *deferred = 0;
    if (Q.rd_cur) reads_vs_write((uintptr_t)c.y, (uintptr_t)c.y + write_len(c));
    for (int guard = 0; guard < 4 && Q.replaying; ++guard) {
        Plan *p = Q.pred;
        if (p->generation != Q.generation || !p->replayable) { THIP_RC(abandon_replay()); break; }
        if (Q.pos == p->calls.size()) { THIP_RC(finish_replay()); continue; }
        if (same_shape(c, p->calls[Q.pos])) {
            if (Q.cur_alpha.size() < p->calls.size()) { Q.cur_alpha.resize(p->calls.size()); Q.cur_beta.resize(p->calls.size()); }
            Q.cur_alpha[Q.pos] = c.alpha; Q.cur_beta[Q.pos] = c.beta;
            Q.pos += 1;
            Q.deferred += 1;
            *deferred = 1;
            Q.pending.store(true, std::memory_order_relaxed);
            return 0;
        }
        THIP_RC(abandon_replay());
        break;
    }
    if (Q.replaying) THIP_RC(abandon_replay());
    return push_slow(c, deferred);
}

int flush_locked()
{
    drop_read_cache();
    close_read_group();
    THIP_RC(flush_work());
    update_pending();
    return 0;
}

int flush_work()
{
    if (Q.replaying && Q.pos > 0) {
        if (Q.pos == Q.pred->calls.size() && Q.pred->generation == Q.generation) return finish_replay();
        THIP_RC(abandon_replay());
    }
    THIP_RC(flush_segment());
    update_pending();
    return 0;
}

bool lazy_on()
{
    if (!Q.env_read) {
        const char *e = getenv("THIP_LAZY_GEMV");
        if (e) Q.enabled = atoi(e) != 0;
        Q.env_read = true;
    }
    return Q.enabled && ctx().stream == ctx().own_stream;
}

}

namespace thip {

bool lazy_pending() { return Q.pending.load(std::memory_order_relaxed); }

int lazy_flush()
{
    std::lock_guard<std::mutex> lock(Q.mu);
    return flush_locked();
}

void lazy_forget(uintptr_t lo, uintptr_t hi)
{
    std::lock_guard<std::mutex> lock(Q.mu);
    if (Q.rd_plans.empty() && !Q.rd_open && Q.rd_learn.empty() && Q.plans.empty()) return;
    auto in = [&](const void *p) { const uintptr_t a = (uintptr_t)p; return p != nullptr && a >= lo && a < hi; };
    bool hit = false;
    for (const Plan *p : Q.plans) {
        if (in(p->base)) hit = true;
        for (const Call &c : p->calls) if (in(c.A) || in(c.x) || in(c.y)) { hit = true; break; }
        if (hit) break;
    }
    if (hit) drop_all_plans();
    bool rd_hit = false;
    for (const ReadReq &r : Q.rd_learn) if (overlap((uintptr_t)r.p, (uintptr_t)(r.p + (r.n ? r.n : 1)), lo, hi)) rd_hit = true;
    if (rd_hit) { Q.rd_open = false; Q.rd_learn.clear(); }
    for (size_t i = 0; i < Q.rd_plans.size();) {
        ReadPlan *p = Q.rd_plans[i];
        const bool meets = !p->suf_lo.empty() && overlap(p->suf_lo[0], p->suf_hi[0], lo, hi);
        if (meets) {
            if (Q.rd_cur == p) drop_read_cache();
            free_read_plan(p);
            Q.rd_plans.erase(Q.rd_plans.begin() + i);
        } else ++i;
    }
}

void lazy_release()
{
    std::lock_guard<std::mutex> lock(Q.mu);
    reset_segment();
    drop_all_plans();
    drop_read_cache();
    Q.rd_open = false; Q.rd_learn.clear();
    for (ReadPlan *p : Q.rd_plans) free_read_plan(p);
    Q.rd_plans.clear();
    if (Q.rd_pin) { hipHostFree(Q.rd_pin); Q.rd_pin = nullptr; Q.rd_pin_n = 0; }
    Q.pending.store(false, std::memory_order_relaxed);
    if (Q.part) { hipFree(Q.part); Q.part = nullptr; Q.part_floats = 0; Q.generation += 1; }
    if (Q.tab) { hipFree(Q.tab); Q.tab = nullptr; Q.tab_bytes = 0; Q.tab_used = 0; }
    for (int k = 0; k < 2; ++k) {
        if (Q.pin[k]) { hipHostFree(Q.pin[k]); Q.pin[k] = nullptr; Q.pin_bytes[k] = 0; }
        if (Q.pin_ev[k]) { hipEventDestroy(Q.pin_ev[k]); Q.pin_ev[k] = nullptr; }
    }
}

int lazy_push(int transpose, size_t n_row, size_t n_col, float alpha, const float *mat, const float *x, float beta,
              float *y, int *deferred)
{
    std::lock_guard<std::mutex> lock(Q.mu);
    *deferred = 0;
    if (!lazy_on() || n_row > 0x7fffffffull || n_col > 0x7fffffffull) return flush_locked();
    Call c{};
    c.op = OP_GE; c.transpose = transpose ? 1 : 0; c.bclass = beta_class(beta); c.alpha = alpha; c.beta = beta;
    c.nr = n_row; c.nc = n_col; c.A = mat; c.x = x; c.y = y;
    return push_call(c, deferred);
}

int lazy_push_scale(size_t n, float alpha, float *x, int *deferred)
{
    std::lock_guard<std::mutex> lock(Q.mu);
    *deferred = 0;
    if (alpha == 1.0f) { *deferred = 1; return 0; }
    if (!lazy_on() || n > LAZY_MAX_VEC || n == 0) return flush_locked();
    Call c{};
    c.op = OP_SCALE; c.bclass = beta_class(alpha); c.beta = alpha; c.nr = n; c.y = x;
    return push_call(c, deferred);
}

int lazy_push_add(size_t n, float alpha, const float *x, float *y, int *deferred)
{
    std::lock_guard<std::mutex> lock(Q.mu);
    *deferred = 0;
    if (!lazy_on() || n > LAZY_MAX_VEC || n == 0) return flush_locked();
    Call c{};
    c.op = OP_ADD; c.bclass = 1; c.alpha = alpha; c.beta = 1.0f; c.nr = n; c.x = x; c.y = y;
    return push_call(c, deferred);
}

int lazy_push_set(float *x, float value, int *deferred)
{
    std::lock_guard<std::mutex> lock(Q.mu);
    *deferred = 0;
    if (!lazy_on()) return flush_locked();
    Call c{};
    c.op = OP_SET; c.bclass = 0; c.alpha = value; c.beta = 0.0f; c.nr = 1; c.y = x;
    return push_call(c, deferred);
}

int lazy_read(int is_norm, const float *p, size_t n, float *value, int *served)
{
    std::lock_guard<std::mutex> lock(Q.mu);
    *served = 0;
    if (!lazy_on() || n == 0 || n > 0xffffffffull) return flush_locked();
    return read_request(is_norm ? RD_NORM : RD_GET, p, n, value, served);
}

int lazy_push_proj(int kind, size_t n, float *x, int *deferred)
{
    std::lock_guard<std::mutex> lock(Q.mu);
    *deferred = 0;
    if (!lazy_on() || n == 0 || n > 0x7fffffffull) return flush_locked();
    Call c{};
    c.op = OP_PROJ; c.pkind = (uint8_t)kind; c.bclass = 1; c.nr = n; c.y = x;
    return push_call(c, deferred);
}

}

extern "C" {

int thip_set_lazy_gemv(int on)
{
    THIP_NEED_INIT();
    std::lock_guard<std::mutex> lock(Q.mu);
    Q.enabled = on != 0;
    Q.env_read = true;
    return 0;
}

int thip_get_lazy_gemv(int *host_on)
{
    if (!host_on) return fail(THIP_E_INVALID, "null argument", __FILE__, __LINE__);
    std::lock_guard<std::mutex> lock(Q.mu);
    (void)lazy_on();
    *host_on = Q.enabled ? 1 : 0;
    return 0;
}

int thip_lazy_gemv_stats(int64_t *host_deferred, int64_t *host_flushes)
{
    if (host_deferred) *host_deferred = Q.deferred;
    if (host_flushes) *host_flushes = Q.flushes;
    return 0;
}

int thip_lazy_read_stats(int64_t *host_served, int64_t *host_fetches)
{
    if (host_served) *host_served = Q.rd_served;
    if (host_fetches) *host_fetches = Q.rd_fetches;
    return 0;
}

int thip_lazy_plan_stats(int64_t *host_hits, int64_t *host_misses)
{
    if (host_hits) *host_hits = Q.hits;
    if (host_misses) *host_misses = Q.misses;
    return 0;
}

}
```

Baseline: 354.3.

## Add flat grouped GEMV kernel for short matrices with run-merged T partials

Adds a grouped GEMV kernel for lazily deferred matrices with at most 128 rows. It reads column-major data as flat float4 vectors and computes N and T products together. Runs of consecutive T-members are accumulated into one shared partial slab, scaled by per-run alpha slots, so fewer finalize members and partial reads are needed. The plan builder is reorganised to partition descriptors into flat and old groups, remap alpha slots and track stats. This adds complexity and touches numerical summation order.

After: 354.0. No clear change (-0.1%).

```diff
diff --git a/include/totsu_f32hip.h b/include/totsu_f32hip.h
--- a/include/totsu_f32hip.h
+++ b/include/totsu_f32hip.h
@@ -47,6 +47,7 @@
 int thip_get_lazy_gemv(int *host_on);
 int thip_lazy_gemv_stats(int64_t *host_deferred, int64_t *host_flushes);
 int thip_lazy_plan_stats(int64_t *host_hits, int64_t *host_misses);
+int thip_lazy_flat_stats(int64_t *descriptors_flat, int64_t *descriptors_old, int64_t *t_slabs);
 int thip_lazy_read_stats(int64_t *host_served, int64_t *host_fetches);
 int thip_transform_sp(size_t n, float alpha, const float *mat, const float *x, float beta, float *y);
 enum { THIP_A_F32 = 0, THIP_A_BF16 = 1, THIP_A_F16 = 2 };
diff --git a/rust/totsu_f32hip/src/ffi.rs b/rust/totsu_f32hip/src/ffi.rs
--- a/rust/totsu_f32hip/src/ffi.rs
+++ b/rust/totsu_f32hip/src/ffi.rs
@@ -142,6 +142,7 @@
     pub fn thip_lazy_gemv_stats(host_deferred: *mut i64, host_flushes: *mut i64) -> c_int;
     pub fn thip_lazy_plan_stats(host_hits: *mut i64, host_misses: *mut i64) -> c_int;
     pub fn thip_lazy_read_stats(host_served: *mut i64, host_fetches: *mut i64) -> c_int;
+    pub fn thip_lazy_flat_stats(descriptors_flat: *mut i64, descriptors_old: *mut i64, t_slabs: *mut i64) -> c_int;
     pub fn thip_proj_zero(dual_cone: c_int, n: usize, x: *mut f32) -> c_int;
     pub fn thip_proj_rpos(n: usize, x: *mut f32) -> c_int;
     pub fn thip_proj_soc(n: usize, x: *mut f32) -> c_int;
diff --git a/totsu_amd/_lib.py b/totsu_amd/_lib.py
--- a/totsu_amd/_lib.py
+++ b/totsu_amd/_lib.py
@@ -107,6 +107,7 @@
     "thip_lazy_gemv_stats": (_i, [C.POINTER(C.c_int64), C.POINTER(C.c_int64)]),
     "thip_lazy_plan_stats": (_i, [C.POINTER(C.c_int64), C.POINTER(C.c_int64)]),
     "thip_lazy_read_stats": (_i, [C.POINTER(C.c_int64), C.POINTER(C.c_int64)]),
+    "thip_lazy_flat_stats": (_i, [C.POINTER(C.c_int64), C.POINTER(C.c_int64), C.POINTER(C.c_int64)]),
     "thip_to_bf16": (_i, [_sz, _sz, _vp, _vp, _sz]),
     "thip_to_f16": (_i, [_sz, _sz, _vp, _vp, _sz, _vp]),
     "thip_transform_ge_f16": (_i, [_i, _sz, _sz, _f, _vp, _sz, _vp, _vp, _f, _vp]),
diff --git a/totsu_amd/csrc/thip_common.h b/totsu_amd/csrc/thip_common.h
--- a/totsu_amd/csrc/thip_common.h
+++ b/totsu_amd/csrc/thip_common.h
@@ -180,8 +180,10 @@
     const float *partN; int nN; size_t strideN;
     const float *partT; int nT; size_t strideT;
 };
-struct GroupDesc { const float *A; const float *xn; const float *xt; float *partN; float *partT; int nr, nc, cpc, pad; };
-int grouped_gemv(hipStream_t st, const GroupDesc *dev_tab, int n_desc, int max_tiles, int max_chunks, int mode);
+struct GroupDesc { const float *A; const float *xn; const float *xt; float *partN; float *partT; int nr, nc, cpc, run; const float *alphaT; };
+constexpr int GROUP_FLAT_MAX_ROWS = 128, GROUP_FLAT_MIN_COLS = 8;
+int grouped_gemv(hipStream_t st, const GroupDesc *dev_tab, int n_desc, int max_tiles, int max_chunks, int mode, int n_flat,
+                 int max_chunks_flat);
 struct GemvHint { int nj; int target_blocks; };
 const GemvHint *gemv_candidates(int *count);
 int dual_gemv_partials(hipStream_t st, size_t n_row, size_t n_col, const DenseA &A,
diff --git a/totsu_amd/csrc/thip_gemv.hip b/totsu_amd/csrc/thip_gemv.hip
--- a/totsu_amd/csrc/thip_gemv.hip
+++ b/totsu_amd/csrc/thip_gemv.hip
@@ -316,6 +316,172 @@
         __builtin_amdgcn_s_waitcnt(0xc07f);
         __builtin_amdgcn_wave_barrier();
         float *dst = d.partT + (size_t)tile * d.nc + c0;
+        for (int t = lane; t < c1 - c0; t += 64) dst[t] = lw[t];
+    }
+}
+
+constexpr int FLAT_LOADS = 4;
+
+__device__ __forceinline__ void wave_lds_fence()
+{
+    __builtin_amdgcn_s_waitcnt(0xc07f);
+    __builtin_amdgcn_wave_barrier();
+}
+
+__device__ __forceinline__ void flat_row_col(int v, int k, int nr, float inv_nr, int &row, int &col)
+{
+    const int f = 4 * v + k;
+    col = (int)(((float)f + 0.5f) * inv_nr);
+    row = f - col * nr;
+}
+
+template <bool DO_N, bool DO_T, int NH, int GU>
+__device__ __forceinline__ void flat_step(const float *__restrict__ Ab, int nr, int cc, const unsigned (&voff)[NH], bool ok_last,
+                                          const float *xsl, const int (&xcol)[NH][4], const float (&xtm)[NH][4][4],
+                                          float (&acc)[NH][4], float *lw, bool first, int lane)
+{
+    typedef float f32x4_t __attribute__((ext_vector_type(4)));
+    f32x4_t q[GU][NH];
+#pragma unroll
+    for (int u = 0; u < GU; ++u) {
+        typedef const __attribute__((address_space(1))) char *gbytes_t;
+        typedef const __attribute__((address_space(1))) f32x4_t *gvec_t;
+        gbytes_t grp = (gbytes_t)(Ab + (size_t)(cc + 4 * u) * nr);
+#pragma unroll
+        for (int h = 0; h < NH; ++h) q[u][h] = __builtin_nontemporal_load((gvec_t)(grp + voff[h]));
+    }
+#pragma unroll
+    for (int u = 0; u < GU; ++u)
+#pragma unroll
+        for (int k = 0; k < 4; ++k) q[u][NH - 1][k] = ok_last ? q[u][NH - 1][k] : 0.0f;
+    if constexpr (DO_N) {
+#pragma unroll
+        for (int u = 0; u < GU; ++u)
+#pragma unroll
+            for (int h = 0; h < NH; ++h)
+#pragma unroll
+                for (int k = 0; k < 4; ++k) acc[h][k] = fmaf(q[u][h][k], xsl[cc + 4 * u + xcol[h][k]], acc[h][k]);
+    }
+    if constexpr (DO_T) {
+        float p[4 * GU];
+#pragma unroll
+        for (int u = 0; u < GU; ++u)
+#pragma unroll
+            for (int j = 0; j < 4; ++j) {
+                float s = 0.0f;
+#pragma unroll
+                for (int h = 0; h < NH; ++h)
+#pragma unroll
+                    for (int k = 0; k < 4; ++k) s = fmaf(q[u][h][k], xtm[h][k][j], s);
+                p[4 * u + j] = s;
+            }
+        if constexpr (GU >= 2) {
+#pragma unroll
+            for (int i = 0; i < GU / 2; ++i) {
+                const float r = multi_reduce<8>(p + 8 * i, lane);
+                if ((lane & 7) == 0) { float *dst = lw + cc + 8 * i + (lane >> 3); *dst = first ? r : *dst + r; }
+            }
+        } else {
+            const float r = multi_reduce<4>(p, lane);
+            if ((lane & 15) == 0) { float *dst = lw + cc + (lane >> 4); *dst = first ? r : *dst + r; }
+        }
+    }
+}
+
+template <bool DO_N, bool DO_T, int NH>
+__device__ __forceinline__ void flat_block(const GroupDesc &d, int chunk, bool first, float *xsl, float *lw, int lane)
+{
+    const int nr = d.nr;
+    const int c0 = chunk * d.cpc, c1 = min(d.nc, c0 + d.cpc), ncu = c1 - c0, n4 = ncu & ~3;
+    const float *__restrict__ Ab = d.A + (size_t)c0 * nr;
+    const float inv_nr = 1.0f / (float)nr;
+    const float alT = (DO_T && d.alphaT != nullptr) ? d.alphaT[0] : 1.0f;
+    unsigned voff[NH];
+    int xcol[NH][4];
+    float xtm[NH][4][4], acc[NH][4];
+    bool ok[NH];
+#pragma unroll
+    for (int h = 0; h < NH; ++h) {
+        const int v = lane + 64 * h;
+        ok[h] = v < nr;
+        voff[h] = ok[h] ? 16u * (unsigned)v : 0u;
+#pragma unroll
+        for (int k = 0; k < 4; ++k) {
+            int row, col;
+            flat_row_col(v, k, nr, inv_nr, row, col);
+            if (!ok[h]) { row = 0; col = 0; }
+            xcol[h][k] = col;
+            acc[h][k] = 0.0f;
+            float xt = 0.0f;
+            if constexpr (DO_T) { if (ok[h]) xt = d.xt[row] * alT; }
+#pragma unroll
+            for (int j = 0; j < 4; ++j) xtm[h][k][j] = (col == j) ? xt : 0.0f;
+        }
+    }
+    if constexpr (DO_N) {
+        for (int t = lane; t < ncu; t += 64) xsl[t] = d.xn[c0 + t];
+        wave_lds_fence();
+    }
+    int cc = 0;
+    constexpr int GU = FLAT_LOADS / NH;
+    for (; cc + 4 * GU <= n4; cc += 4 * GU)
+        flat_step<DO_N, DO_T, NH, GU>(Ab, nr, cc, voff, ok[NH - 1], xsl, xcol, xtm, acc, lw, first, lane);
+    for (; cc < n4; cc += 4)
+        flat_step<DO_N, DO_T, NH, 1>(Ab, nr, cc, voff, ok[NH - 1], xsl, xcol, xtm, acc, lw, first, lane);
+    const int r0 = lane, r1 = lane + 64;
+    const bool ok0 = r0 < nr, ok1 = r1 < nr;
+    float t0 = 0.0f, t1 = 0.0f;
+    if (cc < ncu) {
+        float xt0 = 0.0f, xt1 = 0.0f;
+        if constexpr (DO_T) { xt0 = ok0 ? d.xt[r0] * alT : 0.0f; xt1 = ok1 ? d.xt[r1] * alT : 0.0f; }
+        for (; cc < ncu; ++cc) {
+            const float *col = Ab + (size_t)cc * nr;
+            const float a0 = ok0 ? col[r0] : 0.0f, a1 = ok1 ? col[r1] : 0.0f;
+            if constexpr (DO_N) { const float xs = d.xn[c0 + cc]; t0 = fmaf(a0, xs, t0); t1 = fmaf(a1, xs, t1); }
+            if constexpr (DO_T) {
+                const float r = wave_sum(fmaf(a0, xt0, a1 * xt1));
+                if (lane == 0) lw[cc] = first ? r : lw[cc] + r;
+            }
+        }
+    }
+    if constexpr (DO_N) {
+        wave_lds_fence();
+#pragma unroll
+        for (int h = 0; h < NH; ++h)
+#pragma unroll
+            for (int k = 0; k < 4; ++k) {
+                int row, col, l2 = lane;
+                asm volatile("" : "+v"(l2));
+                flat_row_col(l2 + 64 * h, k, nr, inv_nr, row, col);
+                if (ok[h]) xsl[col * GROUP_FLAT_MAX_ROWS + row] = acc[h][k];
+            }
+        wave_lds_fence();
+        float *dst = d.partN + (size_t)chunk * nr;
+        constexpr int S = GROUP_FLAT_MAX_ROWS;
+        if (ok0) dst[r0] = (((xsl[r0] + xsl[S + r0]) + xsl[2 * S + r0]) + xsl[3 * S + r0]) + t0;
+        if (ok1) dst[r1] = (((xsl[r1] + xsl[S + r1]) + xsl[2 * S + r1]) + xsl[3 * S + r1]) + t1;
+        wave_lds_fence();
+    }
+}
+
+static_assert(4 * GROUP_FLAT_MAX_ROWS <= MAXCW, "the N row sums reuse the unit's x_N slab");
+
+template <bool DO_N, bool DO_T>
+__global__ __launch_bounds__(BLK, 4) void grouped_flat_k(const GroupDesc *__restrict__ tab)
+{
+    __shared__ float ldsX[DO_N ? 4 * MAXCW : 4];
+    __shared__ float ldsT[DO_T ? 4 * MAXCW : 4];
+    const GroupDesc d0 = tab[blockIdx.z];
+    const int lane = threadIdx.x & 63, wave = __builtin_amdgcn_readfirstlane(threadIdx.x >> 6);
+    const int chunk = blockIdx.y * 4 + wave;
+    if (d0.run <= 0 || chunk * d0.cpc >= d0.nc) return;
+    float *xsl = ldsX + wave * (DO_N ? MAXCW : 1), *lw = ldsT + wave * (DO_T ? MAXCW : 1);
+    if (d0.nr > 64) for (int k = 0; k < d0.run; ++k) flat_block<DO_N, DO_T, 2>(tab[blockIdx.z + k], chunk, k == 0, xsl, lw, lane);
+    else            for (int k = 0; k < d0.run; ++k) flat_block<DO_N, DO_T, 1>(tab[blockIdx.z + k], chunk, k == 0, xsl, lw, lane);
+    if constexpr (DO_T) {
+        wave_lds_fence();
+        const int c0 = chunk * d0.cpc, c1 = min(d0.nc, c0 + d0.cpc);
+        float *dst = d0.partT + c0;
         for (int t = lane; t < c1 - c0; t += 64) dst[t] = lw[t];
     }
 }
@@ -607,8 +773,17 @@
     return 0;
 }
 
-int grouped_gemv(hipStream_t st, const GroupDesc *dev_tab, int n_desc, int max_tiles, int max_chunks, int mode)
-{
+int grouped_gemv(hipStream_t st, const GroupDesc *dev_tab, int n_desc, int max_tiles, int max_chunks, int mode, int n_flat,
+                 int max_chunks_flat)
+{
+    if (n_flat > 0) {
+        dim3 gf(1, max_chunks_flat, n_flat);
+        if (mode == 2)      hipLaunchKernelGGL((grouped_flat_k<true, true>), gf, dim3(BLK), 0, st, dev_tab);
+        else if (mode == 1) hipLaunchKernelGGL((grouped_flat_k<false, true>), gf, dim3(BLK), 0, st, dev_tab);
+        else                hipLaunchKernelGGL((grouped_flat_k<true, false>), gf, dim3(BLK), 0, st, dev_tab);
+        THIP_LAUNCH_CHECK();
+        dev_tab += n_flat; n_desc -= n_flat;
+    }
     if (n_desc <= 0) return 0;
     dim3 g(max_tiles, max_chunks, n_desc);
     if (mode == 2)      hipLaunchKernelGGL((grouped_gemv_k<true, true>), g, dim3(BLK), 0, st, dev_tab);
diff --git a/totsu_amd/csrc/thip_lazy.hip b/totsu_amd/csrc/thip_lazy.hip
--- a/totsu_amd/csrc/thip_lazy.hip
+++ b/totsu_amd/csrc/thip_lazy.hip
@@ -65,8 +65,12 @@
     int nN = 0, nT = 0, nD = 0, nDot = 0, nLong = 0, nShort = 0, maxlen = 0;
     int long_members = 0;
     int maxt[3] = { 0, 0, 0 }, maxc[3] = { 0, 0, 0 };
+    int nflat[3] = { 0, 0, 0 }, maxcf[3] = { 0, 0, 0 };
+    int64_t desc_flat = 0, desc_old = 0, t_slabs = 0;
     size_t off_dot = 0, off_grp = 0, off_mem = 0, off_alpha = 0, off_beta = 0;
     size_t n_members = 0, n_groups = 0;
+    std::vector<float> alpha_init;
+    std::vector<int> alpha_slot;
     std::vector<float> alphas, betas;
     std::vector<int> mem_slot, grp_slot;
     std::vector<BigMat> big;
@@ -114,8 +118,20 @@
     char *pin[2] = { nullptr, nullptr }; size_t pin_bytes[2] = { 0, 0 }; hipEvent_t pin_ev[2] = { nullptr, nullptr };
     int pin_next = 0;
     long long flushes = 0, deferred = 0, hits = 0, misses = 0;
+    long long desc_flat = 0, desc_old = 0, t_slabs = 0;
     std::atomic<bool> pending{ false };
 } Q;
+
+bool flat_on()
+{
+    static const int on = getenv("THIP_LAZY_FLAT") ? atoi(getenv("THIP_LAZY_FLAT")) : 1;
+    return on != 0;
+}
+int flat_run_env()
+{
+    static const int k = getenv("THIP_LAZY_FLAT_RUN") ? atoi(getenv("THIP_LAZY_FLAT_RUN")) : 0;
+    return k < 0 ? 0 : (k > 64 ? 64 : k);
+}
 
 bool overlap(uintptr_t a0, uintptr_t a1, uintptr_t b0, uintptr_t b1) { return a0 < b1 && b0 < a1; }
 
@@ -425,9 +441,10 @@
         return 0;
     }
     const GroupDesc *dgd = reinterpret_cast<const GroupDesc *>(p->dev);
-    THIP_RC(grouped_gemv(st, dgd, p->nD, p->maxt[2], (p->maxc[2] + 3) / 4, 2));
-    THIP_RC(grouped_gemv(st, dgd + p->nD, p->nN, p->maxt[0], (p->maxc[0] + 3) / 4, 0));
-    THIP_RC(grouped_gemv(st, dgd + p->nD + p->nN, p->nT, p->maxt[1], (p->maxc[1] + 3) / 4, 1));
+    THIP_RC(grouped_gemv(st, dgd, p->nD, p->maxt[2], (p->maxc[2] + 3) / 4, 2, p->nflat[2], (p->maxcf[2] + 3) / 4));
+    THIP_RC(grouped_gemv(st, dgd + p->nD, p->nN, p->maxt[0], (p->maxc[0] + 3) / 4, 0, p->nflat[0], (p->maxcf[0] + 3) / 4));
+    THIP_RC(grouped_gemv(st, dgd + p->nD + p->nN, p->nT, p->maxt[1], (p->maxc[1] + 3) / 4, 1, p->nflat[1], (p->maxcf[1] + 3) / 4));
+    Q.desc_flat += p->desc_flat; Q.desc_old += p->desc_old; Q.t_slabs += p->t_slabs;
     for (const BigMat &b : p->big) {
         GemvPartials gp;
         THIP_RC(dual_gemv_partials(st, b.nr, b.nc, dense_f32(b.A, b.nr), b.xn, b.xt, b.xn != nullptr, b.xt != nullptr, false,
@@ -471,7 +488,7 @@
 
 void factors_from_calls(const Plan *p, const float *alpha, const float *beta, std::vector<float> &alphas, std::vector<float> &betas)
 {
-    alphas.assign(p->n_members, 0.0f);
+    alphas = p->alpha_init;
     betas.assign(p->n_groups, 1.0f);
     for (size_t i = 0; i < p->calls.size(); ++i) {
         const Call &c = p->calls[i];
@@ -543,6 +560,13 @@
     return 0;
 }
 
+std::vector<float> table_alphas(const Plan *p, const std::vector<float> &by_member)
+{
+    std::vector<float> out = p->alpha_init;
+    for (size_t e = 0; e < by_member.size() && e < p->alpha_slot.size(); ++e) out[p->alpha_slot[e]] = by_member[e];
+    return out;
+}
+
 int flush_products()
 {
     hipStream_t st = ctx().stream;
@@ -568,7 +592,7 @@
     Plan *p = find_plan(key, calls, 0);
     if (p) {
         Q.hits += 1;
-        THIP_RC(upload_factors(p, alphas, betas));
+        THIP_RC(upload_factors(p, table_alphas(p, alphas), betas));
         THIP_RC(launch_plan(p));
         plan_done(p);
         return 0;
@@ -600,38 +624,84 @@
         }
     }
 
-    struct MatPlan { size_t offN, offT; int cpc, tiles, chunks; int big; };
+    struct Rec { int g, m, tg, tm, mode; bool flat; int cpc, tiles, chunks, run, kslot; size_t offN, offT; };
+    std::vector<Rec> recs[3];
+    struct MatPlan { int big, mode, idx; };
     std::vector<std::vector<MatPlan>> mp(groups.size());
-    for (size_t gi = 0; gi < groups.size(); ++gi) mp[gi].assign(groups[gi].mem.size(), MatPlan{ 0, 0, 0, 0, 0, -1 });
+    for (size_t gi = 0; gi < groups.size(); ++gi) mp[gi].assign(groups[gi].mem.size(), MatPlan{ -1, -1, -1 });
+    for (int gi : order)
+        for (size_t mi = 0; mi < groups[gi].mem.size(); ++mi) {
+            const Member &m = groups[gi].mem[mi];
+            if ((m.kind != K_N && m.kind != K_T) || m.nr * m.nc > LAZY_MAX_ELEMS) continue;
+            const MatRef pr = partner[gi][mi];
+            if (m.kind == K_T && pr.g >= 0) continue;
+            Rec r{ gi, (int)mi, -1, -1, 0, false, 0, 0, 0, 0, -1, 0, 0 };
+            if (m.kind == K_T) { r.mode = 1; r.tg = gi; r.tm = (int)mi; }
+            else if (pr.g >= 0) { r.mode = 2; r.tg = pr.g; r.tm = pr.m; }
+            static const size_t wave_elems = getenv("THIP_LAZY_WAVE_ELEMS") ? (size_t)atol(getenv("THIP_LAZY_WAVE_ELEMS")) : 40000;
+            size_t c = wave_elems / (m.nr < 128 ? m.nr : 128);
+            c = std::max<size_t>(8, std::min<size_t>(1024, c / 8 * 8));
+            r.cpc = (int)c; r.tiles = (int)((m.nr + 127) / 128); r.chunks = (int)((m.nc + c - 1) / c);
+            r.flat = flat_on() && m.nr <= (size_t)GROUP_FLAT_MAX_ROWS && m.nc >= (size_t)GROUP_FLAT_MIN_COLS
+                     && ((uintptr_t)m.A & 15) == 0;
+            recs[r.mode].push_back(r);
+        }
+    size_t t_units = 0;
+    for (int k = 0; k < 3; ++k) {
+        std::stable_partition(recs[k].begin(), recs[k].end(), [](const Rec &r) { return r.flat; });
+        for (const Rec &r : recs[k]) if (r.flat && k != 0) t_units += (size_t)r.chunks;
+    }
+    int run_max = flat_run_env();
+    if (run_max == 0) { run_max = 8; while (run_max > 1 && t_units / (size_t)run_max < 8192) run_max /= 2; }
+    int n_kslots = 0, n_followers = 0;
+    for (int k = 0; k < 3; ++k) {
+        int lead = -1;
+        for (size_t i = 0; i < recs[k].size() && recs[k][i].flat; ++i) {
+            Rec &r = recs[k][i];
+            r.run = 1;
+            if (k == 0) continue;
+            r.kslot = n_kslots++;
+            if (lead >= 0) {
+                Rec &l = recs[k][lead];
+                const Member &a = groups[l.tg].mem[l.tm], &b = groups[r.tg].mem[r.tm];
+                if (l.run < run_max && l.tg == r.tg && a.nr == b.nr && a.nc == b.nc) { l.run += 1; r.run = 0; n_followers += 1; continue; }
+            }
+            lead = (int)i;
+        }
+    }
+
     size_t floats = 0;
+    for (int k = 0; k < 3; ++k)
+        for (size_t i = 0; i < recs[k].size(); ++i) {
+            Rec &r = recs[k][i];
+            const Member &m = groups[r.g].mem[r.m];
+            if (k != 1) { r.offN = floats; floats += (size_t)r.chunks * m.nr; floats = (floats + 63) / 64 * 64; }
+            if (k != 0) {
+                if (r.flat && r.run == 0) r.offT = recs[k][i - 1].offT;
+                else { r.offT = floats; floats += (size_t)r.tiles * m.nc; floats = (floats + 63) / 64 * 64; }
+                p->t_slabs += (r.flat && r.run == 0) ? 0 : r.tiles;
+            }
+            (r.flat ? p->desc_flat : p->desc_old) += 1;
+            mp[r.g][r.m] = MatPlan{ -1, k, (int)i };
+            if (k == 2) mp[r.tg][r.tm] = MatPlan{ -1, k, (int)i };
+        }
     int nDot = 0;
     for (size_t gi = 0; gi < groups.size(); ++gi)
         for (size_t mi = 0; mi < groups[gi].mem.size(); ++mi) {
             const Member &m = groups[gi].mem[mi];
             if (m.kind == K_DOT) { nDot += 1; continue; }
-            if (m.kind != K_N && m.kind != K_T) continue;
+            if ((m.kind != K_N && m.kind != K_T) || m.nr * m.nc <= LAZY_MAX_ELEMS) continue;
             const MatRef pr = partner[gi][mi];
             const bool paired = pr.g >= 0;
             if (paired && m.kind == K_T) continue;
             const Member *tm = paired ? &groups[pr.g].mem[pr.m] : nullptr;
-            const bool doN = m.kind == K_N, doT = m.kind == K_T || paired;
-            MatPlan q{ 0, 0, 0, 0, 0, -1 };
-            if (m.nr * m.nc > LAZY_MAX_ELEMS) {
-                BigMat b{ m.A, doN ? m.x : nullptr, m.kind == K_T ? m.x : (tm ? tm->x : nullptr), m.nr, m.nc, floats,
-                          dual_gemv_scratch_floats(m.nr, m.nc) };
-                q.big = (int)p->big.size();
-                p->big.push_back(b);
-                floats += b.scr_floats; floats = (floats + 63) / 64 * 64;
-            } else {
-                static const size_t wave_elems = getenv("THIP_LAZY_WAVE_ELEMS") ? (size_t)atol(getenv("THIP_LAZY_WAVE_ELEMS")) : 40000;
-                size_t c = wave_elems / (m.nr < 128 ? m.nr : 128);
-                c = std::max<size_t>(8, std::min<size_t>(1024, c / 8 * 8));
-                q.cpc = (int)c; q.tiles = (int)((m.nr + 127) / 128); q.chunks = (int)((m.nc + c - 1) / c);
-                if (doN) { q.offN = floats; floats += (size_t)q.chunks * m.nr; floats = (floats + 63) / 64 * 64; }
-                if (doT) { q.offT = floats; floats += (size_t)q.tiles * m.nc; floats = (floats + 63) / 64 * 64; }
-            }
-            mp[gi][mi] = q;
-            if (paired) mp[pr.g][pr.m] = q;
+            const bool doN = m.kind == K_N;
+            BigMat b{ m.A, doN ? m.x : nullptr, m.kind == K_T ? m.x : (tm ? tm->x : nullptr), m.nr, m.nc, floats,
+                      dual_gemv_scratch_floats(m.nr, m.nc) };
+            mp[gi][mi].big = (int)p->big.size();
+            if (paired) mp[pr.g][pr.m].big = mp[gi][mi].big;
+            p->big.push_back(b);
+            floats += b.scr_floats; floats = (floats + 63) / 64 * 64;
         }
     const size_t dot_off = floats;
     floats += (size_t)nDot;
@@ -645,20 +715,14 @@
         dual_gemv_partials_geometry(b.nr, b.nc, dense_f32(b.A, b.nr), b.xn != nullptr, b.xt != nullptr, dpart + b.scr_off, &biggp[k]);
     }
 
-    int nN = 0, nT = 0, nD = 0;
-    for (size_t gi = 0; gi < groups.size(); ++gi)
-        for (size_t mi = 0; mi < groups[gi].mem.size(); ++mi) {
-            const Member &m = groups[gi].mem[mi];
-            if ((m.kind != K_N && m.kind != K_T) || mp[gi][mi].big >= 0) continue;
-            if (partner[gi][mi].g >= 0) { if (m.kind == K_N) nD += 1; }
-            else if (m.kind == K_N) nN += 1; else nT += 1;
-        }
+    const int nN = (int)recs[0].size(), nT = (int)recs[1].size(), nD = (int)recs[2].size();
     p->nN = nN; p->nT = nT; p->nD = nD; p->nDot = nDot;
+    const size_t n_fin = n_members - (size_t)n_followers, n_alpha = n_fin + (size_t)n_kslots;
     const size_t b_gd = up256((size_t)(nN + nT + nD) * sizeof(GroupDesc));
     const size_t b_dot = up256((size_t)nDot * sizeof(DotD));
     const size_t b_grp = up256(groups.size() * sizeof(FinGroup));
-    const size_t b_mem = up256(n_members * sizeof(FinMember));
-    const size_t b_al = up256(n_members * sizeof(float)), b_be = up256(groups.size() * sizeof(float));
+    const size_t b_mem = up256(n_fin * sizeof(FinMember));
+    const size_t b_al = up256(n_alpha * sizeof(float)), b_be = up256(groups.size() * sizeof(float));
     p->off_dot = b_gd; p->off_grp = b_gd + b_dot; p->off_mem = p->off_grp + b_grp; p->off_alpha = p->off_mem + b_mem;
     p->off_beta = p->off_alpha + b_al;
     const size_t b_tab = p->off_beta + b_be;
@@ -674,38 +738,54 @@
     FinMember *hm = reinterpret_cast<FinMember *>(host + p->off_mem);
     p->mem_slot.assign(calls.size(), -1);
     p->grp_slot.assign(groups.size(), -1);
-    int iD = 0, iN = 0, iT = 0, iDot = 0;
-    size_t mpos = 0;
+    const float *dalpha = reinterpret_cast<const float *>(p->dev + p->off_alpha);
+    GroupDesc *gdk[3] = { gdN, gdT, gdD };
+    for (int k = 0; k < 3; ++k)
+        for (size_t i = 0; i < recs[k].size(); ++i) {
+            const Rec &r = recs[k][i];
+            const Member &m = groups[r.g].mem[r.m];
+            GroupDesc gd{ m.A, nullptr, nullptr, nullptr, nullptr, (int)m.nr, (int)m.nc, r.cpc, r.flat ? r.run : 0, nullptr };
+            if (k != 1) { gd.xn = m.x; gd.partN = dpart + r.offN; }
+            if (k != 0) {
+                gd.xt = groups[r.tg].mem[r.tm].x; gd.partT = dpart + r.offT;
+                if (r.flat) gd.alphaT = dalpha + n_fin + r.kslot;
+            }
+            gdk[k][i] = gd;
+            if (r.flat) { p->nflat[k] += 1; p->maxcf[k] = std::max(p->maxcf[k], r.chunks); }
+            else { p->maxt[k] = std::max(p->maxt[k], r.tiles); p->maxc[k] = std::max(p->maxc[k], r.chunks); }
+        }
+    p->alpha_init.assign(n_alpha, 0.0f);
+    p->alpha_slot.assign(n_members, 0);
+    int iDot = 0;
+    size_t mpos = 0, e = 0;
     for (size_t oi = 0; oi < order.size(); ++oi) {
         const int gi = order[oi];
         const Group &g = groups[gi];
         p->grp_slot[gi] = (int)oi;
-        if ((int)g.len > SHORT_LEN) { p->maxlen = std::max(p->maxlen, (int)g.len); p->long_members = std::max(p->long_members, (int)g.mem.size()); }
-        hg[oi] = FinGroup{ g.y, (int)g.len, (int)mpos, (int)g.mem.size() };
-        for (size_t mi = 0; mi < g.mem.size(); ++mi) {
+        const size_t first = mpos;
+        for (size_t mi = 0; mi < g.mem.size(); ++mi, ++e) {
             const Member &m = g.mem[mi];
             FinMember fm{ nullptr, nullptr, 0, M_ADDV, 0 };
+            size_t slot = mpos;
+            bool seen = true;
             if (m.kind == K_N || m.kind == K_T) {
                 const MatPlan &q = mp[gi][mi];
-                const MatRef pr = partner[gi][mi];
                 fm.type = M_PART;
                 if (q.big >= 0) {
                     const GemvPartials &gp = biggp[q.big];
                     if (m.kind == K_N) { fm.src = gp.partN; fm.count = gp.nN; fm.stride = gp.strideN; }
                     else               { fm.src = gp.partT; fm.count = gp.nT; fm.stride = gp.strideT; }
-                } else if (m.kind == K_N) {
-                    GroupDesc gd{ m.A, m.x, nullptr, dpart + q.offN, nullptr, (int)m.nr, (int)m.nc, q.cpc, 0 };
-                    if (pr.g >= 0) {
-                        gd.xt = groups[pr.g].mem[pr.m].x; gd.partT = dpart + q.offT;
-                        gdD[iD++] = gd; p->maxt[2] = std::max(p->maxt[2], q.tiles); p->maxc[2] = std::max(p->maxc[2], q.chunks);
-                    } else { gdN[iN++] = gd; p->maxt[0] = std::max(p->maxt[0], q.tiles); p->maxc[0] = std::max(p->maxc[0], q.chunks); }
-                    fm.src = dpart + q.offN; fm.count = q.chunks; fm.stride = m.nr;
                 } else {
-                    if (pr.g < 0) {
-                        GroupDesc gd{ m.A, nullptr, m.x, nullptr, dpart + q.offT, (int)m.nr, (int)m.nc, q.cpc, 0 };
-                        gdT[iT++] = gd; p->maxt[1] = std::max(p->maxt[1], q.tiles); p->maxc[1] = std::max(p->maxc[1], q.chunks);
+                    const Rec &r = recs[q.mode][q.idx];
+                    if (m.kind == K_N) { fm.src = dpart + r.offN; fm.count = r.chunks; fm.stride = m.nr; }
+                    else {
+                        fm.src = dpart + r.offT; fm.count = r.tiles; fm.stride = m.nc;
+                        if (r.flat) {
+                            slot = n_fin + (size_t)r.kslot;
+                            seen = r.run > 0;
+                            if (seen) p->alpha_init[mpos] = 1.0f;
+                        }
                     }
-                    fm.src = dpart + q.offT; fm.count = q.tiles; fm.stride = m.nc;
                 }
             } else if (m.kind == K_DOT) {
                 dd[iDot] = DotD{ m.A, m.x, dpart + dot_off + iDot, (int)m.inlen, 0 };
@@ -714,10 +794,14 @@
             } else if (m.kind == K_AXPY) { fm.src = m.A; fm.xs = m.x; fm.type = M_AXPY; }
             else if (m.kind == K_CONST) { fm.type = M_CONST; }
             else { fm.src = m.x; fm.type = M_ADDV; }
-            if (m.call >= 0 && (size_t)m.call < calls.size()) p->mem_slot[m.call] = (int)mpos;
-            hm[mpos++] = fm;
-        }
-    }
+            if (m.call >= 0 && (size_t)m.call < calls.size()) p->mem_slot[m.call] = (int)slot;
+            p->alpha_slot[e] = (int)slot;
+            if (seen) hm[mpos++] = fm;
+        }
+        if ((int)g.len > SHORT_LEN) { p->maxlen = std::max(p->maxlen, (int)g.len); p->long_members = std::max(p->long_members, (int)(mpos - first)); }
+        hg[oi] = FinGroup{ g.y, (int)g.len, (int)first, (int)(mpos - first) };
+    }
+    alphas = table_alphas(p, alphas);
     memcpy(host + p->off_alpha, alphas.data(), alphas.size() * sizeof(float));
     memcpy(host + p->off_beta, betas.data(), betas.size() * sizeof(float));
     THIP_TRY(hipMemcpyAsync(p->dev, host, b_tab, hipMemcpyHostToDevice, st));
@@ -1206,6 +1290,14 @@
     return 0;
 }
 
+int thip_lazy_flat_stats(int64_t *descriptors_flat, int64_t *descriptors_old, int64_t *t_slabs)
+{
+    if (descriptors_flat) *descriptors_flat = Q.desc_flat;
+    if (descriptors_old) *descriptors_old = Q.desc_old;
+    if (t_slabs) *t_slabs = Q.t_slabs;
+    return 0;
+}
+
 int thip_lazy_plan_stats(int64_t *host_hits, int64_t *host_misses)
 {
     if (host_hits) *host_hits = Q.hits;
```
